# GothiProCoder/OCR-System

Measured on AMD Instinct MI355X. Metric: pages/sec end-to-end det+rec, A4@200DPI, higher is better.
Workload: dtype bf16; 1 GPU; end-to-end det+rec, batch=64 A4@200DPI pages per GPU (BASELINE configs[3]); pages_per_gpu=64, global_batch=64, lines_last_step=3279, pages_gathered_last_step=64, parallelism=pages sharded dp1, 1 all-gather/step, ranks=1, input=pages pre-decoded (uint8 RGB) and resident in HBM when the timed region starts, det_sub_batch=64

## Files before the change

### include/lumina_ocr.h

```cpp
#ifndef LUMINA_OCR_H
#define LUMINA_OCR_H
#include <stddef.h>
#include <stdint.h>

#ifdef __cplusplus
extern "C" {
#endif

typedef struct lumina_ocr lumina_ocr_t;

#define LUMINA_REC_H 32
#define LUMINA_REC_W 320
#define LUMINA_REC_T 80
#define LUMINA_MAX_WORDS 40
#define LUMINA_MAX_BOXES 1000

int lumina_ocr_create(int device, lumina_ocr_t** out);
void lumina_ocr_destroy(lumina_ocr_t* h);
const char* lumina_ocr_last_error(const lumina_ocr_t* h);
const char* lumina_ocr_version(void);
int lumina_ocr_set_option(lumina_ocr_t* h, const char* key, int value);

int lumina_ocr_load_det_weights(lumina_ocr_t* h, const void* blob, size_t nbytes);
int lumina_ocr_load_rec_weights(lumina_ocr_t* h, const void* blob, size_t nbytes);
int lumina_ocr_num_classes(const lumina_ocr_t* h);

int lumina_ocr_normalize(lumina_ocr_t* h, const uint8_t* img_dev, int n, int height, int width, int hp, int wp,
                         const float scale[3], const float shift[3], int layout_nchw, uint16_t* out_dev, void* stream);

int lumina_ocr_det_forward(lumina_ocr_t* h, const uint8_t* pages_dev, int batch, int height, int width, int hp, int wp,
                           uint16_t* prob_dev, void* stream);

int lumina_ocr_det_postprocess(lumina_ocr_t* h, const uint16_t* prob_dev, int batch, int hp, int wp, int valid_h, int valid_w,
                               float thresh, float box_thresh, float unclip_ratio, int min_size, int max_boxes,
                               int32_t* boxes_dev, float* scores_dev, int32_t* counts_dev, void* stream);

int lumina_ocr_rec_crop(lumina_ocr_t* h, const uint8_t* pages_dev, int batch, int height, int width, const int32_t* quads_dev,
                        const int32_t* page_idx_dev, int n_crops, uint8_t* crops_dev, int32_t* widths_dev, void* stream);

int lumina_ocr_rec_crop_oriented(lumina_ocr_t* h, const uint8_t* pages_dev, int batch, int height, int width, const int32_t* quads_dev,
                                 const int32_t* page_idx_dev, int n_crops, const int32_t* flip_dev, uint8_t* crops_dev, int32_t* widths_dev,
                                 void* stream);

int lumina_ocr_load_cls_weights(lumina_ocr_t* h, const void* blob, size_t nbytes);

int lumina_ocr_cls_crop(lumina_ocr_t* h, const uint8_t* pages_dev, int batch, int height, int width, const int32_t* quads_dev,
                        const int32_t* page_idx_dev, int n_crops, uint8_t* crops_dev, int32_t* widths_dev, void* stream);

int lumina_ocr_cls_forward(lumina_ocr_t* h, const uint8_t* crops_dev, const int32_t* widths_dev, int n_crops, float thresh, int32_t* label_dev,
                           float* score_dev, int32_t* flip_dev, void* stream);

int lumina_ocr_rec_forward(lumina_ocr_t* h, const uint8_t* crops_dev, const int32_t* widths_dev, int n_crops, int32_t* idx_dev,
                           float* prob_dev, void* stream);

int lumina_ocr_ctc_decode(lumina_ocr_t* h, const int32_t* idx_dev, const float* prob_dev, int n, int32_t* text_dev, int32_t* len_dev,
                          float* score_dev, void* stream);

int lumina_ocr_ctc_decode_words(lumina_ocr_t* h, const int32_t* idx_dev, const float* prob_dev, int n, const int32_t* quads_dev,
                                const int32_t* widths_dev, const int32_t* flip_dev , int space_id, int32_t* text_dev,
                                int32_t* len_dev, float* score_dev, int32_t* word_quads_dev, int32_t* word_span_dev, float* word_score_dev,
                                int32_t* word_count_dev, void* stream);

int lumina_ocr_resize_lanczos(lumina_ocr_t* h, const uint8_t* in_dev, int n, int height, int width, int channels, uint8_t* out_dev,
                              int out_h, int out_w, void* stream);
int lumina_ocr_enhance(lumina_ocr_t* h, const uint8_t* img_dev, int n, int height, int width, float contrast, float sharpness,
                       uint8_t* tmp_dev, uint8_t* out_dev, void* stream);

int lumina_ocr_binarize(lumina_ocr_t* h, const uint8_t* img_dev, int n, int height, int width, int adaptive, int threshold, uint8_t* out_dev,
                        void* stream);

int lumina_ocr_exif_transpose(lumina_ocr_t* h, const uint8_t* img_dev, int n, int height, int width, int orientation, uint8_t* out_dev, void* stream);
int lumina_ocr_grayscale(lumina_ocr_t* h, const uint8_t* img_dev, int n, int height, int width, uint8_t* out_dev, void* stream);
int lumina_ocr_denoise(lumina_ocr_t* h, const uint8_t* img_dev, int n, int height, int width, uint8_t* out_dev, void* stream);

int lumina_ocr_deskew(lumina_ocr_t* h, const uint8_t* pages_dev, int n, int height, int width, uint8_t* out_dev, double* rot_dev,
                      int32_t* info_dev, uint8_t* edges_dev, int32_t* segs_dev, int32_t* nsegs_dev, void* stream);
int lumina_ocr_deskew_warp(lumina_ocr_t* h, const uint8_t* pages_dev, int n, int height, int width, const double* rot_dev, uint8_t* out_dev,
                           void* stream);

int lumina_ocr_table_rules(lumina_ocr_t* h, const uint8_t* pages_dev, int n, int height, int width, int threshold, int gap, int min_len,
                           int max_thick, int max_rules, int32_t* hrules_dev, int32_t* vrules_dev, int32_t* counts_dev, uint64_t* hmask_dev,
                           void* stream);

int lumina_ocr_selection_marks(lumina_ocr_t* h, const uint8_t* pages_dev, int n, int height, int width, int threshold, int min_side,
                               int max_side, int max_marks, int32_t* marks_dev, int32_t* counts_dev, uint64_t* mask_dev, void* stream);

int lumina_ocr_rules_and_marks(lumina_ocr_t* h, const uint8_t* pages_dev, int n, int height, int width, int threshold, int gap, int min_len,
                               int max_thick, int max_rules, int32_t* hrules_dev, int32_t* vrules_dev, int32_t* rule_counts_dev, int min_side,
                               int max_side, int max_marks, int32_t* marks_dev, int32_t* mark_counts_dev, void* stream);

int lumina_ocr_selection_marks_round(lumina_ocr_t* h, const uint8_t* pages_dev, int n, int height, int width, int threshold, int min_side,
                                     int max_side, int max_marks, int32_t* marks_dev, int32_t* counts_dev, uint64_t* mask_dev, int out_max,
                                     int ring_div, int band_div, int band_min, int32_t* round_dev, int32_t* round_counts_dev, void* stream);

int lumina_ocr_rules_and_marks_round(lumina_ocr_t* h, const uint8_t* pages_dev, int n, int height, int width, int threshold, int gap,
                                     int min_len, int max_thick, int max_rules, int32_t* hrules_dev, int32_t* vrules_dev,
                                     int32_t* rule_counts_dev, int min_side, int max_side, int max_marks, int32_t* marks_dev,
                                     int32_t* mark_counts_dev, int out_max, int ring_div, int band_div, int band_min, int32_t* round_dev,
                                     int32_t* round_counts_dev, void* stream);

int lumina_ocr_barcodes(lumina_ocr_t* h, const uint8_t* pages_dev, int n, int height, int width, int threshold, int quiet, int max_dist,
                        int min_rows, int row_gap, int max_codes, int32_t* codes_dev, int32_t* syms_dev, int32_t* counts_dev,
                        const uint64_t* mask_in_dev, uint64_t* mask_out_dev, void* stream);

int lumina_ocr_barcodes_kinds(lumina_ocr_t* h, const uint8_t* pages_dev, int n, int height, int width, int threshold, int quiet, int max_dist,
                              int min_rows, int row_gap, int max_codes, int32_t* codes_dev, int32_t* syms_dev, int32_t* counts_dev,
                              const uint64_t* mask_in_dev, uint64_t* mask_out_dev, void* stream, int kinds);

int lumina_ocr_qrcodes(lumina_ocr_t* h, const uint8_t* pages_dev, int n, int height, int width, int threshold, int min_module, int max_module,
                       int quiet, int centre_tol, int ring_tol, int timing_max, int max_finders, int max_codes, int32_t* codes_dev,
                       int32_t* data_dev, int32_t* counts_dev, int32_t* finder_counts_dev, const uint64_t* mask_in_dev, uint64_t* mask_out_dev,
                       void* stream);

int lumina_ocr_qrcodes_versions(lumina_ocr_t* h, const uint8_t* pages_dev, int n, int height, int width, int threshold, int min_module,
                                int max_module, int quiet, int centre_tol, int ring_tol, int timing_max, int max_finders, int max_codes,
                                int max_version, int32_t* codes_dev, uint8_t* data_dev, int32_t* counts_dev, int32_t* finder_counts_dev,
                                const uint64_t* mask_in_dev, uint64_t* mask_out_dev, void* stream);

int lumina_ocr_datamatrix(lumina_ocr_t* h, const uint8_t* pages_dev, int n, int height, int width, int threshold, int min_module, int max_module,
                          int quiet, int timing_max, int solid_max, int max_candidates, int max_codes, int32_t* codes_dev, int32_t* data_dev,
                          int32_t* counts_dev, int32_t* candidate_counts_dev, const uint64_t* mask_in_dev, uint64_t* mask_out_dev, void* stream);

size_t lumina_ocr_aztec_workspace_bytes(int n, int height, int width, int max_finders, int max_codes);
int lumina_ocr_aztec(lumina_ocr_t* h, const uint8_t* pages_dev, int n, int height, int width, int threshold, int min_module, int max_module,
                     int quiet, int centre_tol, int ring_tol, int mark_max, int max_finders, int max_codes, int32_t* codes_dev, int32_t* data_dev,
                     int32_t* counts_dev, int32_t* finder_counts_dev, const uint64_t* mask_in_dev, uint64_t* mask_out_dev, void* stream);

size_t lumina_ocr_aztec_layers_workspace_bytes(int n, int height, int width, int max_finders, int max_codes);
int lumina_ocr_aztec_layers(lumina_ocr_t* h, const uint8_t* pages_dev, int n, int height, int width, int threshold, int min_module, int max_module,
                            int quiet, int centre_tol, int ring_tol, int mark_max, int max_finders, int max_codes, int max_layers, int32_t* codes_dev,
                            uint16_t* data_dev, int32_t* counts_dev, int32_t* finder_counts_dev, const uint64_t* mask_in_dev, uint64_t* mask_out_dev,
                            void* stream);

size_t lumina_ocr_page_quarter_workspace_bytes(int n, int height, int width);
int lumina_ocr_page_quarter(lumina_ocr_t* h, const uint8_t* pages_dev, int n, int height, int width, int threshold, int ratio,
                            int64_t* energies_dev, int32_t* sideways_dev, void* stream);
int lumina_ocr_page_turn(lumina_ocr_t* h, const uint8_t* pages_dev, int n, int height, int width, const int32_t* index_dev, int m, int turn,
                         uint8_t* out_dev, void* stream);
int lumina_ocr_page_vote(lumina_ocr_t* h, const int32_t* flip_dev, const int32_t* page_idx_dev, int n, int pages, int32_t* counts_dev, void* stream);

int lumina_ocr_load_svtr_weights(lumina_ocr_t* h, const void* blob, size_t nbytes);
int lumina_ocr_svtr_forward(lumina_ocr_t* h, const uint8_t* crops_dev, const int32_t* widths_dev, int n_crops, int32_t* idx_dev, float* prob_dev,
                            void* stream);
int lumina_ocr_svtr_num_classes(const lumina_ocr_t* h);
int lumina_ocr_svtr_dtype(const lumina_ocr_t* h);

int lumina_ocr_jpeg_encode(lumina_ocr_t* h, const uint8_t* pages_dev, int n, int height, int width, int quality, int optimize,
                           uint8_t* out_dev, size_t out_stride, int32_t* sizes_dev, void* stream);
int lumina_ocr_jpeg_probe(const uint8_t* file, size_t size, int info[6]);
int lumina_ocr_jpeg_decode(lumina_ocr_t* h, const uint8_t* const* files, const size_t* sizes, int n, int height, int width, uint8_t* out_dev,
                           int* status, void* stream);
int lumina_ocr_jpeg_decode_async(lumina_ocr_t* h, const uint8_t* const* files, const size_t* sizes, int n, int height, int width, uint8_t* out_dev,
                                 int* status_pinned, int passes, void* stream);
int lumina_ocr_jpeg_last_passes(const lumina_ocr_t* h);

int lumina_ocr_png_probe(const uint8_t* file, size_t size, int info[8]);
int lumina_ocr_png_decode(lumina_ocr_t* h, const uint8_t* const* files, const size_t* sizes, int n, int height, int width, uint8_t* out_dev,
                          int* status, void* stream);

int lumina_ocr_flate_image_decode(lumina_ocr_t* h, const uint8_t* const* streams, const size_t* sizes, int n, int height, int width,
                                  const int32_t* params, const uint8_t* const* palettes, uint8_t* out_dev, int* status, void* stream);
int lumina_ocr_ccitt_decode(lumina_ocr_t* h, const uint8_t* const* streams, const size_t* sizes, int n, int rows, int columns,
                            const int32_t* params, uint8_t* out_dev, int* status, void* stream);
int lumina_ocr_fax_decode(lumina_ocr_t* h, const uint8_t* const* streams, const size_t* sizes, int n, int rows, int columns,
                          const int32_t* params, uint8_t* out_dev, int* status, void* stream);

int lumina_ocr_strip_image_decode(lumina_ocr_t* h, const uint8_t* const* strips, const size_t* sizes, int m, const int32_t* strip_counts, int n,
                                  int height, int width, int rows_per_strip, const int32_t* params, const uint8_t* const* palettes,
                                  uint8_t* out_dev, int* status, void* stream);

int lumina_ocr_jpeg_coefficients(lumina_ocr_t* h, const uint8_t* pages_dev, int n, int height, int width, int quality, int16_t* coefs_dev,
                                 void* stream);

int lumina_ocr_conv2d(lumina_ocr_t* h, const uint16_t* x_dev, int n, int height, int width, int cin, const uint16_t* w_host,
                      const float* bias_host, int cout, int ks, int stride, int act, const uint16_t* res_dev, uint16_t* y_dev,
                      void* stream);
int lumina_ocr_read_tap(lumina_ocr_t* h, const char* name, uint16_t* out_host, size_t capacity_elems, int dims[4]);
int lumina_ocr_conv_timing(lumina_ocr_t* h, double* total_ms, double* total_flops, int* launches);
int lumina_ocr_conv_timing_detail(lumina_ocr_t* h, char* buf, size_t cap);

#ifdef __cplusplus
}
#endif
#endif
```

### ocr-system_amd/csrc/capi.hip

```cpp
#include <cstdlib>
#include <cstring>
#include <new>

#include "../../include/lumina_ocr.h"
#include "dbpost.h"
#include "deskew.h"
#include "engine.h"
#include "marks.h"
#include "barcodes.h"
#include "qrcodes.h"
#include "datamatrix.h"
#include "aztec.h"
#include "ops.h"
#include "orient.h"
#include "resize.h"
#include "runs.h"
#include "jpeg.h"
#include "jpegdec.h"
#include "lzw.h"
#include "pngdec.h"
#include "ccitt.h"
#include "stem_conv.h"
#include "tables.h"

#define API_TRY try {
#define API_CATCH(h)                                                             \
    }                                                                            \
    catch (const std::exception& e) { return locr_fail(h, "exception", e.what()); } \
    catch (...) { return locr_fail(h, "exception", "unknown"); }

namespace {
struct DeviceGuard {
    int prev = -1;
    hipError_t err;
    explicit DeviceGuard(int dev) {
        if (hipGetDevice(&prev) != hipSuccess) prev = -1;
        err = hipSetDevice(dev);
        if (prev == dev) prev = -1;
    }
    ~DeviceGuard() { if (prev >= 0) (void)hipSetDevice(prev); }
    DeviceGuard(const DeviceGuard&) = delete;
    DeviceGuard& operator=(const DeviceGuard&) = delete;
};
}
#define BIND(h)                                                                                              \
    if (!(h)) return 1;                                                                                      \
    DeviceGuard _device_guard((h)->device);                                                                  \
    if (_device_guard.err != hipSuccess) return locr_fail((h), "hipSetDevice", hipGetErrorString(_device_guard.err))

static int hip_rc(lumina_ocr* h, const char* what, hipError_t e) { return e == hipSuccess ? 0 : locr_fail(h, what, hipGetErrorString(e)); }

template <class F> static int drain_launches(lumina_ocr* h, const char* what, F&& f) {
    if (hipDeviceSynchronize() != hipSuccess) return locr_fail(h, what, "sync failed");
    for (const LaunchRecord& r : h->launches) {
        float t = 0.f;
        if (hipEventElapsedTime(&t, r.e0.get(), r.e1.get()) != hipSuccess) t = 0.f;
        f(r, t);
    }
    h->launches.clear();
    return 0;
}

template <class WS> static int fit_group(int group, int n, WS&& ws) {
    if (group > n) group = n;
    while (group > 1 && ws(group) > ((size_t)1 << 30)) group = (group + 1) / 2;
    return group;
}
template <class WS, class Body> static int for_page_groups(lumina_ocr* h, int n, int group, WS&& ws, Body&& body) {
    for (int b0 = 0; b0 < n; b0 += group) {
        const int nb = n - b0 < group ? n - b0 : group;
        if (eng_ws_reserve(h, ws(nb)) || body(b0, nb)) return 1;
    }
    return 0;
}

template <class T> struct CodeGroup {
    const uint8_t* rgb; int nb; int32_t* codes; T* data; int32_t* counts; int32_t* slot_counts; const unsigned long long* mask_in; unsigned long long* mask_out;
    template <class P> void bind(P& p) const { p.rgb = rgb; p.B = nb; p.codes = codes; p.counts = counts; p.mask_in = mask_in; p.mask_out = mask_out; }
};
template <class T, class WS, class Launch>
static int matrix_codes(lumina_ocr_t* h, const char* what, const char* bad_params, const uint8_t* pages_dev, int n, int height, int width, int max_codes,
                        int row_len, int32_t* codes_dev, T* data_dev, int32_t* counts_dev, int32_t* slot_counts_dev, const uint64_t* mask_in_dev,
                        uint64_t* mask_out_dev, WS ws, Launch launch) {
    if (!h) return 1;
    if (n == 0) return 0;
    if (!pages_dev || !codes_dev || !data_dev || !counts_dev || n < 0) return locr_fail(h, what, "bad arguments");
    if (bad_params) return locr_fail(h, what, bad_params);
    if (ws(1) == 0) return locr_fail(h, what, "bad dimensions (sides 1..65535)");
    BIND(h);
    API_TRY
    const size_t nw = ((size_t)width + 63) / 64;
    return for_page_groups(h, n, fit_group(h->post_group, n, ws), ws, [&](int b0, int nb) {
        CodeGroup<T> g{};
        g.rgb = pages_dev + (size_t)b0 * height * width * 3; g.nb = nb;
        g.codes = codes_dev + (size_t)b0 * max_codes * 12; g.data = data_dev + (size_t)b0 * max_codes * row_len; g.counts = counts_dev + b0;
        g.slot_counts = slot_counts_dev ? slot_counts_dev + b0 : nullptr;
        g.mask_in = mask_in_dev ? reinterpret_cast<const unsigned long long*>(mask_in_dev) + (size_t)b0 * height * nw : nullptr;
        g.mask_out = mask_out_dev ? reinterpret_cast<unsigned long long*>(mask_out_dev) + (size_t)b0 * height * nw : nullptr;
        return hip_rc(h, what, launch(g, h->ws.get(), h->ws.cap));
    });
    API_CATCH(h)
}

extern "C" {

const char* lumina_ocr_version(void) { return "lumina-ocr-mi355x 0.1 (gfx950)"; }

int lumina_ocr_create(int device, lumina_ocr_t** out) {
    if (!out) return 1;
    *out = nullptr;
    lumina_ocr* eng = new (std::nothrow) lumina_ocr();
    if (!eng) return 1;
    eng->device = device;
    int ndev = 0;
    if (hipGetDeviceCount(&ndev) != hipSuccess || device < 0 || device >= ndev) {
        eng->err = "no HIP device " + std::to_string(device) + " (device count " + std::to_string(ndev) + ")";
        *out = eng;
        return 2;
    }
    if (hipSetDevice(device) != hipSuccess) { eng->err = "hipSetDevice failed"; *out = eng; return 2; }
    if (const char* e = getenv("LUMINA_RING_ORIENT")) eng->ring_orient = atoi(e) < 0 ? -1 : (atoi(e) != 0);
    if (getenv("LUMINA_CONV_NO_RING")) eng->conv_ring = false;
    if (getenv("LUMINA_BLOCKED")) eng->blocked_layout = atoi(getenv("LUMINA_BLOCKED")) != 0;
    *out = eng;
    return 0;
}

void lumina_ocr_destroy(lumina_ocr_t* h) {
    if (!h) return;
    (void)hipSetDevice(h->device);
    delete h;
}

const char* lumina_ocr_last_error(const lumina_ocr_t* h) { return h ? h->err.c_str() : "null handle"; }

int lumina_ocr_set_option(lumina_ocr_t* h, const char* key, int value) {
    if (!h || !key) return 1;
    if (!strcmp(key, "det_sub_batch")) h->det_sub_batch = value > 0 ? value : 1;
    else if (!strcmp(key, "rec_sub_batch")) h->rec_sub_batch = value > 0 ? value : 1;
    else if (!strcmp(key, "cls_sub_batch")) h->cls_sub_batch = value > 0 ? value : 1;
    else if (!strcmp(key, "keep_taps")) h->keep_taps = value < 0 || value > 2 ? 0 : value;
    else if (!strcmp(key, "time_convs")) h->time_convs = value != 0;
    else if (!strcmp(key, "fuse_head")) h->fuse_head = value != 0;
    else if (!strcmp(key, "fuse_mb")) h->fuse_mb = value != 0;
    else if (!strcmp(key, "fuse_pool")) h->fuse_pool = value != 0;
    else if (!strcmp(key, "fuse_stem")) h->fuse_stem = value != 0;
    else if (!strcmp(key, "fpn_multi")) h->fpn_multi = value != 0;
    else if (!strcmp(key, "fpn_compose")) h->fpn_compose = value != 0;
    else if (!strcmp(key, "fuse_short")) h->fuse_short = value != 0;
    else if (!strcmp(key, "conv_ring")) h->conv_ring = value != 0;
    else if (!strcmp(key, "blocked_layout")) h->blocked_layout = value != 0;
    else if (!strcmp(key, "conv_big_min")) h->conv_big_min = value >= 0 ? value : 1024;
    else if (!strcmp(key, "ring_orient")) h->ring_orient = value < 0 ? -1 : (value != 0);
    else if (!strcmp(key, "post_group")) h->post_group = value > 0 ? value : 1;
    else if (!strcmp(key, "tail_group")) h->tail_group = value > 0 ? value : 0;
    else if (!strcmp(key, "svtr_f16")) h->svtr_f16 = value < 0 ? -1 : (value != 0);
    else if (!strcmp(key, "png_sub_batch_mb")) h->pd_sub_batch_mb = value > 0 ? value : 1;
    else if (!strcmp(key, "conv2d_variant")) h->conv2d_variant = value < 0 || value > 2 ? 0 : value;
    else return locr_fail(h, "set_option: unknown key", key);
    return 0;
}

int lumina_ocr_load_det_weights(lumina_ocr_t* h, const void* blob, size_t nbytes) {
    if (!h || !blob) return 1;
    BIND(h);
    API_TRY return eng_load_det(h, blob, nbytes); API_CATCH(h)
}
int lumina_ocr_load_rec_weights(lumina_ocr_t* h, const void* blob, size_t nbytes) {
    if (!h || !blob) return 1;
    BIND(h);
    API_TRY return eng_load_rec(h, blob, nbytes); API_CATCH(h)
}
int lumina_ocr_num_classes(const lumina_ocr_t* h) { return h ? h->num_classes : 0; }

int lumina_ocr_normalize(lumina_ocr_t* h, const uint8_t* img_dev, int n, int height, int width, int hp, int wp, const float scale[3],
                         const float shift[3], int layout_nchw, uint16_t* out_dev, void* stream) {
    if (!h || !img_dev || !out_dev || hp < height || wp < width) return locr_fail(h, "normalize", "bad arguments");
    BIND(h);
    return hip_rc(h, "normalize", normalize_launch(img_dev, out_dev, n, height, width, hp, wp, height, width, scale, shift, layout_nchw, (hipStream_t)stream));
}

int lumina_ocr_det_forward(lumina_ocr_t* h, const uint8_t* pages_dev, int batch, int height, int width, int hp, int wp, uint16_t* prob_dev,
                           void* stream) {
    if (!h || !pages_dev || !prob_dev) return locr_fail(h, "det_forward", "null argument");
    BIND(h);
    API_TRY return eng_det_forward(h, pages_dev, batch, height, width, hp, wp, prob_dev, (hipStream_t)stream); API_CATCH(h)
}

int lumina_ocr_det_postprocess(lumina_ocr_t* h, const uint16_t* prob_dev, int batch, int hp, int wp, int valid_h, int valid_w, float thresh,
                               float box_thresh, float unclip_ratio, int min_size, int max_boxes, int32_t* boxes_dev, float* scores_dev,
                               int32_t* counts_dev, void* stream) {
    if (!h || !prob_dev || !boxes_dev || !scores_dev || !counts_dev) return locr_fail(h, "det_postprocess", "null argument");
    if (batch <= 0 || max_boxes <= 0 || valid_h > hp || valid_w > wp) return locr_fail(h, "det_postprocess", "bad dimensions");
    BIND(h);
    API_TRY
    return for_page_groups(h, batch, h->post_group, [&](int nb) { return dbpost_workspace_bytes(nb, hp, wp, max_boxes); }, [&](int b0, int nb) {
        DbPostParams p{};
        p.prob = prob_dev + (size_t)b0 * hp * wp; p.B = nb; p.Hp = hp; p.Wp = wp; p.valid_h = valid_h; p.valid_w = valid_w;
        p.thresh = thresh; p.box_thresh = box_thresh; p.unclip_ratio = unclip_ratio; p.min_size = min_size; p.max_boxes = max_boxes;
        p.boxes = boxes_dev + (size_t)b0 * max_boxes * 8; p.scores = scores_dev + (size_t)b0 * max_boxes; p.counts = counts_dev + b0;
        return hip_rc(h, "det_postprocess", dbpost_launch(p, h->ws.get(), h->ws.cap, (hipStream_t)stream));
    });
    API_CATCH(h)
}

int lumina_ocr_rec_crop(lumina_ocr_t* h, const uint8_t* pages_dev, int batch, int height, int width, const int32_t* quads_dev,
                        const int32_t* page_idx_dev, int n_crops, uint8_t* crops_dev, int32_t* widths_dev, void* stream) {
    if (!h || !pages_dev || !quads_dev || !page_idx_dev || !crops_dev || !widths_dev) return locr_fail(h, "rec_crop", "null argument");
    BIND(h);
    (void)batch;
    return hip_rc(h, "rec_crop", rec_crop_launch(pages_dev, height, width, quads_dev, page_idx_dev, n_crops, crops_dev, widths_dev, (hipStream_t)stream));
}

int lumina_ocr_load_cls_weights(lumina_ocr_t* h, const void* blob, size_t nbytes) {
    if (!h || !blob) return locr_fail(h, "load_cls_weights", "null argument");
    BIND(h);
    API_TRY return eng_load_cls(h, blob, nbytes); API_CATCH(h)
}

int lumina_ocr_cls_forward(lumina_ocr_t* h, const uint8_t* crops_dev, const int32_t* widths_dev, int n_crops, float thresh, int32_t* label_dev,
                           float* score_dev, int32_t* flip_dev, void* stream) {
    if (!h) return 1;
    if (n_crops <= 0) return 0;
    if (!crops_dev || !label_dev || !score_dev || !flip_dev) return locr_fail(h, "cls_forward", "null argument");
    BIND(h);
    API_TRY return eng_cls_forward(h, crops_dev, widths_dev, n_crops, thresh, label_dev, score_dev, flip_dev, (hipStream_t)stream); API_CATCH(h)
}

int lumina_ocr_rec_crop_oriented(lumina_ocr_t* h, const uint8_t* pages_dev, int batch, int height, int width, const int32_t* quads_dev,
                                 const int32_t* page_idx_dev, int n_crops, const int32_t* flip_dev, uint8_t* crops_dev, int32_t* widths_dev,
                                 void* stream) {
    if (!h) return 1;
    if (n_crops <= 0) return 0;
    if (!pages_dev || !quads_dev || !page_idx_dev || !flip_dev || !crops_dev || !widths_dev) return locr_fail(h, "rec_crop_oriented", "null argument");
    BIND(h);
    (void)batch;
    return hip_rc(h, "rec_crop_oriented", rec_crop_launch(pages_dev, height, width, quads_dev, page_idx_dev, n_crops, crops_dev, widths_dev,
                                                         (hipStream_t)stream, flip_dev));
}

int lumina_ocr_cls_crop(lumina_ocr_t* h, const uint8_t* pages_dev, int batch, int height, int width, const int32_t* quads_dev,
                        const int32_t* page_idx_dev, int n_crops, uint8_t* crops_dev, int32_t* widths_dev, void* stream) {
    if (!h) return 1;
    if (n_crops <= 0) return 0;
    if (!pages_dev || !quads_dev || !page_idx_dev || !crops_dev || !widths_dev) return locr_fail(h, "cls_crop", "null argument");
    BIND(h);
    (void)batch;
    return hip_rc(h, "cls_crop", cls_crop_launch(pages_dev, height, width, quads_dev, page_idx_dev, n_crops, crops_dev, widths_dev, (hipStream_t)stream));
}

int lumina_ocr_rec_forward(lumina_ocr_t* h, const uint8_t* crops_dev, const int32_t* widths_dev, int n_crops, int32_t* idx_dev, float* prob_dev,
                           void* stream) {
    if (!h || !crops_dev || !idx_dev || !prob_dev) return locr_fail(h, "rec_forward", "null argument");
    BIND(h);
    API_TRY return eng_rec_forward(h, crops_dev, widths_dev, n_crops, idx_dev, prob_dev, (hipStream_t)stream); API_CATCH(h)
}

int lumina_ocr_load_svtr_weights(lumina_ocr_t* h, const void* blob, size_t nbytes) {
    if (!h || !blob) return locr_fail(h, "load_svtr_weights", "null argument");
    BIND(h);
    API_TRY return eng_load_svtr(h, blob, nbytes); API_CATCH(h)
}

int lumina_ocr_svtr_forward(lumina_ocr_t* h, const uint8_t* crops_dev, const int32_t* widths_dev, int n_crops, int32_t* idx_dev, float* prob_dev,
                            void* stream) {
    if (!h || !crops_dev || !idx_dev || !prob_dev) return locr_fail(h, "svtr_forward", "null argument");
    BIND(h);
    API_TRY return eng_svtr_forward(h, crops_dev, widths_dev, n_crops, idx_dev, prob_dev, (hipStream_t)stream); API_CATCH(h)
}

int lumina_ocr_ctc_decode(lumina_ocr_t* h, const int32_t* idx_dev, const float* prob_dev, int n, int32_t* text_dev, int32_t* len_dev,
                          float* score_dev, void* stream) {
    if (!h || !idx_dev || !prob_dev || !text_dev || !len_dev || !score_dev) return locr_fail(h, "ctc_decode", "null argument");
    BIND(h);
    if (n <= 0) return 0;
    return hip_rc(h, "ctc_decode", ctc_collapse_launch(idx_dev, prob_dev, text_dev, len_dev, score_dev, n, LUMINA_REC_T, (hipStream_t)stream));
}

int lumina_ocr_ctc_decode_words(lumina_ocr_t* h, const int32_t* idx_dev, const float* prob_dev, int n, const int32_t* quads_dev,
                                const int32_t* widths_dev, const int32_t* flip_dev, int space_id, int32_t* text_dev, int32_t* len_dev,
                                float* score_dev, int32_t* word_quads_dev, int32_t* word_span_dev, float* word_score_dev, int32_t* word_count_dev,
                                void* stream) {
    if (!h) return 1;
    if (n <= 0) return 0;
    if (!idx_dev || !prob_dev || !quads_dev || !widths_dev || !text_dev || !len_dev || !score_dev || !word_quads_dev || !word_span_dev ||
        !word_score_dev || !word_count_dev)
        return locr_fail(h, "ctc_decode_words", "null argument");
    BIND(h);
    return hip_rc(h, "ctc_decode_words", ctc_words_launch(idx_dev, prob_dev, quads_dev, widths_dev, flip_dev, space_id, text_dev, len_dev, score_dev,
                                                          word_quads_dev, word_span_dev, word_score_dev, word_count_dev, n, LUMINA_REC_T,
                                                          (hipStream_t)stream));
}

int lumina_ocr_conv2d(lumina_ocr_t* h, const uint16_t* x_dev, int n, int height, int width, int cin, const uint16_t* w_host,
                      const float* bias_host, int cout, int ks, int stride, int act, const uint16_t* res_dev, uint16_t* y_dev, void* stream) {
    if (!h || !x_dev || !w_host || !bias_host || !y_dev) return locr_fail(h, "conv2d", "null argument");
    if (cout % 8 != 0) return locr_fail(h, "conv2d", "cout must be a multiple of 8");
    BIND(h);
    API_TRY
    ConvLayer L;
    L.name = "conv2d"; L.ks = ks; L.stride = stride; L.cin = cin; L.cout = cout; L.act = act;
    if (!conv_pick_cfg(ks, stride, cin, cout, &L.cfg)) return locr_fail(h, "conv2d", "unsupported ks/stride/cin");
    std::vector<bf16_t> packed(conv_packed_weight_elems(cout, ks, cin, L.cfg.bn));
    pack_conv_weights(w_host, cout, ks, cin, L.cfg.bn, L.cfg.ck, packed.data(), L.cfg.nw == 6 ? 1 : 0);
    const int ntiles = (cout + L.cfg.bn - 1) / L.cfg.bn;
    std::vector<float> bias((size_t)ntiles * L.cfg.bn, 0.f);
    memcpy(bias.data(), bias_host, sizeof(float) * cout);
    const bool big_ok = ks == 3 && stride == 1 && cin >= 32 && cin % 16 == 0 && cout % 64 == 0 && L.cfg.bn == 64;
    if (h->conv2d_variant > 0 && !big_ok) return locr_fail(h, "conv2d", "conv2d_variant 1/2 needs ks 3, stride 1, cin % 16 == 0, cin >= 32, cout % 64 == 0");
    DeviceMem dw, db, dw2;
    auto upload = [](DeviceMem* d, const void* host, size_t bytes) {
        hipError_t e = mem_alloc(d, bytes);
        return e == hipSuccess ? hipMemcpy(d->get(), host, bytes, hipMemcpyHostToDevice) : e;
    };
    if (upload(&dw, packed.data(), packed.size() * 2) != hipSuccess || upload(&db, bias.data(), bias.size() * 4) != hipSuccess) return locr_fail(h, "conv2d", "weight upload");
    L.wpk = static_cast<bf16_t*>(dw.get()); L.bias = static_cast<float*>(db.get());
    if (h->conv2d_variant > 0) {
        L.cfg_big = L.cfg; L.cfg_big.nw = 6; L.cfg_big.ck = 16;
        std::vector<bf16_t> packed2(conv_packed_weight_elems(cout, ks, cin, 64));
        pack_conv_weights(w_host, cout, ks, cin, 64, 16, packed2.data(), 1);
        if (upload(&dw2, packed2.data(), packed2.size() * 2) != hipSuccess) return locr_fail(h, "conv2d", "weight upload");
        L.wpk_big = static_cast<bf16_t*>(dw2.get());
    }
    Tensor4 x; x.p = const_cast<bf16_t*>(x_dev); x.n = n; x.h = height; x.w = width; x.c = cin;
    Tensor4 y; y.p = y_dev; y.n = n; y.c = cout;
    y.h = (ks == 3) ? (height - 1) / stride + 1 : height / stride;
    y.w = (ks == 3) ? (width - 1) / stride + 1 : width / stride;
    Tensor4 r; r.p = const_cast<bf16_t*>(res_dev); r.n = n; r.h = y.h; r.w = y.w; r.c = cout;
    ConvCall call;
    call.res = res_dev ? &r : nullptr; call.variant = h->conv2d_variant;
    int rc = eng_run_conv(h, L, x, &y, (hipStream_t)stream, call);
    hipError_t e = hipStreamSynchronize((hipStream_t)stream);
    if (rc) return rc;
    return hip_rc(h, "conv2d sync", e);
    API_CATCH(h)
}

int lumina_ocr_read_tap(lumina_ocr_t* h, const char* name, uint16_t* out_host, size_t capacity_elems, int dims[4]) {
    if (!h || !name || !dims) return 1;
    auto it = h->taps.find(name);
    if (it == h->taps.end()) return locr_fail(h, "read_tap: unknown tap", name);
    BIND(h);
    const Tensor4& t = it->second;
    dims[0] = t.n; dims[1] = t.h; dims[2] = t.w; dims[3] = t.c;
    if (!out_host) return 0;
    if (capacity_elems < t.elems()) return locr_fail(h, "read_tap", "buffer too small");
    if (hipDeviceSynchronize() != hipSuccess) return locr_fail(h, "read_tap", "sync failed");
    return hip_rc(h, "read_tap", hipMemcpy(out_host, t.p, t.elems() * sizeof(bf16_t), hipMemcpyDeviceToHost));
}

int lumina_ocr_conv_timing(lumina_ocr_t* h, double* total_ms, double* total_flops, int* launches) {
    if (!h || !total_ms || !total_flops || !launches) return 1;
    BIND(h);
    double ms = 0, fl = 0;
    int count = 0;
    if (drain_launches(h, "conv_timing", [&](const LaunchRecord& r, float t) { ms += t; fl += r.flop; ++count; })) return 1;
    *total_ms = ms; *total_flops = fl; *launches = count;
    return 0;
}

static int get_coeffs(lumina_ocr* h, int in_size, int out_size, lumina_ocr::Coeffs* out) {
    auto key = std::make_pair(in_size, out_size);
    auto it = h->coeff_cache.find(key);
    if (it == h->coeff_cache.end()) {
        std::vector<int> bounds, kk;
        lumina_ocr::Coeffs c;
        lanczos_coeffs(in_size, out_size, &c.ksize, &bounds, &kk);
        c.bounds_host = std::make_shared<std::vector<int>>(bounds);
        c.bounds = static_cast<int*>(eng_upload(h, bounds.data(), bounds.size() * 4));
        c.kk = static_cast<int*>(eng_upload(h, kk.data(), kk.size() * 4));
        if (!c.bounds || !c.kk) return locr_fail(h, "resize", "coefficient table upload");
        it = h->coeff_cache.emplace(key, c).first;
    }
    *out = it->second;
    return 0;
}

int lumina_ocr_resize_lanczos(lumina_ocr_t* h, const uint8_t* in_dev, int n, int height, int width, int channels, uint8_t* out_dev,
                              int out_h, int out_w, void* stream) {
    if (!h || !in_dev || !out_dev || n <= 0 || height <= 0 || width <= 0 || out_h <= 0 || out_w <= 0 || channels <= 0)
        return locr_fail(h, "resize_lanczos", "bad arguments");
    BIND(h);
    API_TRY
    hipStream_t st = (hipStream_t)stream;
    const uint8_t* src = in_dev;
    int cur_w = width;
    const bool need_h = out_w != width, need_v = out_h != height;
    if (!need_h && !need_v) {
        return hip_rc(h, "resize_lanczos", hipMemcpyAsync(out_dev, in_dev, (size_t)n * height * width * channels, hipMemcpyDeviceToDevice, st));
    }
    if (need_h) {
        lumina_ocr::Coeffs c;
        if (get_coeffs(h, width, out_w, &c)) return 1;
        uint8_t* dst = out_dev;
        if (need_v) {
            if (hip_rc(h, "resize_lanczos", h->aux.reserve((size_t)n * height * out_w * channels))) return 1;
            dst = h->aux.get();
        }
        if (hip_rc(h, "resize_lanczos", resample_launch(src, dst, c.bounds, c.kk, c.ksize, n, height, width, channels, out_w, 0, c.bounds_host->data(), st))) return 1;
        src = dst; cur_w = out_w;
    }
    if (need_v) {
        lumina_ocr::Coeffs c;
        if (get_coeffs(h, height, out_h, &c)) return 1;
        if (hip_rc(h, "resize_lanczos", resample_launch(src, out_dev, c.bounds, c.kk, c.ksize, n, height, cur_w, channels, out_h, 1, c.bounds_host->data(), st))) return 1;
    }
    return 0;
    API_CATCH(h)
}

int lumina_ocr_enhance(lumina_ocr_t* h, const uint8_t* img_dev, int n, int height, int width, float contrast, float sharpness,
                       uint8_t* tmp_dev, uint8_t* out_dev, void* stream) {
    if (!h || !img_dev || !tmp_dev || !out_dev || n <= 0) return locr_fail(h, "enhance", "bad arguments");
    BIND(h);
    if (hip_rc(h, "enhance", h->sums.reserve(sizeof(unsigned long long) * (size_t)n))) return 1;
    unsigned long long* sums = reinterpret_cast<unsigned long long*>(h->sums.get());
    return hip_rc(h, "enhance", enhance_launch(img_dev, tmp_dev, out_dev, sums, n, height, width, contrast, sharpness, (hipStream_t)stream));
}

int lumina_ocr_binarize(lumina_ocr_t* h, const uint8_t* img_dev, int n, int height, int width, int adaptive, int threshold, uint8_t* out_dev, void* stream) {
    if (!h || !img_dev || !out_dev || n <= 0 || height <= 0 || width <= 0) return locr_fail(h, "binarize", "bad arguments");
    BIND(h);
    return hip_rc(h, "binarize", binarize_launch(img_dev, out_dev, n, height, width, adaptive != 0, threshold, (hipStream_t)stream));
}

int lumina_ocr_exif_transpose(lumina_ocr_t* h, const uint8_t* img_dev, int n, int height, int width, int orientation, uint8_t* out_dev, void* stream) {
    if (!h || !img_dev || !out_dev || n <= 0 || height <= 0 || width <= 0 || orientation < 1 || orientation > 8 || img_dev == out_dev)
        return locr_fail(h, "exif_transpose", "bad arguments (orientation 1..8, not in place)");
    BIND(h);
    return hip_rc(h, "exif_transpose", exif_transpose_launch(img_dev, out_dev, n, height, width, orientation, (hipStream_t)stream));
}

int lumina_ocr_grayscale(lumina_ocr_t* h, const uint8_t* img_dev, int n, int height, int width, uint8_t* out_dev, void* stream) {
    if (!h || !img_dev || !out_dev || n <= 0 || height <= 0 || width <= 0) return locr_fail(h, "grayscale", "bad arguments");
    BIND(h);
    return hip_rc(h, "grayscale", grayscale_launch(img_dev, out_dev, n, height, width, (hipStream_t)stream));
}

int lumina_ocr_denoise(lumina_ocr_t* h, const uint8_t* img_dev, int n, int height, int width, uint8_t* out_dev, void* stream) {
    if (!h || !img_dev || !out_dev || n <= 0 || height <= 0 || width <= 0 || img_dev == out_dev) return locr_fail(h, "denoise", "bad arguments (not in place)");
    BIND(h);
    return hip_rc(h, "denoise", median3_launch(img_dev, out_dev, n, height, width, (hipStream_t)stream));
}

int lumina_ocr_jpeg_encode(lumina_ocr_t* h, const uint8_t* pages_dev, int n, int height, int width, int quality, int optimize,
                           uint8_t* out_dev, size_t out_stride, int32_t* sizes_dev, void* stream) {
    if (!h || !pages_dev || !out_dev || !sizes_dev || n <= 0 || height <= 0 || width <= 0) return locr_fail(h, "jpeg_encode", "bad arguments");
    BIND(h);
    API_TRY
    if (eng_ws_reserve(h, jpeg_workspace_bytes(n, height, width))) return 1;
    JpegParams p{};
    p.rgb = pages_dev; p.n = n; p.height = height; p.width = width; p.quality = quality; p.optimize = optimize != 0; p.out = out_dev; p.out_stride = out_stride; p.sizes = sizes_dev;
    return hip_rc(h, "jpeg_encode", jpeg_encode_launch(p, h->ws.get(), h->ws.cap, (hipStream_t)stream));
    API_CATCH(h)
}

int lumina_ocr_jpeg_probe(const uint8_t* file, size_t size, int info[6]) {
    if (!file || !info) return -1;
    JdInfo i{};
    const int rc = jpegdec_probe(file, size, &i);
    info[0] = i.width; info[1] = i.height; info[2] = i.ncomp; info[3] = i.hs; info[4] = i.vs; info[5] = i.restart;
    return rc;
}

// ... 483 lines not shown
```

### ocr-system_amd/csrc/conv_mfma.h

```cpp
#pragma once
#include "common.h"

enum ConvOutMode : int {
    OUT_NORMAL = 0,
    OUT_UPSAMPLE = 1,
    OUT_CONVT = 2,
    OUT_CONVT1 = 3,
    OUT_POOL = 4,
};

struct ConvParams {
    const bf16_t* x;
    const bf16_t* wpk;
    const float* bias;
    const bf16_t* res;
    bf16_t* y;
    int N, H, W, Cin;
    int Ho, Wo;
    int Cout;
    int y_cstride, y_coff;
    int res_cstride, res_h, res_w, res_shift;
    int act;
    int out_mode, up_shift, convt_c;
    int tiles_x, tiles_y, n_tiles;
    const bf16_t* fuse_w;
    float fuse_b;
    const bf16_t* gate;
    int gate_hw;
    int dbg_skip;
    int pix_limit;
    const bf16_t* zeros;
    int x_blk, y_blk, res_blk;
    int n_src;
    const bf16_t* xs[4];
    int xs_shift[4];
    int xs_nchunk[4], xs_cstride[4];
    const bf16_t* wpk2;
    const float* bias2;
    bf16_t* y2;
    int y2_cstride;
};

struct ConvKernelCfg {
    int ks, stride, bn, ck, tw, nw;
};

size_t conv_packed_weight_elems(int cout_gemm, int ks, int cin, int bn);
void pack_conv_weights(const bf16_t* ohwi, int cout_gemm, int ks, int cin, int bn, int ck, bf16_t* out, int row_major = 0);

bool conv_pick_cfg(int ks, int stride, int cin, int cout_gemm, ConvKernelCfg* cfg);
hipError_t conv_launch(const ConvKernelCfg& cfg, ConvParams p, hipStream_t stream);
const char* conv_kernel_name(const ConvKernelCfg& cfg);

bool conv_ring_supported(const ConvKernelCfg& cfg, const ConvParams& p);
bool conv_ring_transposed(const ConvParams& p, int orientation);
hipError_t conv_ring_launch(ConvParams p, int orientation, hipStream_t stream);
const char* conv_ring_kernel_name(const ConvParams& p, int orientation);

bool conv_pw_supported(const ConvKernelCfg& cfg, const ConvParams& p);
hipError_t conv_pw_launch(const ConvParams& p, hipStream_t stream);
```

### ocr-system_amd/csrc/conv_mfma.hip

```cpp
#include "conv_mfma.h"

#include <cstdlib>

namespace {

template <int KS, int S, int BN, int CK, int TW, int NW = 4, int DB = 0, int MT = 2>
struct Cfg {
    static constexpr int NTHR = NW * 64;
    static constexpr bool DMA = (DB == 3 || DB == 4);
    static constexpr bool POOL = (DB == 4);
    static constexpr bool SC = (DB == 5);
    static_assert(!SC || (KS == 3 && S == 2 && CK == 16), "fused shortcut: the 3x3 / stride-2 block-entry kernel");
    static constexpr int TH = NW * MT;
    static constexpr int PAD = (KS == 3) ? 1 : 0;
    static constexpr int HH = (TH - 1) * S + KS;
    static constexpr int HW = (TW - 1) * S + KS;
    static constexpr int HWP = HW;
    static constexpr int NPL = CK / 8;
    static constexpr int HPX = HH * HWP;
    static constexpr int PMOD = (NPL >= 8) ? 2 : 4;
    static constexpr int PLANE_A = HPX + ((PMOD - HPX % 16) + 16) % 16;
    static constexpr int TAPS = KS * KS;
    static constexpr int WROWS = TAPS * BN;
    static constexpr int PLANE_W = WROWS;
    static constexpr int NT = BN / 32;
    static constexpr int A_BYTES = DMA ? HPX * NPL * 16 : PLANE_A * NPL * 16;
    static constexpr int W_BYTES = PLANE_W * NPL * 16;
    static constexpr int W2_ROWS = SC ? 4 * BN : 0, W2_ITEMS = W2_ROWS * NPL, W2IT = (W2_ITEMS + NTHR - 1) / NTHR, W2_BYTES = W2_ITEMS * 16;
    static constexpr int A_PIX = DMA ? NPL * 16 : 16, A_SL = DMA ? 16 : PLANE_A * 16;
    static constexpr int W_ROW = DMA ? NPL * 16 : 16, W_SL = DMA ? 16 : PLANE_W * 16;
    static constexpr int STAGE_PITCH = BN * 2 + 16;
    static constexpr int STAGE_BYTES = TH * TW * STAGE_PITCH;
    static constexpr int BUF_BYTES = A_BYTES + W_BYTES + W2_BYTES;
    static constexpr int LDS_BYTES = (BUF_BYTES * (DMA ? 2 : 1)) > STAGE_BYTES ? (BUF_BYTES * (DMA ? 2 : 1)) : STAGE_BYTES;
    static_assert(!DMA || (CK == 16 && KS == 3 && S == 1), "DMA variant: 3x3 / stride 1 / 16-channel chunks");
    static constexpr int A_ITEMS = HH * HW * NPL;
    static constexpr int AIT = (A_ITEMS + NTHR - 1) / NTHR;
    static constexpr int W_ITEMS = WROWS * NPL;
    static constexpr int WIT = (W_ITEMS + NTHR - 1) / NTHR;
    static constexpr int CPP = BN / 8;
};

__device__ __forceinline__ bf16x8_t lds_frag(const unsigned char* p) { return *reinterpret_cast<const bf16x8_t*>(p); }

__device__ __forceinline__ uint32_t mul_bf16x2(uint32_t a, uint32_t b) {
    const float lo = __uint_as_float(a << 16) * __uint_as_float(b << 16);
    const float hi = __uint_as_float(a & 0xFFFF0000u) * __uint_as_float(b & 0xFFFF0000u);
    return pack_bf16x2(lo, hi);
}
__device__ __forceinline__ uint4 mul_bf16x8(uint4 a, uint4 b) {
    return make_uint4(mul_bf16x2(a.x, b.x), mul_bf16x2(a.y, b.y), mul_bf16x2(a.z, b.z), mul_bf16x2(a.w, b.w));
}

template <int KS, int S, int BN, int CK, int TW, int NW, int DB, int MT>
__global__ __launch_bounds__(NW * 64, (BN <= 64 ? 2 : 1)) void conv_mfma_kernel(const ConvParams p) {
    using C = Cfg<KS, S, BN, CK, TW, NW, DB, MT>;
    constexpr int NTHR = C::NTHR;
    extern __shared__ __attribute__((aligned(16))) unsigned char smem[];

    const int tid = threadIdx.x, lane = tid & 63, wave = tid >> 6;
    unsigned char* sA = smem;
    unsigned char* sW = sA + C::A_BYTES;
    const int r = lane & 31, h = lane >> 5;

    const int lid = xcd_remap(blockIdx.x, gridDim.x);
    const int ntile = lid % p.n_tiles;
    const int mtile = lid / p.n_tiles;
    const int tiles_per_img = p.tiles_x * p.tiles_y;
    const int n_img = mtile / tiles_per_img;
    const int trem = mtile - n_img * tiles_per_img;
    const int tile_y = trem / p.tiles_x, tile_x = trem - tile_y * p.tiles_x;

    const bf16_t* ximg = p.x + (size_t)n_img * p.H * p.W * p.Cin;
    const int nchunks = p.Cin / CK;
    const bf16_t* wbase = p.wpk + (size_t)ntile * nchunks * C::W_ITEMS * 8;

    const bool blk_dbg = CK == 16 && (p.dbg_skip & 8);
    const int pstride = blk_dbg ? 16 : p.Cin;
    const int cadv = blk_dbg ? p.H * p.W * 16 : CK;
    int a_goff[C::AIT], a_loff[C::AIT];
    int a_gate[KS == 1 ? C::AIT : 1];
    constexpr bool pool = C::POOL;
    const int oyb = pool ? tile_y * (C::TH - 2) - 1 : tile_y * C::TH, oxb = pool ? tile_x * (TW - 2) - 1 : tile_x * TW;
    const int iy0 = oyb * S - C::PAD, ix0 = oxb * S - C::PAD;
#pragma unroll
    for (int it = 0; it < C::AIT; ++it) {
        const int i = tid + NTHR * it;
        const int pi = i / C::NPL, c = i - pi * C::NPL;
        const int hy = pi / C::HW, hx = pi - hy * C::HW;
        const int iy = iy0 + hy, ix = ix0 + hx;
        const bool item = i < C::A_ITEMS;
        const bool inb = item && iy >= 0 && iy < p.H && ix >= 0 && ix < p.W && (p.pix_limit == 0 || iy * p.W + ix < p.pix_limit);
        a_goff[it] = inb ? (iy * p.W + ix) * pstride + c * 8 : -1;
        a_loff[it] = item ? (c * C::PLANE_A + hy * C::HWP + hx) * 16 : -1;
        if constexpr (KS == 1) a_gate[it] = (inb && p.gate != nullptr) ? ((iy * p.W + ix) / p.gate_hw) * p.Cin + c * 8 : -1;
    }

    uint4 a_reg[C::AIT], w_reg[C::WIT];
    uint4 g_reg[KS == 1 ? C::AIT : 1];
    uint4 w2_reg[C::SC ? C::W2IT : 1];
    unsigned char* sW2 = sW + C::W_BYTES;
    const bf16_t* wbase2 = C::SC ? p.wpk2 + (size_t)ntile * nchunks * C::W2_ITEMS * 8 : nullptr;
#define ISSUE_LOADS(chunk_)                                                                          \
    {                                                                                                \
        const bf16_t* xa = ximg + (chunk_) * cadv;                                                   \
        const bool skipa_ = (p.dbg_skip & 2) && (chunk_) > 0, skipw_ = (p.dbg_skip & 1) && (chunk_) > 0; \
        _Pragma("unroll") for (int it = 0; it < C::AIT; ++it) {                                      \
            uint4 t_ = make_uint4(0, 0, 0, 0);                                                       \
            if (a_goff[it] >= 0 && !skipa_) t_ = *reinterpret_cast<const uint4*>(xa + a_goff[it]);   \
            a_reg[it] = t_;                                                                          \
            if constexpr (KS == 1) {                                                                 \
                uint4 g_ = make_uint4(0, 0, 0, 0);                                                   \
                if (a_gate[it] >= 0) g_ = *reinterpret_cast<const uint4*>(p.gate + a_gate[it] + (chunk_) * CK); \
                g_reg[it] = g_;                                                                      \
            }                                                                                        \
        }                                                                                            \
        const uint4* wsrc = reinterpret_cast<const uint4*>(wbase + (size_t)(chunk_) * C::W_ITEMS * 8); \
        _Pragma("unroll") for (int it = 0; it < C::WIT; ++it) {                                      \
            const int i = tid + NTHR * it;                                                          \
            uint4 t_ = make_uint4(0, 0, 0, 0);                                                       \
            if ((C::W_ITEMS % NTHR == 0 || i < C::W_ITEMS) && !skipw_) t_ = wsrc[i];                 \
            w_reg[it] = t_;                                                                          \
        }                                                                                            \
        if constexpr (C::SC) {                                                                       \
            const uint4* w2src = reinterpret_cast<const uint4*>(wbase2 + (size_t)(chunk_) * C::W2_ITEMS * 8); \
            _Pragma("unroll") for (int it = 0; it < C::W2IT; ++it) {                                 \
                const int i = tid + NTHR * it;                                                      \
                uint4 t_ = make_uint4(0, 0, 0, 0);                                                   \
                if (C::W2_ITEMS % NTHR == 0 || i < C::W2_ITEMS) t_ = w2src[i];                       \
                w2_reg[it] = t_;                                                                     \
            }                                                                                        \
        }                                                                                            \
    }
#define WRITE_LDS(boff_)                                                                             \
    {                                                                                                \
        _Pragma("unroll") for (int it = 0; it < C::AIT; ++it) {                                      \
            if constexpr (KS == 1) { if (a_gate[it] >= 0) a_reg[it] = mul_bf16x8(a_reg[it], g_reg[it]); } \
            if (a_loff[it] >= 0) *reinterpret_cast<uint4*>(sA + (boff_) + a_loff[it]) = a_reg[it];   \
        }                                                                                            \
        _Pragma("unroll") for (int it = 0; it < C::WIT; ++it) {                                      \
            const int i = tid + NTHR * it;                                                          \
            if (C::W_ITEMS % NTHR == 0 || i < C::W_ITEMS) *reinterpret_cast<uint4*>(sW + (boff_) + i * 16) = w_reg[it]; \
        }                                                                                            \
        if constexpr (C::SC) {                                                                       \
            _Pragma("unroll") for (int it = 0; it < C::W2IT; ++it) {                                 \
                const int i = tid + NTHR * it;                                                      \
                if (C::W2_ITEMS % NTHR == 0 || i < C::W2_ITEMS) *reinterpret_cast<uint4*>(sW2 + (boff_) + i * 16) = w2_reg[it]; \
            }                                                                                        \
        }                                                                                            \
    }

#define DMA_ISSUE(chunk_, boff_)                                                                     \
    {                                                                                                \
        const bf16_t* xa = ximg + (chunk_) * cadv;                                                   \
        const bool skipa_ = (p.dbg_skip & 2) && (chunk_) > 0, skipw_ = (p.dbg_skip & 1) && (chunk_) > 0; \
        _Pragma("unroll") for (int it = 0; it < C::AIT; ++it) {                                      \
            const int i = tid + NTHR * it;                                                           \
            if ((C::A_ITEMS % NTHR == 0 || i < C::A_ITEMS) && !skipa_) {                             \
                const bf16_t* src_ = a_goff[it] >= 0 ? xa + a_goff[it] : p.zeros;                    \
                __builtin_amdgcn_global_load_lds((const __attribute__((address_space(1))) void*)(src_), \
                    (__attribute__((address_space(3))) void*)(sA + (boff_) + (i - lane) * 16), 16, 0, 0); \
            }                                                                                        \
        }                                                                                            \
        const bf16_t* wsrc = wbase + (size_t)(chunk_) * C::W_ITEMS * 8;                              \
        _Pragma("unroll") for (int it = 0; it < C::WIT; ++it) {                                      \
            const int i = tid + NTHR * it;                                                           \
            if ((C::W_ITEMS % NTHR == 0 || i < C::W_ITEMS) && !skipw_)                               \
                __builtin_amdgcn_global_load_lds((const __attribute__((address_space(1))) void*)(wsrc + i * 8), \
                    (__attribute__((address_space(3))) void*)(sW + (boff_) + (i - lane) * 16), 16, 0, 0); \
        }                                                                                            \
    }

    f32x16_t acc[MT][C::NT];
#pragma unroll
    for (int mt = 0; mt < MT; ++mt)
#pragma unroll
        for (int nt = 0; nt < C::NT; ++nt)
#pragma unroll
            for (int j = 0; j < 16; ++j) acc[mt][nt][j] = 0.f;
    f32x16_t acc2[C::SC ? MT : 1][C::SC ? C::NT : 1];
    if constexpr (C::SC) {
#pragma unroll
        for (int mt = 0; mt < MT; ++mt)
#pragma unroll
            for (int nt = 0; nt < C::NT; ++nt)
#pragma unroll
                for (int j = 0; j < 16; ++j) acc2[mt][nt][j] = 0.f;
    }

    int aoff[MT];
#pragma unroll
    for (int mt = 0; mt < MT; ++mt) {
        const int ty = wave * MT + mt, tx = r;
        aoff[mt] = h * C::A_SL + ((ty * S) * C::HWP + tx * S) * C::A_PIX;
    }
    const int woff = h * C::W_SL + r * C::W_ROW;
    const int woff2 = h * (C::W2_ROWS * 16) + r * 16;

    constexpr int NSTEPS = C::TAPS * (CK / 16);
    bf16x8_t bfr[2][MT], afr[2][C::NT];
#define LOAD_FRAGS(boff_, st_, set_)                                                                               \
    {                                                                                                              \
        const int tap_ = (st_) / (CK / 16), kc_ = (st_) % (CK / 16), kh_ = tap_ / KS, kw_ = tap_ % KS;              \
        _Pragma("unroll") for (int mt = 0; mt < MT; ++mt)                                                           \
            bfr[set_][mt] = lds_frag(sA + (boff_) + aoff[mt] + (2 * kc_) * C::A_SL + (kh_ * C::HWP + kw_) * C::A_PIX); \
        _Pragma("unroll") for (int nt = 0; nt < C::NT; ++nt)                                                       \
            afr[set_][nt] = lds_frag(sW + (boff_) + woff + (2 * kc_) * C::W_SL + (tap_ * BN + nt * 32) * C::W_ROW);   \
    }
#define COMPUTE_CHUNK(boff_)                                                                                       \
    LOAD_FRAGS(boff_, 0, 0)                                                                                        \
    __builtin_amdgcn_sched_barrier(0);                                                                             \
    _Pragma("unroll") for (int st = 0; st < NSTEPS; ++st) {                                                        \
        _Pragma("unroll") for (int mt = 0; mt < MT; ++mt)                                                           \
            _Pragma("unroll") for (int nt = 0; nt < C::NT; ++nt)                                                   \
                acc[mt][nt] = __builtin_amdgcn_mfma_f32_32x32x16_bf16(afr[st & 1][nt], bfr[st & 1][mt], acc[mt][nt], 0, 0, 0); \
        if constexpr (C::SC) {    \
            if (st == 4 || st == 5 || st == 7 || st == 8) {                                                        \
                const int t2_ = (st == 4) ? 0 : (st == 5) ? 1 : (st == 7) ? 2 : 3;                                 \
                bf16x8_t a2_[C::NT];                                                                               \
                _Pragma("unroll") for (int nt = 0; nt < C::NT; ++nt) a2_[nt] = lds_frag(sW2 + (boff_) + woff2 + (t2_ * BN + nt * 32) * 16); \
                _Pragma("unroll") for (int mt = 0; mt < MT; ++mt)                                                   \
                    _Pragma("unroll") for (int nt = 0; nt < C::NT; ++nt)                                           \
                        acc2[mt][nt] = __builtin_amdgcn_mfma_f32_32x32x16_bf16(a2_[nt], bfr[st & 1][mt], acc2[mt][nt], 0, 0, 0); \
            }                                                                                                      \
        }                                                                                                          \
        if (st + 1 < NSTEPS) LOAD_FRAGS(boff_, st + 1, (st + 1) & 1)                                               \
        _Pragma("unroll") for (int q_ = 0; q_ < MT * C::NT; ++q_) {                                                \
            __builtin_amdgcn_sched_group_barrier(0x008, 1, 0);                      \
            if (q_ < MT + C::NT) __builtin_amdgcn_sched_group_barrier(0x100, 1, 0);  \
        }                                                                                                          \
        __builtin_amdgcn_sched_barrier(0);                                                                         \
    }
    if constexpr (C::DMA) {
        DMA_ISSUE(0, 0);
        for (int chunk = 0; chunk < nchunks; ++chunk) {
            const int boff = (chunk & 1) * C::BUF_BYTES;
            asm volatile("s_waitcnt vmcnt(0)" ::: "memory");
            __syncthreads();
            if (chunk + 1 < nchunks) DMA_ISSUE(chunk + 1, C::BUF_BYTES - boff);
            COMPUTE_CHUNK(boff)
        }
    } else {
        ISSUE_LOADS(0);
        for (int chunk = 0; chunk < nchunks; ++chunk) {
            __syncthreads();
            WRITE_LDS(0);
            __syncthreads();
            if (chunk + 1 < nchunks) ISSUE_LOADS(chunk + 1);
            COMPUTE_CHUNK(0)
        }
    }
#undef COMPUTE_CHUNK
#undef LOAD_FRAGS
#undef DMA_ISSUE

    const int cout_r8 = (p.Cout + 7) & ~7;
    const float* bptr = p.bias + ntile * BN;
    float4 bias_r[C::NT][4];
#pragma unroll
    for (int nt = 0; nt < C::NT; ++nt)
#pragma unroll
        for (int g = 0; g < 4; ++g) bias_r[nt][g] = *reinterpret_cast<const float4*>(bptr + nt * 32 + 8 * g + 4 * h);
    uint2 res_r[MT][C::NT][4];
    const bool has_res = p.res != nullptr;
    if (has_res) {
#pragma unroll
        for (int mt = 0; mt < MT; ++mt) {
            const int ty = wave * MT + mt, tx = r;
            const int oy = oyb + ty, ox = oxb + tx;
            const bool pvalid = oy >= 0 && ox >= 0 && oy < p.Ho && ox < p.Wo && (p.pix_limit == 0 || oy * p.Wo + ox < p.pix_limit);
            const bf16_t* rrow = p.res + (((size_t)n_img * p.res_h + (oy >> p.res_shift)) * p.res_w + (ox >> p.res_shift)) * p.res_cstride + ntile * BN;
#pragma unroll
            for (int nt = 0; nt < C::NT; ++nt)
#pragma unroll
                for (int g = 0; g < 4; ++g) {
                    const int cn = nt * 32 + 8 * g + 4 * h;
                    uint2 rv = make_uint2(0, 0);
                    if (pvalid && ntile * BN + cn < cout_r8) rv = *reinterpret_cast<const uint2*>(rrow + cn);
                    res_r[mt][nt][g] = rv;
                }
        }
    }
    const bool direct = KS == 3 && !C::DMA && p.out_mode == OUT_NORMAL && !(p.dbg_skip & 32);
    if (!direct) __syncthreads();
    unsigned char* stage = smem;
#pragma unroll
    for (int mt = 0; mt < MT; ++mt)
#pragma unroll
        for (int nt = 0; nt < C::NT; ++nt)
#pragma unroll
            for (int g = 0; g < 4; ++g) {
                const float4 b4 = bias_r[nt][g];
                acc[mt][nt][4 * g + 0] += b4.x; acc[mt][nt][4 * g + 1] += b4.y;
                acc[mt][nt][4 * g + 2] += b4.z; acc[mt][nt][4 * g + 3] += b4.w;
                if (has_res) {
                    const uint2 rv = res_r[mt][nt][g];
                    acc[mt][nt][4 * g + 0] += __uint_as_float(rv.x << 16); acc[mt][nt][4 * g + 1] += __uint_as_float(rv.x & 0xFFFF0000u);
                    acc[mt][nt][4 * g + 2] += __uint_as_float(rv.y << 16); acc[mt][nt][4 * g + 3] += __uint_as_float(rv.y & 0xFFFF0000u);
                }
            }
#define FOR_ALL_ACC(expr)                                                          \
    _Pragma("unroll") for (int mt = 0; mt < MT; ++mt)                               \
        _Pragma("unroll") for (int nt = 0; nt < C::NT; ++nt)                       \
            _Pragma("unroll") for (int j = 0; j < 16; ++j) { const float v = acc[mt][nt][j]; acc[mt][nt][j] = (expr); }
    if (p.act == ACT_RELU) { FOR_ALL_ACC(fmaxf(v, 0.f)) }
    else if (p.act == ACT_HSWISH) { FOR_ALL_ACC(v * fminf(fmaxf(v + 3.f, 0.f), 6.f) * (1.f / 6.f)) }
    else if (p.act == ACT_SIGMOID) { FOR_ALL_ACC(fast_sigmoidf(v)) }
    else if (p.act == ACT_HSIGMOID) { FOR_ALL_ACC(fminf(fmaxf(0.2f * v + 0.5f, 0.f), 1.f)) }
    else if (p.act == ACT_GELU) { FOR_ALL_ACC(gelu_erf(v)) }
#undef FOR_ALL_ACC
    if constexpr (KS == 3) {
        if (direct) {
#pragma unroll
            for (int mt = 0; mt < MT; ++mt) {
                const int oy = oyb + wave * MT + mt, ox = oxb + r;
                const bool pvalid = oy < p.Ho && ox < p.Wo;
#pragma unroll
                for (int nt = 0; nt < C::NT; ++nt)
#pragma unroll
                    for (int gp = 0; gp < 2; ++gp) {
                        const int g0 = 2 * gp, g1 = 2 * gp + 1;
                        const uint32_t q0x = pack_bf16x2(acc[mt][nt][4 * g0 + 0], acc[mt][nt][4 * g0 + 1]), q0y = pack_bf16x2(acc[mt][nt][4 * g0 + 2], acc[mt][nt][4 * g0 + 3]);
                        const uint32_t q1x = pack_bf16x2(acc[mt][nt][4 * g1 + 0], acc[mt][nt][4 * g1 + 1]), q1y = pack_bf16x2(acc[mt][nt][4 * g1 + 2], acc[mt][nt][4 * g1 + 3]);
                        const auto sx = __builtin_amdgcn_permlane32_swap(q0x, q1x, false, false);
                        const auto sy = __builtin_amdgcn_permlane32_swap(q0y, q1y, false, false);
                        const uint4 v = make_uint4(sx[0], sy[0], sx[1], sy[1]);
                        const int co = ntile * BN + nt * 32 + 16 * gp + 8 * h;
                        if (!pvalid || co >= cout_r8) continue;
                        *reinterpret_cast<uint4*>(p.y + (((size_t)n_img * p.Ho + oy) * p.Wo + ox) * p.y_cstride + p.y_coff + co) = v;
                    }
            }
            if constexpr (C::SC) {
                const float* b2 = p.bias2 + ntile * BN;
#pragma unroll
                for (int mt = 0; mt < MT; ++mt) {
                    const int oy = oyb + wave * MT + mt, ox = oxb + r;
                    const bool pvalid = oy < p.Ho && ox < p.Wo;
#pragma unroll
                    for (int nt = 0; nt < C::NT; ++nt)
#pragma unroll
                        for (int gp = 0; gp < 2; ++gp) {
                            const int g0 = 2 * gp, g1 = 2 * gp + 1;
                            const float4 ba = *reinterpret_cast<const float4*>(b2 + nt * 32 + 8 * g0 + 4 * h), bb = *reinterpret_cast<const float4*>(b2 + nt * 32 + 8 * g1 + 4 * h);
                            const uint32_t q0x = pack_bf16x2(acc2[mt][nt][4 * g0 + 0] + ba.x, acc2[mt][nt][4 * g0 + 1] + ba.y), q0y = pack_bf16x2(acc2[mt][nt][4 * g0 + 2] + ba.z, acc2[mt][nt][4 * g0 + 3] + ba.w);
                            const uint32_t q1x = pack_bf16x2(acc2[mt][nt][4 * g1 + 0] + bb.x, acc2[mt][nt][4 * g1 + 1] + bb.y), q1y = pack_bf16x2(acc2[mt][nt][4 * g1 + 2] + bb.z, acc2[mt][nt][4 * g1 + 3] + bb.w);
                            const auto sx = __builtin_amdgcn_permlane32_swap(q0x, q1x, false, false);
                            const auto sy = __builtin_amdgcn_permlane32_swap(q0y, q1y, false, false);
                            const uint4 v = make_uint4(sx[0], sy[0], sx[1], sy[1]);
                            const int co = ntile * BN + nt * 32 + 16 * gp + 8 * h;
                            if (!pvalid || co >= cout_r8) continue;
                            *reinterpret_cast<uint4*>(p.y2 + (((size_t)n_img * p.Ho + oy) * p.Wo + ox) * p.y2_cstride + co) = v;
                        }
                }
            }
            return;
        }
    }
#pragma unroll
    for (int mt = 0; mt < MT; ++mt) {
        const int tp = (wave * MT + mt) * TW + r;
#pragma unroll
        for (int nt = 0; nt < C::NT; ++nt)
#pragma unroll
            for (int g = 0; g < 4; ++g) {
                const int cn = nt * 32 + 8 * g + 4 * h;
                uint2 o;
                o.x = pack_bf16x2(acc[mt][nt][4 * g + 0], acc[mt][nt][4 * g + 1]);
                o.y = pack_bf16x2(acc[mt][nt][4 * g + 2], acc[mt][nt][4 * g + 3]);
                *reinterpret_cast<uint2*>(stage + tp * C::STAGE_PITCH + cn * 2) = o;
            }
    }
    __syncthreads();
    if (p.out_mode == OUT_CONVT && p.fuse_w != nullptr) {
        if constexpr (BN == 64) {
            const int q = ntile;
#pragma unroll
            for (int mt = 0; mt < MT; ++mt) {
                f32x16_t d2;
#pragma unroll
                for (int j = 0; j < 16; ++j) d2[j] = 0.f;
                const int tp = (wave * MT + mt) * TW + r;
#pragma unroll
                for (int ks = 0; ks < 4; ++ks) {
                    const bf16x8_t bfr = lds_frag(stage + tp * C::STAGE_PITCH + (ks * 16 + h * 8) * 2);
                    const bf16x8_t afr = *reinterpret_cast<const bf16x8_t*>(p.fuse_w + ((ks * 2 + h) * 32 + r) * 8);
                    d2 = __builtin_amdgcn_mfma_f32_32x32x16_bf16(afr, bfr, d2, 0, 0, 0);
                }
                const int ty = wave * MT + mt, tx = r;
                const int oy = oyb + ty, ox = oxb + tx;
                if (h == 0 && oy < p.Ho && ox < p.Wo) {
                    const int yy = 4 * oy + 2 * (q >> 1), xx = 4 * ox + 2 * (q & 1);
                    bf16_t* dst = p.y + ((size_t)n_img * (4 * p.Ho) + yy) * (size_t)(4 * p.Wo) + xx;
                    *reinterpret_cast<uint32_t*>(dst) = pack_bf16x2(apply_act(d2[0] + p.fuse_b, ACT_SIGMOID), apply_act(d2[1] + p.fuse_b, ACT_SIGMOID));
                    *reinterpret_cast<uint32_t*>(dst + 4 * p.Wo) = pack_bf16x2(apply_act(d2[2] + p.fuse_b, ACT_SIGMOID), apply_act(d2[3] + p.fuse_b, ACT_SIGMOID));
                }
            }
        }
        return;
    }
    if constexpr (C::POOL) {
        {
            constexpr int PH = (C::TH - 2) / 2, PW = (TW - 2) / 2;
            const int Hq = (p.Ho - 1) / 2 + 1, Wq = (p.Wo - 1) / 2 + 1;
            for (int i = tid; i < PH * PW * C::CPP; i += NTHR) {
                const int pp = i / C::CPP, ch = i - pp * C::CPP;
                const int pr = pp / PW, pc = pp - pr * PW;
                const int py = tile_y * PH + pr, px = tile_x * PW + pc;
                const int co = ntile * BN + ch * 8;
                if (py >= Hq || px >= Wq || co >= cout_r8) continue;
                float m[8];
#pragma unroll
                for (int j = 0; j < 8; ++j) m[j] = -3.0e38f;
#pragma unroll
                for (int dy = 0; dy < 3; ++dy)
#pragma unroll
                    for (int dx = 0; dx < 3; ++dx) {
                        const int lr = 2 * pr + dy, lc = 2 * pc + dx;
                        const int cy = oyb + lr, cx = oxb + lc;
                        if (cy < 0 || cy >= p.Ho || cx < 0 || cx >= p.Wo) continue;
                        const uint4 v = *reinterpret_cast<const uint4*>(stage + (lr * TW + lc) * C::STAGE_PITCH + ch * 16);
                        const uint32_t w4[4] = {v.x, v.y, v.z, v.w};
#pragma unroll
                        for (int j = 0; j < 4; ++j) {
                            m[2 * j] = fmaxf(m[2 * j], __uint_as_float(w4[j] << 16));
                            m[2 * j + 1] = fmaxf(m[2 * j + 1], __uint_as_float(w4[j] & 0xFFFF0000u));
                        }
                    }
                const uint4 o = make_uint4(pack_bf16x2(m[0], m[1]), pack_bf16x2(m[2], m[3]), pack_bf16x2(m[4], m[5]), pack_bf16x2(m[6], m[7]));
                *reinterpret_cast<uint4*>(p.y + (((size_t)n_img * Hq + py) * Wq + px) * p.y_cstride + p.y_coff + co) = o;
            }
            return;
        }
    }
#pragma unroll
    for (int k = 0; k < (C::TH * TW * C::CPP + NTHR - 1) / NTHR; ++k) {
        const int i = tid + NTHR * k;
        const int tp = i / C::CPP, ch = i - tp * C::CPP;
        if (tp >= C::TH * TW) continue;
        const int ty = tp / TW, tx = tp - ty * TW;
        const int oy = oyb + ty, ox = oxb + tx;
        const int co = ntile * BN + ch * 8;
        if (oy >= p.Ho || ox >= p.Wo || co >= cout_r8 || (p.pix_limit != 0 && oy * p.Wo + ox >= p.pix_limit)) continue;
        const uint4 v = *reinterpret_cast<const uint4*>(stage + tp * C::STAGE_PITCH + ch * 16);
        if (p.out_mode == OUT_NORMAL) {
            bf16_t* dst = p.y + (((size_t)n_img * p.Ho + oy) * p.Wo + ox) * p.y_cstride + p.y_coff + co;
            *reinterpret_cast<uint4*>(dst) = v;
        } else if (p.out_mode == OUT_UPSAMPLE) {
            const int f = 1 << p.up_shift;
            const int HoU = p.Ho << p.up_shift, WoU = p.Wo << p.up_shift;
            for (int dy = 0; dy < f; ++dy)
                for (int dx = 0; dx < f; ++dx) {
                    bf16_t* dst = p.y + (((size_t)n_img * HoU + (oy * f + dy)) * WoU + (ox * f + dx)) * p.y_cstride + p.y_coff + co;
                    *reinterpret_cast<uint4*>(dst) = v;
                }
        } else if (p.out_mode == OUT_CONVT) {
            const int q = co / p.convt_c, cc = co - q * p.convt_c;
            const int yy = 2 * oy + (q >> 1), xx = 2 * ox + (q & 1);
            bf16_t* dst = p.y + (((size_t)n_img * (2 * p.Ho) + yy) * (2 * p.Wo) + xx) * p.y_cstride + p.y_coff + cc;
            *reinterpret_cast<uint4*>(dst) = v;
        } else {
            if (ch == 0) {
                bf16_t* dst = p.y + ((size_t)n_img * (2 * p.Ho) + 2 * oy) * (size_t)(2 * p.Wo) + 2 * ox;
                *reinterpret_cast<uint32_t*>(dst) = v.x;
                *reinterpret_cast<uint32_t*>(dst + 2 * p.Wo) = v.y;
            }
        }
    }
}

template <int KS, int S, int BN, int CK, int TW, int NW = 4, int DB = 0, int MT = 2>
hipError_t launch_t(const ConvParams& p, hipStream_t stream) {
    using C = Cfg<KS, S, BN, CK, TW, NW, DB, MT>;
    auto kern = conv_mfma_kernel<KS, S, BN, CK, TW, NW, DB, MT>;
    { hipError_t e = locr_dyn_lds(reinterpret_cast<const void*>(kern), C::LDS_BYTES); if (e != hipSuccess) return e; }
    const int grid = p.N * p.tiles_x * p.tiles_y * p.n_tiles;
    hipLaunchKernelGGL(kern, dim3(grid), dim3(C::NTHR), C::LDS_BYTES, stream, p);
    return hipGetLastError();
}

}

size_t conv_packed_weight_elems(int cout_gemm, int ks, int cin, int bn) {
    const int ntiles = (cout_gemm + bn - 1) / bn;
    return (size_t)ntiles * bn * ks * ks * cin;
}

void pack_conv_weights(const bf16_t* ohwi, int cout_gemm, int ks, int cin, int bn, int ck, bf16_t* out, int row_major) {
    const int ntiles = (cout_gemm + bn - 1) / bn, taps = ks * ks, npl = ck / 8, nchunks = cin / ck;
    const size_t wrows = (size_t)taps * bn;
    if (row_major) {
        for (int nt = 0; nt < ntiles; ++nt)
            for (int chunk = 0; chunk < nchunks; ++chunk)
                for (int tap = 0; tap < taps; ++tap)
                    for (int n = 0; n < bn; ++n) {
                        const int co = nt * bn + n;
                        bf16_t* dst = out + (((size_t)nt * nchunks + chunk) * wrows + (size_t)tap * bn + n) * ck;
                        for (int j = 0; j < ck; ++j)
                            dst[j] = co < cout_gemm ? ohwi[((size_t)co * taps + tap) * cin + chunk * ck + j] : (bf16_t)0;
                    }
        return;
    }
    for (int nt = 0; nt < ntiles; ++nt)
        for (int chunk = 0; chunk < nchunks; ++chunk)
            for (int c = 0; c < npl; ++c)
                for (int tap = 0; tap < taps; ++tap)
                    for (int n = 0; n < bn; ++n) {
                        const int co = nt * bn + n;
                        bf16_t* dst = out + ((((size_t)nt * nchunks + chunk) * npl + c) * wrows + (size_t)tap * bn + n) * 8;
                        for (int j = 0; j < 8; ++j)
                            dst[j] = co < cout_gemm ? ohwi[((size_t)co * taps + tap) * cin + chunk * ck + c * 8 + j] : (bf16_t)0;
                    }
}

bool conv_pick_cfg(int ks, int stride, int cin, int cout_gemm, ConvKernelCfg* cfg) {
    if (!((ks == 1 && stride == 1) || (ks == 2 && stride == 2) || (ks == 3 && (stride == 1 || stride == 2)))) return false;
    if (cin % 16 != 0) return false;
    cfg->ks = ks; cfg->stride = stride; cfg->tw = 32; cfg->nw = 4;
    cfg->ck = (cin % 32 == 0) ? 32 : 16;
    cfg->bn = cout_gemm <= 32 ? 32 : (cout_gemm <= 64 ? 64 : 128);
    if (cfg->bn == 128) cfg->bn = 64;
    if (ks == 3 && stride == 2 && cfg->bn == 128 && cfg->ck == 32) cfg->bn = 64;
    if (stride == 2) cfg->ck = 16;
    if (const char* e = getenv("LUMINA_CONV_CKS2")) { if (stride == 2) cfg->ck = atoi(e) == 32 && cin % 32 == 0 ? 32 : 16; }
    if (ks == 3 && stride == 1 && cin == 32 && cfg->bn == 32) cfg->ck = 16;
    if (const char* e = getenv("LUMINA_CONV_CK3")) { if (ks == 3 && stride == 1 && cin >= atoi(e)) cfg->ck = 16; }
    if (const char* e = getenv("LUMINA_CONV_NW")) {
        if ((atoi(e) == 5 || atoi(e) == 6) && ks == 3 && stride == 1 && cfg->bn == 64 && cin >= 64) { cfg->nw = atoi(e); cfg->ck = 16; }
    }
    return true;
}

const char* conv_kernel_name(const ConvKernelCfg& c) {
    static thread_local char buf[64];
    const int db = c.nw == 6 ? 3 : 0, mt = (c.nw == 5 || c.nw == 6) ? 4 : 2;
    snprintf(buf, sizeof(buf), "conv_mfma_kernel<%d,%d,%d,%d,32,4,%d,%d>", c.ks, c.stride, c.bn, c.ck, db, mt);
    return buf;
}

#define DISPATCH(KS_, S_, BN_, CK_)                                                             \
    if (cfg.ks == KS_ && cfg.stride == S_ && cfg.bn == BN_ && cfg.ck == CK_) return launch_t<KS_, S_, BN_, CK_, 32>(p, stream);

hipError_t conv_launch(const ConvKernelCfg& cfg, ConvParams p, hipStream_t stream) {
    static const int dbg = getenv("LUMINA_CONV_DBG") ? atoi(getenv("LUMINA_CONV_DBG")) : 0;
    p.dbg_skip = dbg;
    p.tiles_x = ceil_div(p.Wo, 32);
    p.tiles_y = ceil_div(p.Ho, 8);
    p.n_tiles = ceil_div(p.Cout, cfg.bn);
    if (cfg.nw == 5) {
        p.tiles_y = ceil_div(p.Ho, 16);
        if (cfg.ks == 3 && cfg.stride == 1 && cfg.bn == 64 && cfg.ck == 16) return launch_t<3, 1, 64, 16, 32, 4, 0, 4>(p, stream);
        return hipErrorInvalidValue;
    }
    if (p.wpk2 != nullptr) {
        if (!(cfg.ks == 3 && cfg.stride == 2 && cfg.bn == 64 && cfg.ck == 16 && cfg.nw == 4) || p.out_mode != OUT_NORMAL || (dbg & 32) || p.bias2 == nullptr ||
            p.y2 == nullptr || p.H % 2 != 0 || p.W % 2 != 0 || p.res != nullptr || p.y2_cstride % 8 != 0) return hipErrorInvalidValue;
        return launch_t<3, 2, 64, 16, 32, 4, 5, 2>(p, stream);
    }
    if (p.out_mode == OUT_POOL && cfg.nw != 6) return hipErrorInvalidValue;
    if (cfg.nw == 6) {
        p.tiles_y = ceil_div(p.Ho, 16);
        if (p.out_mode == OUT_POOL) {
            p.tiles_y = ceil_div((p.Ho - 1) / 2 + 1, 7);
            p.tiles_x = ceil_div((p.Wo - 1) / 2 + 1, 15);
        }
        if (p.zeros == nullptr) return hipErrorInvalidValue;
        if (cfg.ks == 3 && cfg.stride == 1 && cfg.bn == 64 && cfg.ck == 16)
            return p.out_mode == OUT_POOL ? launch_t<3, 1, 64, 16, 32, 4, 4, 4>(p, stream) : launch_t<3, 1, 64, 16, 32, 4, 3, 4>(p, stream);
        return hipErrorInvalidValue;
    }
    DISPATCH(3, 1, 32, 32) DISPATCH(3, 1, 64, 32) DISPATCH(3, 1, 128, 32) DISPATCH(3, 1, 64, 16)
    DISPATCH(3, 2, 32, 32) DISPATCH(3, 2, 64, 32) DISPATCH(3, 2, 64, 16)
    DISPATCH(1, 1, 32, 32) DISPATCH(1, 1, 64, 32) DISPATCH(1, 1, 128, 32)
    DISPATCH(1, 1, 32, 16) DISPATCH(1, 1, 64, 16) DISPATCH(1, 1, 128, 16)
    DISPATCH(2, 2, 32, 32) DISPATCH(2, 2, 64, 32) DISPATCH(2, 2, 128, 32) DISPATCH(2, 2, 32, 16) DISPATCH(2, 2, 64, 16)
    DISPATCH(3, 2, 32, 16) DISPATCH(3, 1, 32, 16)
    return hipErrorInvalidValue;
}
```

### ocr-system_amd/csrc/engine.h

```cpp
#pragma once
#include <map>
#include <memory>
#include <string>
#include <type_traits>
#include <vector>

#include "common.h"
#include "conv_mfma.h"
#include "mbconv.h"
#include "svtr.h"

struct Tensor4 {
    bf16_t* p = nullptr;
    int n = 0, h = 0, w = 0, c = 0;
    bool blk = false;
    int n_src = 0; const bf16_t* xs[4] = {nullptr, nullptr, nullptr, nullptr}; int xs_shift[4] = {0, 0, 0, 0};
    int xs_c[4] = {0, 0, 0, 0}, xs_cs[4] = {0, 0, 0, 0};
    int src_c(int k) const { return xs_c[k] ? xs_c[k] : c / n_src; }
    int src_cs(int k) const { return xs_cs[k] ? xs_cs[k] : src_c(k); }
    size_t elems() const { return (size_t)n * h * w * c; }
};

struct ConvLayer {
    std::string name;
    int ks = 1, stride = 1, cin = 0, cout = 0;
    int act = ACT_NONE;
    bool convt = false;
    int convt_c = 0;
    ConvKernelCfg cfg{};
    bf16_t* wpk = nullptr;
    ConvKernelCfg cfg_big{}; bf16_t* wpk_big = nullptr;
    bf16_t* fuse_w = nullptr; float fuse_b = 0.f;
    double alg_flop_per_px = 0;
    float* bias = nullptr;
};

struct DwLayer { int k = 3, c = 0; bf16_t* w = nullptr; float* bias = nullptr; };
struct SeLayer { int c = 0, mid = 0; bf16_t *w1 = nullptr, *w2 = nullptr; float *b1 = nullptr, *b2 = nullptr; };

struct RecBlock {
    int k, cin, exp, cout, se_mid, stride_h, act;
    bool se, res;
    ConvLayer expand, project;
    DwLayer dw;
    bf16_t* we_pk = nullptr; float* be_pk = nullptr;
    SeLayer sel;
};

struct SvtrLinear {
    int K = 0, N = 0, taps = 1, cin = 0, act = ACT_NONE;
    uint16_t* w = nullptr;
    float* bias = nullptr;
    float *gamma = nullptr, *beta = nullptr;
};
struct SvtrBlock { int dim = 0, heads = 0, gh = 0, gw = 0; bool local = false; SvtrLinear qkv, proj, fc1, fc2; };
struct SvtrModel {
    bool loaded = false;
    int dtype = 0;
    int dims[3] = {64, 128, 256}, depths[3] = {3, 6, 3}, heads[3] = {2, 4, 8}, local_blocks = 6, out_ch = 192;
    int num_classes = 0, ctc_ntiles = 0;
    SvtrLinear pe1, pe2, sub[2], last;
    uint16_t* pos = nullptr;
    std::vector<SvtrBlock> blocks;
    bf16_t* ctc_wpk = nullptr; float* ctc_bias = nullptr;
};

struct DeviceFree { void operator()(void* p) const { (void)hipFree(p); } };
struct PinnedFree { void operator()(void* p) const { (void)hipHostFree(p); } };
struct EventDestroy { void operator()(hipEvent_t e) const { (void)hipEventDestroy(e); } };
using DeviceMem = std::unique_ptr<void, DeviceFree>;
using PinnedMem = std::unique_ptr<void, PinnedFree>;
using Event = std::unique_ptr<std::remove_pointer<hipEvent_t>::type, EventDestroy>;
inline hipError_t mem_alloc(DeviceMem* m, size_t bytes) { void* p = nullptr; hipError_t e = hipMalloc(&p, bytes); m->reset(p); return e; }
inline hipError_t mem_alloc(PinnedMem* m, size_t bytes) { void* p = nullptr; hipError_t e = hipHostMalloc(&p, bytes, hipHostMallocDefault); m->reset(p); return e; }

template <class Mem> struct Growable {
    Mem mem;
    size_t cap = 0;
    uint8_t* get() const { return static_cast<uint8_t*>(mem.get()); }
    hipError_t reserve(size_t bytes, hipEvent_t in_use = nullptr) {
        if (bytes <= cap) return hipSuccess;
        hipError_t e = in_use ? hipEventSynchronize(in_use) : hipDeviceSynchronize();
        if (e != hipSuccess) return e;
        mem.reset(); cap = 0;
        if ((e = mem_alloc(&mem, bytes)) != hipSuccess) return e;
        cap = bytes;
        return hipSuccess;
    }
};

struct LaunchRecord { Event e0, e1; double flop, bytes; std::string layer, kernel; };

struct HostBlobTensor { int dtype; std::vector<int> dims; const uint8_t* data; size_t nbytes; };

struct lumina_ocr {
    int device = 0;
    std::string err;
    bool det_loaded = false;
    std::map<std::string, ConvLayer> det;
    bf16_t* stem_wpk = nullptr; float* stem_bias = nullptr;
    bool rec_loaded = false;
    int num_classes = 0, ctc_ntiles = 0;
    bf16_t* rstem_wpk = nullptr; float* rstem_bias = nullptr;
    std::vector<RecBlock> rblocks;
    ConvLayer rconv2, xproj[2];
    bf16_t* whh[2] = {nullptr, nullptr};
    bf16_t* ctc_wpk = nullptr; float* ctc_bias = nullptr;
    SvtrModel svtr;
    bool cls_loaded = false;
    bf16_t* cstem_wpk = nullptr; float* cstem_bias = nullptr;
    std::vector<RecBlock> cblocks;
    ConvLayer cconv2;
    float *cls_fc_w = nullptr, *cls_fc_b = nullptr;
    Growable<DeviceMem> ws;
    Arena arena;
    std::vector<DeviceMem> owned;
    bf16_t* zeros = nullptr;
    int det_sub_batch = 16, rec_sub_batch = 4096, cls_sub_batch = 4096, post_group = 64;
    int tail_group = 16;
    std::map<std::string, Tensor4> taps;
    int keep_taps = 0;
    bool fuse_head = true;
    bool fuse_pool = true;
    int conv_big_min = 1024;
    bool blocked_layout = true;
    bool conv_ring = true;
    int svtr_f16 = -1;
    int conv2d_variant = 0;
    int ring_orient = -1;
    bool fuse_short = true;
    bool fpn_compose = true;
    bool fpn_multi = true;
    bool fuse_stem = true;
    bool fuse_mb = true;
    bool time_convs = false;
    std::vector<LaunchRecord> launches;
    struct Coeffs { int ksize = 0; int* bounds = nullptr; int* kk = nullptr; std::shared_ptr<std::vector<int>> bounds_host; };
    std::map<std::pair<int, int>, Coeffs> coeff_cache;
    Growable<DeviceMem> aux;
    Growable<DeviceMem> sums;
    int jd_last_passes = 0;
    struct Staging { Growable<PinnedMem> buf; Event uploaded; };
    Staging jd_stage[2];
    int jd_stage_next = 0;
    Staging pd_stage;
    int pd_sub_batch_mb = 768;
    float* dk_trig = nullptr; short* dk_wtab = nullptr;
};

int locr_fail(lumina_ocr* eng, const char* what, const char* detail);
bool parse_blob(lumina_ocr* eng, const void* blob, size_t n, std::map<std::string, HostBlobTensor>* out);

int eng_load_det(lumina_ocr* eng, const void* blob, size_t n);
int eng_load_rec(lumina_ocr* eng, const void* blob, size_t n);
int eng_det_forward(lumina_ocr* eng, const uint8_t* pages, int B, int H, int W, int Hp, int Wp, bf16_t* prob, hipStream_t st);
int eng_rec_forward(lumina_ocr* eng, const uint8_t* crops, const int* widths, int N, int* idx, float* prob, hipStream_t st);
int eng_load_svtr(lumina_ocr* eng, const void* blob, size_t n);
int eng_load_cls(lumina_ocr* eng, const void* blob, size_t n);
int eng_cls_forward(lumina_ocr* eng, const uint8_t* crops, const int* widths, int N, float thresh, int* label, float* score, int* flip, hipStream_t st);
int eng_svtr_forward(lumina_ocr* eng, const uint8_t* crops, const int* widths, int N, int* idx, float* prob, hipStream_t st);
int eng_ws_reserve(lumina_ocr* eng, size_t bytes);
void* eng_upload(lumina_ocr* eng, const void* host, size_t bytes);
struct ConvCall {
    const Tensor4* res = nullptr; int res_shift = 0;
    int out_mode = OUT_NORMAL, up_shift = 0;
    int y_cstride = 0, y_coff = 0;
    bool flat = false;
    const bf16_t* gate = nullptr;
    const ConvLayer* short_l = nullptr; Tensor4* short_y = nullptr;
    int variant = 0;
    ConvCall& residual(const Tensor4* r, int shift = 0) { res = r; res_shift = shift; return *this; }
    ConvCall& mode(int m) { out_mode = m; return *this; }
    ConvCall& upsample(int shift) { out_mode = OUT_UPSAMPLE; up_shift = shift; return *this; }
    ConvCall& channel_slice(int cstride, int coff) { y_cstride = cstride; y_coff = coff; return *this; }
    ConvCall& flat_gemm(bool on = true) { flat = on; return *this; }
    ConvCall& gated(const bf16_t* g) { gate = g; return *this; }
    ConvCall& shortcut(const ConvLayer* l, Tensor4* y) { short_l = l; short_y = y; return *this; }
};
int eng_run_conv(lumina_ocr* eng, const ConvLayer& L, const Tensor4& x, Tensor4* y, hipStream_t st, const ConvCall& c = {});
```

### ocr-system_amd/csrc/engine.hip

```cpp
#include "engine.h"

#include <cstdlib>
#include <cstring>

#include "ops.h"
#include "stem_conv.h"

int locr_fail(lumina_ocr* eng, const char* what, const char* detail) {
    if (eng) eng->err = std::string(what) + ": " + (detail ? detail : "");
    return 1;
}

#define RUN(expr) do { if ((expr) != 0) return 1; } while (0)

#include <mutex>
#include <set>
hipError_t locr_dyn_lds(const void* kernel, int bytes) {
    static std::mutex mu;
    static std::set<std::pair<int, const void*>> done;
    int dev = 0;
    hipError_t e = hipGetDevice(&dev);
    if (e != hipSuccess) return e;
    std::lock_guard<std::mutex> lk(mu);
    if (done.count({dev, kernel})) return hipSuccess;
// ... 67 lines not shown

static inline int rup(int v, int m) { return (v + m - 1) / m * m; }
constexpr int CLS_H = 48, CLS_W = 192, CLS_FEAT = 200;

static bool get_wb(lumina_ocr* eng, const std::map<std::string, HostBlobTensor>& m, const std::string& name,
                   const HostBlobTensor** w, const HostBlobTensor** b) {
    auto iw = m.find(name + ".w"), ib = m.find(name + ".b");
    if (iw == m.end() || ib == m.end() || iw->second.dtype != 1 || ib->second.dtype != 0) {
        locr_fail(eng, "missing/ill-typed tensor", name.c_str());
        return false;
    }
    *w = &iw->second; *b = &ib->second;
    return true;
}

static bool make_conv(lumina_ocr* eng, const std::map<std::string, HostBlobTensor>& m, const std::string& name, int ks, int stride,
                      int cin_r, int cout_r, int cin_p, int cout_p, int act, ConvLayer* L, int bias_repeat = 1) {
    const HostBlobTensor *w, *b;
    if (!get_wb(eng, m, name, &w, &b)) return false;
    if (w->dims.size() != 4 || w->dims[0] != cout_r || w->dims[1] != ks || w->dims[3] != cin_r ||
        (int)b->dims[0] * bias_repeat != cout_r) {
        locr_fail(eng, "unexpected tensor shape", name.c_str());
        return false;
    }
    L->name = name; L->ks = ks; L->stride = stride; L->cin = cin_p; L->cout = cout_p; L->act = act;
    if (!conv_pick_cfg(ks, stride, cin_p, cout_p, &L->cfg)) { locr_fail(eng, "no conv kernel config", name.c_str()); return false; }
    const int taps = ks * ks;
    std::vector<bf16_t> padded((size_t)cout_p * taps * cin_p, 0);
    const bf16_t* src = reinterpret_cast<const bf16_t*>(w->data);
    for (int co = 0; co < cout_r; ++co)
        for (int t = 0; t < taps; ++t)
            memcpy(&padded[((size_t)co * taps + t) * cin_p], &src[((size_t)co * taps + t) * cin_r], sizeof(bf16_t) * cin_r);
    std::vector<bf16_t> packed(conv_packed_weight_elems(cout_p, ks, cin_p, L->cfg.bn));
    pack_conv_weights(padded.data(), cout_p, ks, cin_p, L->cfg.bn, L->cfg.ck, packed.data());
    L->wpk = static_cast<bf16_t*>(eng_upload(eng, packed.data(), packed.size() * sizeof(bf16_t)));
    static const int dma = getenv("LUMINA_CONV_DMA") != nullptr ? atoi(getenv("LUMINA_CONV_DMA")) : 1;
    if (ks == 3 && stride == 1 && L->cfg.bn == 64 && (cin_p >= 64 || name == "stem.conv3") && L->cfg.nw == 4) {
        L->cfg_big = L->cfg; L->cfg_big.nw = dma ? 6 : 5; L->cfg_big.ck = 16;
        std::vector<bf16_t> packed2(conv_packed_weight_elems(cout_p, ks, cin_p, 64));
        pack_conv_weights(padded.data(), cout_p, ks, cin_p, 64, 16, packed2.data(), dma ? 1 : 0);
        L->wpk_big = static_cast<bf16_t*>(eng_upload(eng, packed2.data(), packed2.size() * sizeof(bf16_t)));
    }
    const int ntiles = (cout_p + L->cfg.bn - 1) / L->cfg.bn;
    std::vector<float> bias((size_t)ntiles * L->cfg.bn, 0.f);
    const float* bs = reinterpret_cast<const float*>(b->data);
    const int bn_r = b->dims[0];
    for (int i = 0; i < cout_r; ++i) bias[i] = bs[i % bn_r];
    L->bias = static_cast<float*>(eng_upload(eng, bias.data(), bias.size() * sizeof(float)));
    if (!L->wpk || !L->bias) { locr_fail(eng, "device upload failed", name.c_str()); return false; }
    return true;
}

static inline float host_bf16_to_f32(bf16_t b) { uint32_t u = (uint32_t)b << 16; float f; memcpy(&f, &u, 4); return f; }
static inline bf16_t host_f32_to_bf16(float f) {
    uint32_t u; memcpy(&u, &f, 4);
    return (bf16_t)((u + 0x7fffu + ((u >> 16) & 1u)) >> 16);
}

static inline uint16_t bf16_bits_to(uint16_t b, int dtype) {
    if (!dtype) return b;
    uint32_t u = (uint32_t)b << 16;
    float f; memcpy(&f, &u, 4);
    const _Float16 hv = (_Float16)f;
    uint16_t o; memcpy(&o, &hv, 2);
    return o;
}

static int load_stem(lumina_ocr* eng, const std::map<std::string, HostBlobTensor>& m, const char* name, int cout, bf16_t** wpk, float** bias) {
    const HostBlobTensor *w, *b;
    if (!get_wb(eng, m, name, &w, &b)) return 1;
    if (w->dims.size() != 4 || w->dims[0] != cout || w->dims[1] != 3 || w->dims[2] != 3 || w->dims[3] != 3 || b->dims[0] != cout)
        return locr_fail(eng, name, "shape");
    bf16_t packed[2 * 2 * 32 * 8];
    pack_stem_weights(reinterpret_cast<const bf16_t*>(w->data), cout, packed);
    float padded[32] = {0};
    memcpy(padded, b->data, sizeof(float) * cout);
    *wpk = static_cast<bf16_t*>(eng_upload(eng, packed, sizeof(packed)));
    *bias = static_cast<float*>(eng_upload(eng, padded, sizeof(padded)));
    return *wpk && *bias ? 0 : locr_fail(eng, "upload", name);
}

static int load_ctc_head(lumina_ocr* eng, const std::map<std::string, HostBlobTensor>& m, const char* name, int K, int dtype, int* num_classes,
                         int* ntiles, bf16_t** wpk, float** bias) {
    auto w = m.find(std::string(name) + ".w"), b = m.find(std::string(name) + ".b");
    if (w == m.end() || b == m.end() || w->second.dims.size() != 2 || w->second.dims[1] != K || b->second.dims[0] != w->second.dims[0])
        return locr_fail(eng, name, "missing/shape");
    const int C = w->second.dims[0];
    *num_classes = C; *ntiles = (C + 63) / 64;
    std::vector<bf16_t> conv((size_t)C * K), packed(ctc_packed_weight_elems(C, K));
    const bf16_t* src = reinterpret_cast<const bf16_t*>(w->second.data);
    for (size_t i = 0; i < conv.size(); ++i) conv[i] = bf16_bits_to(src[i], dtype);
    pack_ctc_weights(conv.data(), C, K, packed.data());
    std::vector<float> padded((size_t)*ntiles * 64, -1.0e30f);
    memcpy(padded.data(), b->second.data, sizeof(float) * C);
    *wpk = static_cast<bf16_t*>(eng_upload(eng, packed.data(), packed.size() * sizeof(bf16_t)));
    *bias = static_cast<float*>(eng_upload(eng, padded.data(), padded.size() * sizeof(float)));
    return *wpk && *bias ? 0 : locr_fail(eng, "upload", name);
}

static int compose_fpn_p2(lumina_ocr* eng, const std::map<std::string, HostBlobTensor>& m) {
    const HostBlobTensor *wi, *bi, *wp, *bp;
    if (!get_wb(eng, m, "fpn.in2", &wi, &bi) || !get_wb(eng, m, "fpn.p2", &wp, &bp)) return 1;
    const float* b_in2 = reinterpret_cast<const float*>(bi->data);
    for (int i = 0; i < 256; ++i)
        if (b_in2[i] != 0.f) return 0;
    const bf16_t* Wi = reinterpret_cast<const bf16_t*>(wi->data);
    const bf16_t* Wp = reinterpret_cast<const bf16_t*>(wp->data);
    std::vector<bf16_t> w((size_t)64 * 9 * 320);
    std::vector<double> win((size_t)256 * 64);
    for (size_t i = 0; i < win.size(); ++i) win[i] = (double)host_bf16_to_f32(Wi[i]);
    for (int co = 0; co < 64; ++co)
        for (int t = 0; t < 9; ++t) {
            double acc[64] = {0};
            const bf16_t* row = Wp + ((size_t)co * 9 + t) * 256;
            for (int mm = 0; mm < 256; ++mm) {
                const double a = (double)host_bf16_to_f32(row[mm]);
                for (int ci = 0; ci < 64; ++ci) acc[ci] += a * win[(size_t)mm * 64 + ci];
            }
            bf16_t* dst = &w[((size_t)co * 9 + t) * 320];
            for (int ci = 0; ci < 64; ++ci) dst[ci] = host_f32_to_bf16((float)acc[ci]);
            memcpy(dst + 64, row, 256 * sizeof(bf16_t));
        }
    std::map<std::string, HostBlobTensor> mm;
    mm["fpn.p2c.w"] = HostBlobTensor{1, {64, 3, 3, 320}, reinterpret_cast<const uint8_t*>(w.data()), w.size() * sizeof(bf16_t)};
    mm["fpn.p2c.b"] = *bp;
    ConvLayer& L = eng->det["fpn.p2c"];
    if (!make_conv(eng, mm, "fpn.p2c", 3, 1, 320, 64, 320, 64, ACT_NONE, &L)) return 1;
    L.alg_flop_per_px = 2.0 * 64 * 256 + 2.0 * 9 * 256 * 64;
    return 0;
}

int eng_load_det(lumina_ocr* eng, const void* blob, size_t n) {
    std::map<std::string, HostBlobTensor> m;
    if (!parse_blob(eng, blob, n, &m)) return 1;
    LOCR_CHECK(hipSetDevice(eng->device));
    eng->det.clear();
    RUN(load_stem(eng, m, "stem.conv1", 32, &eng->stem_wpk, &eng->stem_bias));
    auto add = [&](const std::string& name, int ks, int stride, int cin, int cout, int act) -> bool {
        return make_conv(eng, m, name, ks, stride, cin, cout, cin, cout, act, &eng->det[name]);
    };
    if (!add("stem.conv2", 3, 1, 32, 32, ACT_RELU) || !add("stem.conv3", 3, 1, 32, 64, ACT_RELU)) return 1;
    const int chs[4] = {64, 128, 256, 512};
    int cin = 64;
    for (int i = 0; i < 4; ++i) {
        for (int j = 0; j < 2; ++j) {
            const std::string p = "s" + std::to_string(i) + ".b" + std::to_string(j);
            const int stride = (i > 0 && j == 0) ? 2 : 1;
            if (!add(p + ".conv0", 3, stride, cin, chs[i], ACT_RELU)) return 1;
            if (!add(p + ".conv1", 3, 1, chs[i], chs[i], ACT_RELU)) return 1;
            if (j == 0) {
                if (i == 0) { if (!add(p + ".short", 1, 1, cin, chs[i], ACT_NONE)) return 1; }
                else { if (!add(p + ".short", 2, 2, cin, chs[i], ACT_NONE)) return 1; }
            }
            cin = chs[i];
        }
    }
    for (int l = 5; l >= 2; --l) {
        if (!add("fpn.in" + std::to_string(l), 1, 1, chs[l - 2], 256, ACT_NONE)) return 1;
        if (!add("fpn.p" + std::to_string(l), 3, 1, 256, 64, ACT_NONE)) return 1;
    }
    if (!add("head.conv1", 3, 1, 256, 64, ACT_RELU)) return 1;
    if (compose_fpn_p2(eng, m)) return 1;
    {
        ConvLayer& L = eng->det["head.convt2"];
        if (!make_conv(eng, m, "head.convt2", 1, 1, 64, 256, 64, 256, ACT_RELU, &L, 4)) return 1;
        L.convt = true; L.convt_c = 64;
        ConvLayer& L3 = eng->det["head.convt3"];
        if (!make_conv(eng, m, "head.convt3", 1, 1, 64, 4, 64, 4, ACT_SIGMOID, &L3, 4)) return 1;
        L3.convt = true; L3.convt_c = 1;
        const HostBlobTensor *w3, *b3;
        if (!get_wb(eng, m, "head.convt3", &w3, &b3)) return 1;
        ConvLayer& Lf = eng->det["head.convt2.fused"];
        Lf = L;
        Lf.name = "head.convt2+3";
        {
            const bf16_t* w3s = reinterpret_cast<const bf16_t*>(w3->data);
            std::vector<bf16_t> img(4 * 2 * 32 * 8, 0);
            for (int ks = 0; ks < 4; ++ks)
                for (int hh = 0; hh < 2; ++hh)
                    for (int row = 0; row < 4; ++row)
                        for (int j = 0; j < 8; ++j) img[((ks * 2 + hh) * 32 + row) * 8 + j] = w3s[row * 64 + ks * 16 + hh * 8 + j];
            Lf.fuse_w = static_cast<bf16_t*>(eng_upload(eng, img.data(), img.size() * sizeof(bf16_t)));
        }
        Lf.fuse_b = reinterpret_cast<const float*>(b3->data)[0];
        if (!Lf.fuse_w) return locr_fail(eng, "upload", "head.convt3 fused weights");
    }
    eng->det_loaded = true;
    return 0;
}

static bool conv_takes_big(const lumina_ocr* eng, const ConvLayer& L, int n, int ho, int wo, bool flat) {
    static const bool no_big = getenv("LUMINA_CONV_NO_BIG") != nullptr;
    static const long long big_min_env = getenv("LUMINA_CONV_BIG_MIN") ? atoll(getenv("LUMINA_CONV_BIG_MIN")) : -1;
    const long long nb_eff = n > eng->det_sub_batch ? n : eng->det_sub_batch;
    const long long big_blocks = nb_eff * ((ho + 15) / 16) * ((wo + 31) / 32) * ((L.cout + L.cfg.bn - 1) / L.cfg.bn);
    const long long big_min = big_min_env >= 0 ? big_min_env : eng->conv_big_min;
    return !no_big && !flat && L.wpk_big != nullptr && big_blocks >= big_min;
}

struct LaunchTimer {
    lumina_ocr* eng; hipStream_t st; Event e0, e1;
    LaunchTimer(lumina_ocr* e, hipStream_t s, bool enabled = true) : eng(e), st(s) {
        if (!enabled || !e->time_convs) return;
        hipEvent_t a = nullptr, b = nullptr;
        if (hipEventCreate(&a) == hipSuccess) e0.reset(a);
        if (hipEventCreate(&b) == hipSuccess) e1.reset(b);
        if (!e0 || !e1 || hipEventRecord(e0.get(), st) != hipSuccess) { e0.reset(); e1.reset(); }
    }
    bool on() const { return e1 != nullptr; }
    void done(std::string layer, std::string kernel, double flop, double bytes) {
        if (!on() || hipEventRecord(e1.get(), st) != hipSuccess) return;
        eng->launches.push_back(LaunchRecord{std::move(e0), std::move(e1), flop, bytes, std::move(layer), std::move(kernel)});
    }
};

static int conv_params(lumina_ocr* eng, const ConvLayer& L, const Tensor4& x, const Tensor4& y, const ConvCall& c, ConvParams* out) {
    ConvParams p{};
    p.zeros = zero_block(eng);
    if (!p.zeros) return locr_fail(eng, "conv", "zero block upload failed");
    p.gate = c.gate; p.gate_hw = x.h * x.w;
    p.x = x.p; p.wpk = L.wpk; p.bias = L.bias; p.res = c.res ? c.res->p : nullptr; p.y = y.p;
    p.Cin = L.cin; p.Cout = L.cout; p.act = L.act;
    p.out_mode = c.out_mode; p.up_shift = c.up_shift; p.convt_c = L.convt_c;
    p.fuse_w = (c.out_mode == OUT_CONVT) ? L.fuse_w : nullptr; p.fuse_b = L.fuse_b;
    if (c.flat) {
        const long long m = (long long)x.n * x.h * x.w;
        p.N = 1; p.W = 32; p.H = (int)((m + 31) / 32); p.pix_limit = (int)m;
        p.Ho = p.H; p.Wo = 32;
        p.res_h = p.H; p.res_w = 32;
    } else {
        p.N = x.n; p.H = x.h; p.W = x.w; p.pix_limit = 0;
        p.Ho = (L.ks == 3) ? (x.h - 1) / L.stride + 1 : x.h / L.stride;
        p.Wo = (L.ks == 3) ? (x.w - 1) / L.stride + 1 : x.w / L.stride;
        if (c.res) { p.res_h = c.res->h; p.res_w = c.res->w; }
    }
    p.res_shift = c.res_shift;
    p.x_blk = x.blk; p.y_blk = y.blk; p.res_blk = c.res ? c.res->blk : 0;
    p.n_src = x.n_src;
    for (int k = 0; k < 4; ++k) {
        p.xs[k] = x.xs[k]; p.xs_shift[k] = x.xs_shift[k];
        p.xs_nchunk[k] = k < x.n_src ? x.src_c(k) / 16 : 0; p.xs_cstride[k] = k < x.n_src ? x.src_cs(k) : 0;
    }
    p.res_cstride = c.res ? c.res->c : 0;
    p.y_cstride = c.y_cstride ? c.y_cstride : y.c;
    p.y_coff = c.y_coff;
    if (const ConvLayer* s = c.short_l) {
        const Tensor4* sy = c.short_y;
        if (sy == nullptr || s->cin != L.cin || s->cout != L.cout || s->cfg.bn != L.cfg.bn || s->cfg.ck != L.cfg.ck || s->ks != 2 || s->stride != 2 ||
            sy->c != L.cout || sy->h != y.h || sy->w != y.w)
            return locr_fail(eng, "fused shortcut: layer mismatch", L.name.c_str());
        p.wpk2 = s->wpk; p.bias2 = s->bias; p.y2 = sy->p; p.y2_cstride = sy->c;
    }
    if (x.c != L.cin) return locr_fail(eng, "conv input channels mismatch", L.name.c_str());
    *out = p;
    return 0;
}

enum ConvKernel { CONV_TILE_8X32, CONV_TILE_16X32, CONV_POINTWISE, CONV_RING };
struct ConvChoice { ConvKernel kernel; ConvKernelCfg cfg; const bf16_t* wpk; };

static int conv_choose(lumina_ocr* eng, const ConvLayer& L, const ConvParams& p, const ConvCall& c, ConvChoice* out) {
    if (p.out_mode == OUT_POOL && (L.wpk_big == nullptr || L.cfg_big.nw != 6)) return locr_fail(eng, "fused max pool needs the LDS-DMA conv kernel", L.name.c_str());
    const bool forced = c.variant != 0 && L.wpk_big != nullptr;
    const bool big = forced || p.out_mode == OUT_POOL || p.n_src > 1 || conv_takes_big(eng, L, p.N, p.Ho, p.Wo, c.flat);
    if (forced && c.variant == 2 && !conv_ring_supported(L.cfg_big, p)) return locr_fail(eng, "conv2d_variant 2: the ring kernel does not take this layer", L.name.c_str());
    *out = big ? ConvChoice{CONV_TILE_16X32, L.cfg_big, L.wpk_big} : ConvChoice{CONV_TILE_8X32, L.cfg, L.wpk};
    static const bool no_pw = getenv("LUMINA_CONV_NO_PW") != nullptr;
    const bool ring_on = c.variant == 0 ? eng->conv_ring : c.variant == 2;
    if (!no_pw && !big && conv_pw_supported(out->cfg, p)) out->kernel = CONV_POINTWISE;
    else if (ring_on && big && conv_ring_supported(out->cfg, p)) out->kernel = CONV_RING;
    if (p.n_src > 1 && out->kernel != CONV_RING) return locr_fail(eng, "a multi-source input reached a kernel other than the ring kernel", L.name.c_str());
    if (out->kernel != CONV_RING && (p.x_blk || p.y_blk || p.res_blk)) return locr_fail(eng, "a channel-blocked tensor reached a kernel that cannot address it", L.name.c_str());
    return 0;
}

static hipError_t conv_dispatch(const lumina_ocr* eng, const ConvChoice& k, const ConvParams& p, hipStream_t st) {
    if (k.kernel == CONV_RING) return conv_ring_launch(p, eng->ring_orient, st);
    return k.kernel == CONV_POINTWISE ? conv_pw_launch(p, st) : conv_launch(k.cfg, p, st);
}

static void conv_account(const lumina_ocr* eng, const ConvLayer& L, const Tensor4& x, const ConvCall& c, const ConvParams& p, const ConvChoice& k, LaunchTimer* tm) {
    const ConvLayer* s = c.short_l;
    const double px = c.flat ? (double)p.pix_limit : (double)p.N * p.Ho * p.Wo;
    const double flop = (L.alg_flop_per_px > 0 ? px * L.alg_flop_per_px : 2.0 * px * L.ks * L.ks * L.cin * L.cout) + (s ? 2.0 * px * 4 * s->cin * s->cout : 0.0);
    double in_elems = (double)x.elems();
    if (x.n_src > 1) { in_elems = 0; for (int i = 0; i < x.n_src; ++i) in_elems += (double)x.n * (x.h >> x.xs_shift[i]) * (x.w >> x.xs_shift[i]) * x.src_c(i); }
    const double bytes = 2.0 * (in_elems + px * (c.out_mode == OUT_CONVT && p.fuse_w ? 4.0 : (double)L.cout) * (c.out_mode == OUT_UPSAMPLE ? (double)(1 << (2 * c.up_shift)) : (c.out_mode == OUT_POOL ? 0.25 : 1.0)) + (c.res ? px * (double)L.cout / (double)(1 << (2 * c.res_shift)) : 0.0) + (double)L.ks * L.ks * L.cin * L.cout +
                                (s ? px * (double)s->cout + 4.0 * s->cin * s->cout : 0.0));
    std::string kname = k.kernel == CONV_POINTWISE ? (L.cin == 64 ? "conv_pw_kernel<64>" : "conv_pw_kernel<128>") : conv_kernel_name(k.cfg);
    if (k.kernel == CONV_RING) kname = conv_ring_kernel_name(p, eng->ring_orient);
    if (s) { const size_t pos = kname.rfind(",0,2>"); if (pos != std::string::npos) kname.replace(pos, 5, ",5,2>"); }
    if (c.out_mode == OUT_POOL && k.kernel != CONV_RING) { const size_t pos = kname.rfind(",3,4>"); if (pos != std::string::npos) kname.replace(pos, 5, ",4,4>"); }
    tm->done(s ? L.name + "+short" : L.name, kname, flop, bytes);
}

int eng_run_conv(lumina_ocr* eng, const ConvLayer& L, const Tensor4& x, Tensor4* y, hipStream_t st, const ConvCall& c) {
    ConvParams p;
    RUN(conv_params(eng, L, x, *y, c, &p));
    if (x.p == nullptr || y->p == nullptr) return ws_null(eng, L.name.c_str());
    LaunchTimer tm(eng, st);
    ConvChoice k;
    RUN(conv_choose(eng, L, p, c, &k));
    p.wpk = k.wpk;
    hipError_t e = conv_dispatch(eng, k, p, st);
    if (e != hipSuccess) return locr_fail(eng, L.name.c_str(), hipGetErrorString(e));
    if (tm.on()) conv_account(eng, L, x, c, p, k, &tm);
    return 0;
}

static void tap(lumina_ocr* eng, const char* name, const Tensor4& t) { if (eng->keep_taps && t.p) eng->taps[name] = t; }

static int run_stem(lumina_ocr* eng, const char* name, const uint8_t* x, const int* widths, int N, int H, int W, const bf16_t* wpk, const float* bias,
                    int act, const float scale[3], const float shift[3], const Tensor4& y, hipStream_t st, const ConvLayer* conv2 = nullptr) {
    if (eng->arena.counting() || y.p == nullptr) return 0;
    StemParams sp{};
    sp.x = x; sp.wpk = wpk; sp.bias = bias; sp.y = y.p; sp.valid_w_per_img = widths;
    sp.N = N; sp.H = H; sp.W = W; sp.valid_h = H; sp.valid_w = W; sp.Ho = y.h; sp.Wo = y.w; sp.Cout_store = y.c;
    sp.act = act;
    for (int c = 0; c < 3; ++c) { sp.scale[c] = scale[c]; sp.shift[c] = shift[c]; }
    hipError_t e = conv2 ? stem12_launch(sp, conv2->wpk, conv2->bias, st) : stem_conv_launch(sp, st);
    return e == hipSuccess ? 0 : locr_fail(eng, name, hipGetErrorString(e));
}
static const float STEM_SCALE_PM1[3] = {2.0f / 255.0f, 2.0f / 255.0f, 2.0f / 255.0f}, STEM_SHIFT_PM1[3] = {-1.0f, -1.0f, -1.0f};

static int det_forward_sub(lumina_ocr* eng, const uint8_t* pages, int B, int H, int W, int Hp, int Wp, bf16_t* prob, hipStream_t st) {
    const bool dry = eng->arena.counting();
    auto& D = eng->det;
    ConvLayer& c2 = D["stem.conv2"];
    const bool fuse_stem = eng->fuse_stem && eng->keep_taps != 1 && c2.cfg.bn == 32 && c2.cfg.ck == 16 && c2.act == ACT_RELU;
    Tensor4 t1{};
    if (!fuse_stem || dry) t1 = ws_tensor(eng, B, Hp / 2, Wp / 2, 32);
    Tensor4 t2 = ws_tensor(eng, B, Hp / 2, Wp / 2, 32);
    {
        const float mean[3] = {0.485f, 0.456f, 0.406f}, stdv[3] = {0.229f, 0.224f, 0.225f};
        float scale[3], shift[3];
        for (int c = 0; c < 3; ++c) { scale[c] = 1.0f / (255.0f * stdv[c]); shift[c] = -mean[c] / stdv[c]; }
        RUN(run_stem(eng, "stem.conv1", pages, nullptr, B, H, W, eng->stem_wpk, eng->stem_bias, ACT_RELU, scale, shift, fuse_stem ? t2 : t1, st, fuse_stem ? &c2 : nullptr));
    }
    if (!fuse_stem) {
        tap(eng, "stem.conv1", t1);
        RUN(eng_run_conv(eng, c2, t1, &t2, st)); tap(eng, "stem.conv2", t2);
    }
    const bool fuse_pool = eng->fuse_pool && eng->keep_taps != 1;
    Tensor4 t3{};
    if (!fuse_pool || dry) t3 = ws_tensor(eng, B, Hp / 2, Wp / 2, 64);
    Tensor4 x = ws_tensor(eng, B, Hp / 4, Wp / 4, 64);
    if (fuse_pool) {
        RUN(eng_run_conv(eng, D["stem.conv3"], t2, &x, st, ConvCall().mode(OUT_POOL)));
    } else {
        RUN(eng_run_conv(eng, D["stem.conv3"], t2, &t3, st)); tap(eng, "stem.conv3", t3);
        if (!dry && x.p) {
            hipError_t e = maxpool_launch(t3.p, x.p, B, t3.h, t3.w, 64, 3, 2, 1, x.h, x.w, st);
            if (e != hipSuccess) return locr_fail(eng, "stem.pool", hipGetErrorString(e));
        }
    }
    tap(eng, "stem.pool", x);
    const int chs[4] = {64, 128, 256, 512};
    Tensor4 feats[4];
    for (int i = 0; i < 4; ++i) {
        for (int j = 0; j < 2; ++j) {
            const std::string p = "s" + std::to_string(i) + ".b" + std::to_string(j);
            const int stride = (i > 0 && j == 0) ? 2 : 1;
            Tensor4 y = ws_tensor(eng, B, x.h / stride, x.w / stride, chs[i]);
            const bool blk = i == 0 && eng->blocked_layout && eng->keep_taps == 0 && eng->conv_ring && !dry &&
                             conv_takes_big(eng, D[p + ".conv0"], B, x.h, x.w, false) && conv_takes_big(eng, D[p + ".conv1"], B, x.h, x.w, false);
            y.blk = blk;
            const ConvLayer& c0 = D[p + ".conv0"];
            const bool fuse_sc = eng->fuse_short && i > 0 && j == 0 && x.h % 2 == 0 && x.w % 2 == 0 && c0.cfg.bn == 64 && c0.cfg.ck == 16 && c0.cfg.nw == 4 &&
                                 D[p + ".short"].cfg.bn == 64 && D[p + ".short"].cfg.ck == 16;
            Tensor4 sc = x;
            if (j == 0) sc = ws_tensor(eng, B, y.h, y.w, chs[i]);
            if (fuse_sc) {
                RUN(eng_run_conv(eng, c0, x, &y, st, ConvCall().shortcut(&D[p + ".short"], &sc)));
            } else {
                RUN(eng_run_conv(eng, c0, x, &y, st));
                if (j == 0) RUN(eng_run_conv(eng, D[p + ".short"], x, &sc, st, ConvCall().flat_gemm(i == 0)));
            }
            Tensor4 o = ws_tensor(eng, B, y.h, y.w, chs[i]);
            o.blk = blk && j == 0;
            RUN(eng_run_conv(eng, D[p + ".conv1"], y, &o, st, ConvCall().residual(&sc)));
            tap(eng, p.c_str(), o);
            x = o;
        }
        feats[i] = x;
    }
    Tensor4 in5 = ws_tensor(eng, B, feats[3].h, feats[3].w, 256);
    RUN(eng_run_conv(eng, D["fpn.in5"], feats[3], &in5, st));
    Tensor4 out4 = ws_tensor(eng, B, feats[2].h, feats[2].w, 256);
    RUN(eng_run_conv(eng, D["fpn.in4"], feats[2], &out4, st, ConvCall().residual(&in5, 1)));
    Tensor4 out3 = ws_tensor(eng, B, feats[1].h, feats[1].w, 256);
    RUN(eng_run_conv(eng, D["fpn.in3"], feats[1], &out3, st, ConvCall().residual(&out4, 1)));
    ConvLayer& hc1 = D["head.conv1"];
    const bool multi = eng->fpn_multi && eng->keep_taps != 1 && eng->conv_ring && conv_takes_big(eng, hc1, B, Hp / 4, Wp / 4, false) &&
                       (Hp / 4) % 8 == 0 && (Wp / 4) % 8 == 0;
    auto slice = [](const Tensor4& t, int b0, int nb) {
        Tensor4 r = t;
        r.n = nb;
        if (t.p) r.p = t.p + (size_t)b0 * t.h * t.w * t.c;
        return r;
    };
    const bool compose = eng->fpn_compose && eng->conv_ring && D.count("fpn.p2c") != 0;
    auto run_p2 = [&](const Tensor4& c2, const Tensor4& o3, Tensor4* lateral, Tensor4* dst, int y_cstride, int y_coff) -> int {
        if (compose) {
            Tensor4 in = c2;
            in.c = 320; in.n_src = 2;
            in.xs[0] = c2.p; in.xs[1] = o3.p; in.p = o3.p;
            in.xs_shift[0] = 0; in.xs_shift[1] = 1; in.xs_c[0] = 64; in.xs_c[1] = 256;
            return eng_run_conv(eng, D["fpn.p2c"], in, dst, st, ConvCall().channel_slice(y_cstride, y_coff));
        }
        RUN(eng_run_conv(eng, D["fpn.in2"], c2, lateral, st, ConvCall().residual(&o3, 1)));
        return eng_run_conv(eng, D["fpn.p2"], *lateral, dst, st, ConvCall().channel_slice(y_cstride, y_coff));
    };
    auto head_tail = [&](const Tensor4& h1, bf16_t* prob_g, int nb) -> int {
        Tensor4 pm; pm.p = dry ? nullptr : prob_g; pm.n = nb; pm.h = Hp; pm.w = Wp; pm.c = 1;
        if (eng->fuse_head && eng->keep_taps != 1)
            return eng_run_conv(eng, D["head.convt2.fused"], h1, &pm, st, ConvCall().mode(OUT_CONVT));
        Tensor4 h2 = ws_tensor(eng, nb, Hp / 2, Wp / 2, 64);
        RUN(eng_run_conv(eng, D["head.convt2"], h1, &h2, st, ConvCall().mode(OUT_CONVT))); tap(eng, "head.convt2", h2);
        return eng_run_conv(eng, D["head.convt3"], h2, &pm, st, ConvCall().mode(OUT_CONVT1));
    };
    if (multi) {
        Tensor4 p5 = ws_tensor(eng, B, in5.h, in5.w, 64), p4 = ws_tensor(eng, B, out4.h, out4.w, 64), p3 = ws_tensor(eng, B, out3.h, out3.w, 64);
        RUN(eng_run_conv(eng, D["fpn.p5"], in5, &p5, st)); tap(eng, "fpn.p5", p5);
        RUN(eng_run_conv(eng, D["fpn.p4"], out4, &p4, st)); tap(eng, "fpn.p4", p4);
        RUN(eng_run_conv(eng, D["fpn.p3"], out3, &p3, st)); tap(eng, "fpn.p3", p3);
        const int G = (eng->keep_taps == 0 && eng->tail_group > 0 && B > eng->tail_group) ? eng->tail_group : B;
        Tensor4 out2{};
        if (!compose) out2 = ws_tensor(eng, G, feats[0].h, feats[0].w, 256);
        Tensor4 p2 = ws_tensor(eng, G, feats[0].h, feats[0].w, 64);
        Tensor4 h1 = ws_tensor(eng, G, Hp / 4, Wp / 4, 64);
        for (int g0 = 0; g0 < B; g0 += G) {
            const int nb = B - g0 < G ? B - g0 : G;
            Tensor4 o2 = slice(out2, 0, nb), p2g = slice(p2, 0, nb), h1g = slice(h1, 0, nb), o3 = slice(out3, g0, nb);
            RUN(run_p2(slice(feats[0], g0, nb), o3, &o2, &p2g, 0, 0));
            tap(eng, "fpn.p2", p2g);
            Tensor4 cat = p2g;
            cat.c = 256; cat.n_src = 4;
            cat.xs[0] = slice(p5, g0, nb).p; cat.xs[1] = slice(p4, g0, nb).p; cat.xs[2] = slice(p3, g0, nb).p; cat.xs[3] = p2g.p;
            cat.xs_shift[0] = 3; cat.xs_shift[1] = 2; cat.xs_shift[2] = 1; cat.xs_shift[3] = 0;
            RUN(eng_run_conv(eng, hc1, cat, &h1g, st)); tap(eng, "head.conv1", h1g);
            RUN(head_tail(h1g, prob ? prob + (size_t)g0 * Hp * Wp : nullptr, nb));
        }
        return 0;
    }
    Tensor4 out2{};
    if (!compose) out2 = ws_tensor(eng, B, feats[0].h, feats[0].w, 256);
    Tensor4 fuse = ws_tensor(eng, B, Hp / 4, Wp / 4, 256);
    RUN(eng_run_conv(eng, D["fpn.p5"], in5, &fuse, st, ConvCall().upsample(3).channel_slice(256, 0)));
    RUN(eng_run_conv(eng, D["fpn.p4"], out4, &fuse, st, ConvCall().upsample(2).channel_slice(256, 64)));
    RUN(eng_run_conv(eng, D["fpn.p3"], out3, &fuse, st, ConvCall().upsample(1).channel_slice(256, 128)));
    RUN(run_p2(feats[0], out3, &out2, &fuse, 256, 192));
    tap(eng, "fpn.fuse", fuse);
    Tensor4 h1 = ws_tensor(eng, B, Hp / 4, Wp / 4, 64);
    RUN(eng_run_conv(eng, hc1, fuse, &h1, st)); tap(eng, "head.conv1", h1);
    return head_tail(h1, prob, B);
}

template <class Run> static int forward_sub_batched(lumina_ocr* eng, int n, int sb, Run&& run) {
    eng->arena = Arena();
    RUN(run(0, sb));
    RUN(eng_ws_reserve(eng, eng->arena.off + 4096));
    eng->taps.clear();
    for (int b0 = 0; b0 < n; b0 += sb) {
        eng->arena = Arena(eng->ws.get(), eng->ws.cap);
        RUN(run(b0, n - b0 < sb ? n - b0 : sb));
        if (eng->arena.overflow) return ws_null(eng, "forward");
    }
    return 0;
}

int eng_det_forward(lumina_ocr* eng, const uint8_t* pages, int B, int H, int W, int Hp, int Wp, bf16_t* prob, hipStream_t st) {
    if (!eng->det_loaded) return locr_fail(eng, "det_forward", "det weights not loaded");
    if (Hp % 32 || Wp % 32 || Hp < H || Wp < W || B <= 0) return locr_fail(eng, "det_forward", "Hp/Wp must be multiples of 32 and >= H/W");
    LOCR_CHECK(hipSetDevice(eng->device));
    return forward_sub_batched(eng, B, eng->det_sub_batch < B ? eng->det_sub_batch : B, [&](int b0, int nb) {
        return det_forward_sub(eng, pages + (size_t)b0 * H * W * 3, nb, H, W, Hp, Wp, prob + (size_t)b0 * Hp * Wp, st);
    });
}

static inline int cp16(int c) { return rup(c, 16); }
static int make_div(double v, int d = 8) {
    int nv = (int)(v + d / 2.0) / d * d;
    if (nv < d) nv = d;
    if (nv < 0.9 * v) nv += d;
    return nv;
}

static bool make_dw(lumina_ocr* eng, const std::map<std::string, HostBlobTensor>& m, const std::string& name, int k, int c_r, int c_p, DwLayer* L) {
    const HostBlobTensor *w, *b;
    if (!get_wb(eng, m, name, &w, &b)) return false;
    if (w->dims.size() != 4 || w->dims[0] != c_r || w->dims[1] != k || w->dims[3] != 1) { locr_fail(eng, "dw shape", name.c_str()); return false; }
    std::vector<bf16_t> wt((size_t)k * k * c_p, 0);
    const bf16_t* src = reinterpret_cast<const bf16_t*>(w->data);
    for (int c = 0; c < c_r; ++c)
        for (int t = 0; t < k * k; ++t) wt[(size_t)t * c_p + c] = src[(size_t)c * k * k + t];
    std::vector<float> bias(c_p, 0.f);
    memcpy(bias.data(), b->data, sizeof(float) * c_r);
    L->k = k; L->c = c_p;
    L->w = static_cast<bf16_t*>(eng_upload(eng, wt.data(), wt.size() * sizeof(bf16_t)));
    L->bias = static_cast<float*>(eng_upload(eng, bias.data(), bias.size() * sizeof(float)));
    return L->w && L->bias;
}

static bool make_se(lumina_ocr* eng, const std::map<std::string, HostBlobTensor>& m, const std::string& pfx, int c_r, int c_p, int mid, SeLayer* L) {
    const HostBlobTensor *w1, *b1, *w2, *b2;
    if (!get_wb(eng, m, pfx + ".se1", &w1, &b1) || !get_wb(eng, m, pfx + ".se2", &w2, &b2)) return false;
    if (w1->dims[0] != mid || w1->dims[3] != c_r || w2->dims[0] != c_r || w2->dims[3] != mid) { locr_fail(eng, "se shape", pfx.c_str()); return false; }
    std::vector<bf16_t> a((size_t)mid * c_p, 0), bmat((size_t)c_p * mid, 0);
    const bf16_t* s1 = reinterpret_cast<const bf16_t*>(w1->data);
    const bf16_t* s2 = reinterpret_cast<const bf16_t*>(w2->data);
    for (int i = 0; i < mid; ++i) memcpy(&a[(size_t)i * c_p], &s1[(size_t)i * c_r], sizeof(bf16_t) * c_r);
    memcpy(bmat.data(), s2, sizeof(bf16_t) * (size_t)c_r * mid);
    std::vector<float> bb2(c_p, 0.f);
    memcpy(bb2.data(), b2->data, sizeof(float) * c_r);
    L->c = c_p; L->mid = mid;
    L->w1 = static_cast<bf16_t*>(eng_upload(eng, a.data(), a.size() * sizeof(bf16_t)));
    L->w2 = static_cast<bf16_t*>(eng_upload(eng, bmat.data(), bmat.size() * sizeof(bf16_t)));
    L->b1 = static_cast<float*>(eng_upload(eng, b1->data, sizeof(float) * mid));
    L->b2 = static_cast<float*>(eng_upload(eng, bb2.data(), bb2.size() * sizeof(float)));
    return L->w1 && L->w2 && L->b1 && L->b2;
}

static int load_mv3_blocks(lumina_ocr* eng, const std::map<std::string, HostBlobTensor>& m, const std::string& prefix, double scale, const int* sh,
                           int cin, std::vector<RecBlock>* blocks) {
    struct Row { int k, exp, c; bool se; int act; };
    static const Row rows[11] = {{3, 16, 16, true, ACT_RELU},    {3, 72, 24, false, ACT_RELU},   {3, 88, 24, false, ACT_RELU},
                                 {5, 96, 40, true, ACT_HSWISH},  {5, 240, 40, true, ACT_HSWISH}, {5, 240, 40, true, ACT_HSWISH},
                                 {5, 120, 48, true, ACT_HSWISH}, {5, 144, 48, true, ACT_HSWISH}, {5, 288, 96, true, ACT_HSWISH},
                                 {5, 576, 96, true, ACT_HSWISH}, {5, 576, 96, true, ACT_HSWISH}};
    blocks->clear();
    blocks->resize(11);
    for (int i = 0; i < 11; ++i) {
        RecBlock& B = (*blocks)[i];
        B.k = rows[i].k; B.cin = cin; B.exp = make_div(rows[i].exp * scale); B.cout = make_div(rows[i].c * scale);
        B.se = rows[i].se; B.se_mid = B.exp / 4; B.stride_h = sh[i]; B.act = rows[i].act;
        B.res = (B.stride_h == 1 && B.cin == B.cout);
        const std::string p = prefix + ".b" + std::to_string(i);
        if (!make_conv(eng, m, p + ".expand", 1, 1, B.cin, B.exp, cp16(B.cin), cp16(B.exp), B.act, &B.expand)) return 1;
        if (!make_dw(eng, m, p + ".dw", B.k, B.exp, cp16(B.exp), &B.dw)) return locr_fail(eng, "dw", p.c_str());
        {
            const HostBlobTensor *w, *b;
            if (!get_wb(eng, m, p + ".expand", &w, &b)) return 1;
            const int ec = cp16(B.exp), cc = cp16(B.cin);
            std::vector<bf16_t> padded((size_t)ec * cc, 0), packed(mbconv_expand_packed_elems(ec, cc));
            const bf16_t* src = reinterpret_cast<const bf16_t*>(w->data);
            for (int r = 0; r < B.exp; ++r) memcpy(&padded[(size_t)r * cc], &src[(size_t)r * B.cin], sizeof(bf16_t) * B.cin);
            mbconv_pack_expand(padded.data(), ec, cc, packed.data());
            std::vector<float> bias((size_t)((ec + 31) / 32) * 32, 0.f);
            memcpy(bias.data(), b->data, sizeof(float) * B.exp);
            B.we_pk = static_cast<bf16_t*>(eng_upload(eng, packed.data(), packed.size() * sizeof(bf16_t)));
            B.be_pk = static_cast<float*>(eng_upload(eng, bias.data(), bias.size() * sizeof(float)));
            if (!B.we_pk || !B.be_pk) return locr_fail(eng, "upload", (p + ".expand (fused)").c_str());
        }
        if (B.se && !make_se(eng, m, p, B.exp, cp16(B.exp), B.se_mid, &B.sel)) return 1;
        if (!make_conv(eng, m, p + ".project", 1, 1, B.exp, B.cout, cp16(B.exp), cp16(B.cout), ACT_NONE, &B.project)) return 1;
        cin = B.cout;
    }
    return 0;
}

int eng_load_rec(lumina_ocr* eng, const void* blob, size_t n) {
    std::map<std::string, HostBlobTensor> m;
    if (!parse_blob(eng, blob, n, &m)) return 1;
    LOCR_CHECK(hipSetDevice(eng->device));
    const double scale = 0.5;
    const int c0 = make_div(16 * scale);
    RUN(load_stem(eng, m, "rec.conv1", c0, &eng->rstem_wpk, &eng->rstem_bias));
    static const int sh[11] = {1, 2, 1, 2, 1, 1, 1, 1, 2, 1, 1};
    if (load_mv3_blocks(eng, m, "rec", scale, sh, c0, &eng->rblocks)) return 1;
    const int cin = eng->rblocks.back().cout;
    if (!make_conv(eng, m, "rec.conv2", 1, 1, cin, 288, cp16(cin), 288, ACT_HSWISH, &eng->rconv2)) return 1;
    const int Hh = 96;
    for (int l = 0; l < 2; ++l) {
        const int din = l == 0 ? 288 : 2 * Hh;
        const std::string pf = "lstm.l" + std::to_string(l) + ".fw", pb = "lstm.l" + std::to_string(l) + ".bw";
        auto wf = m.find(pf + ".w_ih"), wb = m.find(pb + ".w_ih"), bf = m.find(pf + ".b"), bb = m.find(pb + ".b");
        auto hf = m.find(pf + ".w_hh"), hb = m.find(pb + ".w_hh");
        if (wf == m.end() || wb == m.end() || bf == m.end() || bb == m.end() || hf == m.end() || hb == m.end())
            return locr_fail(eng, "lstm tensors missing", pf.c_str());
        if (wf->second.dims[0] != 4 * Hh || wf->second.dims[1] != din || hf->second.dims[1] != Hh) return locr_fail(eng, "lstm shape", pf.c_str());
        std::vector<uint8_t> wcat(wf->second.nbytes + wb->second.nbytes), bcat(bf->second.nbytes + bb->second.nbytes);
        memcpy(wcat.data(), wf->second.data, wf->second.nbytes); memcpy(wcat.data() + wf->second.nbytes, wb->second.data, wb->second.nbytes);
        memcpy(bcat.data(), bf->second.data, bf->second.nbytes); memcpy(bcat.data() + bf->second.nbytes, bb->second.data, bb->second.nbytes);
        std::map<std::string, HostBlobTensor> mm;
        mm["x.w"] = HostBlobTensor{1, {8 * Hh, 1, 1, din}, wcat.data(), wcat.size()};
        mm["x.b"] = HostBlobTensor{0, {8 * Hh}, bcat.data(), bcat.size()};
        if (!make_conv(eng, mm, "x", 1, 1, din, 8 * Hh, din, 8 * Hh, ACT_NONE, &eng->xproj[l])) return 1;
        eng->xproj[l].name = "lstm.l" + std::to_string(l) + ".xproj";
        std::vector<uint8_t> hcat(hf->second.nbytes + hb->second.nbytes);
        memcpy(hcat.data(), hf->second.data, hf->second.nbytes); memcpy(hcat.data() + hf->second.nbytes, hb->second.data, hb->second.nbytes);
        eng->whh[l] = static_cast<bf16_t*>(eng_upload(eng, hcat.data(), hcat.size()));
        if (!eng->whh[l]) return locr_fail(eng, "upload", "whh");
    }
    RUN(load_ctc_head(eng, m, "ctc.fc", 2 * Hh, 0, &eng->num_classes, &eng->ctc_ntiles, &eng->ctc_wpk, &eng->ctc_bias));
    eng->rec_loaded = true;
    return 0;
}

#define LAUNCH(name, expr)                                                                                        \
    do {                                                                                                          \
        if (!dry) {                                                                                               \
            if (eng->arena.overflow) return ws_null(eng, name);                                                   \
            hipError_t _e = (expr); if (_e != hipSuccess) return locr_fail(eng, name, hipGetErrorString(_e));     \
        }                                                                                                         \
    } while (0)

static int run_mv3_block(lumina_ocr* eng, const RecBlock& B, const std::string& name, Tensor4* x, hipStream_t st) {
    const bool dry = eng->arena.counting();
    const int N = x->n;
    const int ho = (x->h + 2 * (B.k / 2) - B.k) / B.stride_h + 1;
    MbParams mp{};
    mp.we = B.we_pk; mp.be = B.be_pk; mp.wd = B.dw.w; mp.bd = B.dw.bias;
    mp.N = N; mp.H = x->h; mp.W = x->w; mp.cin = x->c; mp.expc = cp16(B.exp); mp.Ho = ho; mp.act = B.act;
    const bool fused_mb = eng->fuse_mb && mbconv_supported(mp, B.k, B.stride_h);
    Tensor4 e1{};
    if (!fused_mb || dry) e1 = ws_tensor(eng, N, x->h, x->w, cp16(B.exp));
    Tensor4 d = ws_tensor(eng, N, ho, x->w, cp16(B.exp));
    float* pool = B.se ? eng->arena.take<float>((size_t)N * mb_strips(x->w) * d.c) : nullptr;
    if (fused_mb) {
        mp.x = x->p; mp.d = d.p; mp.pool = pool;
        if (!dry && x->p && d.p) {
            LaunchTimer tm(eng, st);
            LAUNCH("mbconv", mbconv_launch(mp, B.k, B.stride_h, st));
            const double opx = (double)N * ho * x->w, ipx = (double)N * x->h * x->w;
            tm.done(name + ".expand+dw", "mbconv_kernel<" + std::to_string(B.k) + "," + std::to_string(B.stride_h) + "," + std::to_string(B.act) + ">",
                    2.0 * ipx * x->c * mp.expc + 2.0 * opx * B.k * B.k * mp.expc, 2.0 * (ipx * x->c + opx * mp.expc));
        }
    } else {
        RUN(eng_run_conv(eng, B.expand, *x, &e1, st, ConvCall().flat_gemm()));
        LAUNCH("dwconv", dwconv_launch(e1.p, B.dw.w, B.dw.bias, d.p, N, e1.h, e1.w, e1.c, B.k, B.stride_h, B.act, st));
        if (B.se) LAUNCH("se_pool", se_pool_launch(d.p, pool, N, d.h, d.w, d.c, st));
    }
    const bf16_t* se_gate_ptr = nullptr;
    if (B.se) {
        bf16_t* gate = eng->arena.take<bf16_t>((size_t)N * d.c);
        LAUNCH("se_fc", se_fc_launch(pool, mb_strips(d.w), B.sel.w1, B.sel.b1, B.sel.w2, B.sel.b2, gate, N, d.h * d.w, d.c, B.sel.mid, st));
        se_gate_ptr = gate;
    }
    Tensor4 o = ws_tensor(eng, N, d.h, d.w, cp16(B.cout));
    RUN(eng_run_conv(eng, B.project, d, &o, st, ConvCall().flat_gemm().residual(B.res ? x : nullptr).gated(se_gate_ptr)));
    tap(eng, name.c_str(), o);
    *x = o;
    return 0;
}
// ... 292 lines not shown
```

### ocr-system_amd/csrc/stem_conv.hip

```cpp
#include "stem_conv.h"

namespace {

constexpr int TH = 8, TW = 32;
constexpr int HH = 2 * (TH - 1) + 3, HW = 2 * (TW - 1) + 3;
constexpr int ROW = HW * 3 + 1;
constexpr int STAGE_PITCH = 32 * 2 + 16;

template <int NHH, int NHW, int NROW>
__device__ __forceinline__ void fill_halo_u8(bf16_t* halo, const StemParams& p, int n_img, int iy0, int ix0, int vh, int vw, int tid) {
    constexpr int SEG = NHW * 3, WPR = (SEG + 3) / 4 + 1, NIT = (NHH * WPR + 255) / 256;
    static_assert(NROW > SEG, "one dump element per row");
    const long long img_off = (long long)n_img * p.H * p.W * 3, all_bytes = (long long)p.N * p.H * p.W * 3;
    const unsigned char* xal = p.x + (img_off & ~3ll);
    const int mis = (int)(img_off & 3);
    const long long lo64 = -(img_off & ~3ll), hi64 = all_bytes - (img_off & ~3ll);
    const int lo_lim = lo64 < -0x7fffffffll ? -0x7fffffff : (int)lo64, hi_lim = hi64 > 0x7fffffffll ? 0x7fffffff : (int)hi64;
    const float sc0 = p.scale[0], sc1 = p.scale[1], sc2 = p.scale[2], sh0 = p.shift[0], sh1 = p.shift[1], sh2 = p.shift[2];
    uint32_t word[NIT];
    int e0s[NIT];
#pragma unroll
    for (int u = 0; u < NIT; ++u) {
        const int i = tid + 256 * u;
        const int hy = i / WPR, wi = i - hy * WPR, iy = iy0 + hy;
        const int q = mis + (iy * p.W + ix0) * 3;
        const int w0 = (q & ~3) + 4 * wi;
        e0s[u] = w0 - q;
        const bool ld = i < NHH * WPR && iy >= 0 && iy < vh && w0 >= lo_lim && w0 + 4 <= hi_lim;
        const uint32_t wv = *reinterpret_cast<const uint32_t*>(xal + (ld ? w0 : 0));
        word[u] = ld ? wv : 0u;
    }
    if (hi_lim & 3) {
#pragma unroll 1
        for (int u = 0; u < NIT; ++u) {
            const int i = tid + 256 * u;
            const int hy = i / WPR, wi = i - hy * WPR, iy = iy0 + hy;
            const int q = mis + (iy * p.W + ix0) * 3, w0 = (q & ~3) + 4 * wi;
            if (i < NHH * WPR && iy >= 0 && iy < vh && w0 >= lo_lim && w0 < hi_lim && w0 + 4 > hi_lim) {
                uint32_t wv = 0;
                for (int b = 0; b < 4; ++b) if (w0 + b < hi_lim) wv |= (uint32_t)xal[w0 + b] << (8 * b);
#pragma unroll
                for (int uu = 0; uu < NIT; ++uu) if (uu == u) word[uu] = wv;
            }
        }
    }
#pragma unroll
    for (int u = 0; u < NIT; ++u) {
        const int i = tid + 256 * u;
        const int hy = min(i / WPR, NHH - 1), iy = iy0 + hy;
        const bool rowin = iy >= 0 && iy < vh, item = i < NHH * WPR;
        const int e0 = e0s[u];
        const int hx0 = (e0 + 3) / 3 - 1, c0 = e0 - hx0 * 3;
        bf16_t* hrow = halo + hy * NROW;
        float S[4], T[4];
        S[0] = c0 == 0 ? sc0 : (c0 == 1 ? sc1 : sc2); S[1] = c0 == 0 ? sc1 : (c0 == 1 ? sc2 : sc0); S[2] = c0 == 0 ? sc2 : (c0 == 1 ? sc0 : sc1); S[3] = S[0];
        T[0] = c0 == 0 ? sh0 : (c0 == 1 ? sh1 : sh2); T[1] = c0 == 0 ? sh1 : (c0 == 1 ? sh2 : sh0); T[2] = c0 == 0 ? sh2 : (c0 == 1 ? sh0 : sh1); T[3] = T[0];
#pragma unroll
        for (int b = 0; b < 4; ++b) {
            const int e = e0 + b;
            const int ix = ix0 + hx0 + ((c0 + b >= 3) ? 1 : 0);
            float v = (float)((word[u] >> (8 * b)) & 0xffu) * S[b];
            v = v + T[b];
            const uint32_t keep = (rowin && (unsigned)ix < (unsigned)vw) ? 0xffffu : 0u;
            const int idx = (item && (unsigned)e < (unsigned)SEG) ? e : SEG;
            hrow[idx] = (bf16_t)(f32_to_bf16(v) & keep);
        }
    }
}

template <int NROW>
__device__ __forceinline__ void stem_koff(int h, int (&koff)[2][8]) {
#pragma unroll
    for (int ks = 0; ks < 2; ++ks)
#pragma unroll
        for (int j = 0; j < 8; ++j) {
            const int k = ks * 16 + h * 8 + j, kh = k / 9;
            koff[ks][j] = k < 27 ? kh * NROW + (k - kh * 9) : 0;
        }
}

__global__ __launch_bounds__(256) void stem_conv_kernel(const StemParams p) {
    __shared__ __attribute__((aligned(16))) unsigned char smem[256 * STAGE_PITCH > HH * ROW * 2 ? 256 * STAGE_PITCH : HH * ROW * 2];
    bf16_t* halo = reinterpret_cast<bf16_t*>(smem);

    const int tid = threadIdx.x, lane = tid & 63, wave = tid >> 6, r = lane & 31, h = lane >> 5;
    const int tiles_x = (p.Wo + TW - 1) / TW, tiles_y = (p.Ho + TH - 1) / TH;
    const int bid = blockIdx.x;
    const int n_img = bid / (tiles_x * tiles_y);
    const int trem = bid - n_img * tiles_x * tiles_y;
    const int tile_y = trem / tiles_x, tile_x = trem - tile_y * tiles_x;
    const int vw = p.valid_w_per_img ? p.valid_w_per_img[n_img] : p.valid_w;
    const int vh = p.valid_h;

    const int iy0 = tile_y * TH * 2 - 1, ix0 = tile_x * TW * 2 - 1;
    fill_halo_u8<HH, HW, ROW>(halo, p, n_img, iy0, ix0, vh, vw, tid);
    __syncthreads();

    f32x16_t acc[2];
#pragma unroll
    for (int mt = 0; mt < 2; ++mt)
#pragma unroll
        for (int j = 0; j < 16; ++j) acc[mt][j] = 0.f;
    int koff[2][8];
    stem_koff<ROW>(h, koff);
#pragma unroll
    for (int ks = 0; ks < 2; ++ks) {
        const bf16x8_t afr = *reinterpret_cast<const bf16x8_t*>(p.wpk + ((ks * 2 + h) * 32 + r) * 8);
#pragma unroll
        for (int mt = 0; mt < 2; ++mt) {
            const bf16_t* hb = halo + (2 * (wave * 2 + mt)) * ROW + 6 * r;
            union { bf16x8_t v; bf16_t s[8]; } b;
#pragma unroll
            for (int j = 0; j < 8; ++j) b.s[j] = hb[koff[ks][j]];
            acc[mt] = __builtin_amdgcn_mfma_f32_32x32x16_bf16(afr, b.v, acc[mt], 0, 0, 0);
        }
    }
    __syncthreads();

    unsigned char* stage = smem;
#pragma unroll
    for (int mt = 0; mt < 2; ++mt)
#pragma unroll
        for (int g = 0; g < 4; ++g) {
            const float4 b4 = *reinterpret_cast<const float4*>(p.bias + 8 * g + 4 * h);
            acc[mt][4 * g + 0] += b4.x; acc[mt][4 * g + 1] += b4.y; acc[mt][4 * g + 2] += b4.z; acc[mt][4 * g + 3] += b4.w;
        }
#define STEM_ALL(expr) _Pragma("unroll") for (int mt = 0; mt < 2; ++mt) _Pragma("unroll") for (int j = 0; j < 16; ++j) { const float v = acc[mt][j]; acc[mt][j] = (expr); }
    if (p.act == ACT_RELU) { STEM_ALL(fmaxf(v, 0.f)) }
    else if (p.act == ACT_HSWISH) { STEM_ALL(v * fminf(fmaxf(v + 3.f, 0.f), 6.f) * (1.f / 6.f)) }
    else if (p.act != ACT_NONE) { STEM_ALL(apply_act(v, p.act)) }
#undef STEM_ALL
#pragma unroll
    for (int mt = 0; mt < 2; ++mt) {
        const int tp = (wave * 2 + mt) * TW + r;
#pragma unroll
        for (int g = 0; g < 4; ++g) {
            uint2 o;
            o.x = pack_bf16x2(acc[mt][4 * g + 0], acc[mt][4 * g + 1]);
            o.y = pack_bf16x2(acc[mt][4 * g + 2], acc[mt][4 * g + 3]);
            *reinterpret_cast<uint2*>(stage + tp * STAGE_PITCH + (8 * g + 4 * h) * 2) = o;
        }
    }
    __syncthreads();
    const int cpp = p.Cout_store / 8;
    for (int i = tid; i < 256 * cpp; i += 256) {
        const int tp = i / cpp, ch = i - tp * cpp;
        const int ty = tp / TW, tx = tp - ty * TW;
        const int oy = tile_y * TH + ty, ox = tile_x * TW + tx;
        if (oy >= p.Ho || ox >= p.Wo) continue;
        const uint4 v = *reinterpret_cast<const uint4*>(stage + tp * STAGE_PITCH + ch * 16);
        *reinterpret_cast<uint4*>(p.y + (((size_t)n_img * p.Ho + oy) * p.Wo + ox) * p.Cout_store + ch * 8) = v;
    }
}

constexpr int F_T1H = TH + 2, F_T1W = TW + 2, F_T1PX = F_T1H * F_T1W;
constexpr int F_HH = 2 * (F_T1H - 1) + 3, F_HW = 2 * (F_T1W - 1) + 3;
constexpr int F_ROW = F_HW * 3 + 1;
constexpr int F_HALO_BYTES = F_HH * F_ROW * 2, F_T1_BYTES = ((F_T1PX + 31) / 32) * 32 * 64;
__global__ __launch_bounds__(256) void stem12_kernel(const StemParams p, const bf16_t* w2pk, const float* bias2) {
    static_assert(256 * STAGE_PITCH <= F_T1_BYTES, "the output stage re-uses the t1 tile");
    __shared__ __attribute__((aligned(16))) unsigned char smem[F_HALO_BYTES + F_T1_BYTES];
    bf16_t* halo = reinterpret_cast<bf16_t*>(smem);
    unsigned char* t1 = smem + F_HALO_BYTES;
    const int tid = threadIdx.x, lane = tid & 63, wave = tid >> 6, r = lane & 31, h = lane >> 5;
    const int tiles_x = (p.Wo + TW - 1) / TW, tiles_y = (p.Ho + TH - 1) / TH;
    const int bid = blockIdx.x;
    const int n_img = bid / (tiles_x * tiles_y);
    const int trem = bid - n_img * tiles_x * tiles_y;
    const int tile_y = trem / tiles_x, tile_x = trem - tile_y * tiles_x;
    const int vw = p.valid_w, vh = p.valid_h;

    const int y1_0 = tile_y * TH - 1, x1_0 = tile_x * TW - 1;
    const int iy0 = 2 * y1_0 - 1, ix0 = 2 * x1_0 - 1;
    fill_halo_u8<F_HH, F_HW, F_ROW>(halo, p, n_img, iy0, ix0, vh, vw, tid);
    __syncthreads();

    {
        bf16x8_t a1[2];
#pragma unroll
        for (int ks = 0; ks < 2; ++ks) a1[ks] = *reinterpret_cast<const bf16x8_t*>(p.wpk + ((ks * 2 + h) * 32 + r) * 8);
        float4 b1[4];
#pragma unroll
        for (int g = 0; g < 4; ++g) b1[g] = *reinterpret_cast<const float4*>(p.bias + 8 * g + 4 * h);
        int koff[2][8];
        stem_koff<F_ROW>(h, koff);
        for (int tile = wave; tile * 32 < F_T1PX; tile += 4) {
            const int pidx = tile * 32 + r;
            const int pc = min(pidx, F_T1PX - 1);
            const int py = pc / F_T1W, px = pc - py * F_T1W;
            const bf16_t* hb = halo + (2 * py) * F_ROW + 6 * px;
            f32x16_t acc;
#pragma unroll
            for (int j = 0; j < 16; ++j) acc[j] = 0.f;
#pragma unroll
            for (int ks = 0; ks < 2; ++ks) {
                union { bf16x8_t v; bf16_t s[8]; } b;
#pragma unroll
                for (int j = 0; j < 8; ++j) b.s[j] = hb[koff[ks][j]];
                acc = __builtin_amdgcn_mfma_f32_32x32x16_bf16(a1[ks], b.v, acc, 0, 0, 0);
            }
            const int y1 = y1_0 + py, x1 = x1_0 + px;
            const bool inimg = y1 >= 0 && y1 < p.Ho && x1 >= 0 && x1 < p.Wo;
            if (pidx < F_T1PX) {
                const int swz = (pidx >> 2) & 3;
#pragma unroll
                for (int g = 0; g < 4; ++g) {
                    uint2 o = make_uint2(0, 0);
                    if (inimg) {
                        o.x = pack_bf16x2(fmaxf(acc[4 * g + 0] + b1[g].x, 0.f), fmaxf(acc[4 * g + 1] + b1[g].y, 0.f));
                        o.y = pack_bf16x2(fmaxf(acc[4 * g + 2] + b1[g].z, 0.f), fmaxf(acc[4 * g + 3] + b1[g].w, 0.f));
                    }
                    *reinterpret_cast<uint2*>(t1 + pidx * 64 + ((g ^ swz) * 16) + 8 * h) = o;
                }
            }
        }
    }
    bf16x8_t w2[9];
#pragma unroll
    for (int tap = 0; tap < 9; ++tap) w2[tap] = *reinterpret_cast<const bf16x8_t*>(w2pk + ((size_t)h * (9 * 32) + tap * 32 + r) * 8);
    __syncthreads();

    f32x16_t acc2[2];
#pragma unroll
    for (int mt = 0; mt < 2; ++mt)
#pragma unroll
        for (int j = 0; j < 16; ++j) acc2[mt][j] = 0.f;
#pragma unroll
    for (int kc = 0; kc < 2; ++kc) {
#pragma unroll
        for (int tap = 0; tap < 9; ++tap) {
#pragma unroll
            for (int mt = 0; mt < 2; ++mt) {
                const int pp = (wave * 2 + mt + tap / 3) * F_T1W + r + tap % 3;
                const bf16x8_t bf = *reinterpret_cast<const bf16x8_t*>(t1 + pp * 64 + (((2 * kc + h) ^ ((pp >> 2) & 3)) * 16));
                acc2[mt] = __builtin_amdgcn_mfma_f32_32x32x16_bf16(w2[tap], bf, acc2[mt], 0, 0, 0);
            }
        }
        if (kc == 0) {
#pragma unroll
            for (int tap = 0; tap < 9; ++tap) w2[tap] = *reinterpret_cast<const bf16x8_t*>(w2pk + ((size_t)(2 + h) * (9 * 32) + tap * 32 + r) * 8);
        }
    }
    __syncthreads();

    unsigned char* stage = t1;
#pragma unroll
    for (int mt = 0; mt < 2; ++mt) {
        const int tp = (wave * 2 + mt) * TW + r;
#pragma unroll
        for (int g = 0; g < 4; ++g) {
            const float4 b4 = *reinterpret_cast<const float4*>(bias2 + 8 * g + 4 * h);
            uint2 o;
            o.x = pack_bf16x2(apply_act(acc2[mt][4 * g + 0] + b4.x, ACT_RELU), apply_act(acc2[mt][4 * g + 1] + b4.y, ACT_RELU));
            o.y = pack_bf16x2(apply_act(acc2[mt][4 * g + 2] + b4.z, ACT_RELU), apply_act(acc2[mt][4 * g + 3] + b4.w, ACT_RELU));
            *reinterpret_cast<uint2*>(stage + tp * STAGE_PITCH + (8 * g + 4 * h) * 2) = o;
        }
    }
    __syncthreads();
    for (int i = tid; i < 256 * 4; i += 256) {
        const int tp = i >> 2, ch = i & 3;
        const int ty = tp / TW, tx = tp - ty * TW;
        const int oy = tile_y * TH + ty, ox = tile_x * TW + tx;
        if (oy >= p.Ho || ox >= p.Wo) continue;
        *reinterpret_cast<uint4*>(p.y + (((size_t)n_img * p.Ho + oy) * p.Wo + ox) * 32 + ch * 8) = *reinterpret_cast<const uint4*>(stage + tp * STAGE_PITCH + ch * 16);
    }
}

__global__ void normalize_kernel(const uint8_t* x, bf16_t* y, int N, int H, int W, int Hp, int Wp, int vh, int vw,
                                 float s0, float s1, float s2, float b0, float b1, float b2, int nchw) {
    const size_t total = (size_t)N * Hp * Wp;
    for (size_t i = (size_t)blockIdx.x * blockDim.x + threadIdx.x; i < total; i += (size_t)gridDim.x * blockDim.x) {
        const int xx = (int)(i % Wp);
        const size_t t = i / Wp;
        const int yy = (int)(t % Hp), n = (int)(t / Hp);
        float v[3] = {0.f, 0.f, 0.f};
        if (yy < vh && xx < vw) {
            const uint8_t* s = x + (((size_t)n * H + yy) * W + xx) * 3;
            v[0] = (float)s[0] * s0; v[0] = v[0] + b0;
            v[1] = (float)s[1] * s1; v[1] = v[1] + b1;
            v[2] = (float)s[2] * s2; v[2] = v[2] + b2;
        }
        if (nchw) {
            const size_t plane = (size_t)Hp * Wp;
            bf16_t* d = y + (size_t)n * 3 * plane + (size_t)yy * Wp + xx;
            d[0] = f32_to_bf16(v[0]); d[plane] = f32_to_bf16(v[1]); d[2 * plane] = f32_to_bf16(v[2]);
        } else {
            bf16_t* d = y + i * 3;
            d[0] = f32_to_bf16(v[0]); d[1] = f32_to_bf16(v[1]); d[2] = f32_to_bf16(v[2]);
        }
    }
}

}

void pack_stem_weights(const bf16_t* ohwi, int cout, bf16_t* out ) {
    for (int ks = 0; ks < 2; ++ks)
        for (int h = 0; h < 2; ++h)
            for (int co = 0; co < 32; ++co)
                for (int j = 0; j < 8; ++j) {
                    const int k = ks * 16 + h * 8 + j;
                    out[((ks * 2 + h) * 32 + co) * 8 + j] = (co < cout && k < 27) ? ohwi[co * 27 + k] : (bf16_t)0;
                }
}

hipError_t stem_conv_launch(const StemParams& p, hipStream_t stream) {
    const int tiles_x = (p.Wo + TW - 1) / TW, tiles_y = (p.Ho + TH - 1) / TH;
    hipLaunchKernelGGL(stem_conv_kernel, dim3(p.N * tiles_x * tiles_y), dim3(256), 0, stream, p);
    return hipGetLastError();
}

hipError_t stem12_launch(const StemParams& p, const bf16_t* w2pk, const float* bias2, hipStream_t stream) {
    if (p.valid_w_per_img != nullptr || p.Cout_store != 32 || p.act != ACT_RELU) return hipErrorInvalidValue;
    const int tiles_x = (p.Wo + TW - 1) / TW, tiles_y = (p.Ho + TH - 1) / TH;
    hipLaunchKernelGGL(stem12_kernel, dim3(p.N * tiles_x * tiles_y), dim3(256), 0, stream, p, w2pk, bias2);
    return hipGetLastError();
}

hipError_t normalize_launch(const uint8_t* x, bf16_t* y, int N, int H, int W, int Hp, int Wp, int vh, int vw,
                            const float* scale, const float* shift, int nchw, hipStream_t stream) {
    const size_t total = (size_t)N * Hp * Wp;
    int grid = (int)((total + 255) / 256);
    if (grid > 256 * 16) grid = 256 * 16;
    hipLaunchKernelGGL(normalize_kernel, dim3(grid), dim3(256), 0, stream, x, y, N, H, W, Hp, Wp, vh, vw, scale[0], scale[1],
                       scale[2], shift[0], shift[1], shift[2], nchw);
    return hipGetLastError();
}
```

### ocr-system_amd/lumina_ocr/engine.py

```python
from __future__ import annotations

import ctypes
import os
from pathlib import Path
from typing import Dict, Optional, Tuple

import numpy as np

from . import arch

_LIB_PATH = Path(__file__).resolve().parent.parent / "lib" / "liblumina_ocr.so"

REC_H, REC_W, REC_T = 32, 320, 80
MAX_WORDS = 40
MAX_BOXES = 1000


class EngineUnavailable(RuntimeError):
    pass


class EngineError(RuntimeError):
    pass


_lib = None


def load_library() -> ctypes.CDLL:
    global _lib
    if _lib is not None:
        return _lib
    path = Path(os.environ.get("LUMINA_OCR_LIB", str(_LIB_PATH)))
    if not path.exists():
        raise EngineUnavailable(f"{path} not found: build it with `make -C ocr-system_amd` (hipcc, gfx950)")
    lib = ctypes.CDLL(str(path))
    c = ctypes
    vp, i32, f32, sz = c.c_void_p, c.c_int, c.c_float, c.c_size_t
    sig = {
        "lumina_ocr_create": (i32, [i32, c.POINTER(vp)]),
        "lumina_ocr_destroy": (None, [vp]),
        "lumina_ocr_last_error": (c.c_char_p, [vp]),
        "lumina_ocr_version": (c.c_char_p, []),
        "lumina_ocr_set_option": (i32, [vp, c.c_char_p, i32]),
        "lumina_ocr_load_det_weights": (i32, [vp, vp, sz]),
        "lumina_ocr_load_rec_weights": (i32, [vp, vp, sz]),
        "lumina_ocr_num_classes": (i32, [vp]),
        "lumina_ocr_normalize": (i32, [vp, vp, i32, i32, i32, i32, i32, c.POINTER(f32), c.POINTER(f32), i32, vp, vp]),
        "lumina_ocr_det_forward": (i32, [vp, vp, i32, i32, i32, i32, i32, vp, vp]),
        "lumina_ocr_det_postprocess": (i32, [vp, vp, i32, i32, i32, i32, i32, f32, f32, f32, i32, i32, vp, vp, vp, vp]),
        "lumina_ocr_rec_crop": (i32, [vp, vp, i32, i32, i32, vp, vp, i32, vp, vp, vp]),
        "lumina_ocr_rec_crop_oriented": (i32, [vp, vp, i32, i32, i32, vp, vp, i32, vp, vp, vp, vp]),
        "lumina_ocr_cls_crop": (i32, [vp, vp, i32, i32, i32, vp, vp, i32, vp, vp, vp]),
        "lumina_ocr_load_cls_weights": (i32, [vp, vp, sz]),
        "lumina_ocr_cls_forward": (i32, [vp, vp, vp, i32, f32, vp, vp, vp, vp]),
        "lumina_ocr_rec_forward": (i32, [vp, vp, vp, i32, vp, vp, vp]),
        "lumina_ocr_ctc_decode": (i32, [vp, vp, vp, i32, vp, vp, vp, vp]),
        "lumina_ocr_ctc_decode_words": (i32, [vp, vp, vp, i32, vp, vp, vp, i32, vp, vp, vp, vp, vp, vp, vp, vp]),
        "lumina_ocr_conv2d": (i32, [vp, vp, i32, i32, i32, i32, vp, vp, i32, i32, i32, i32, vp, vp, vp]),
        "lumina_ocr_read_tap": (i32, [vp, c.c_char_p, vp, sz, c.POINTER(i32)]),
        "lumina_ocr_conv_timing": (i32, [vp, c.POINTER(c.c_double), c.POINTER(c.c_double), c.POINTER(i32)]),
        "lumina_ocr_conv_timing_detail": (i32, [vp, c.c_char_p, sz]),
        "lumina_ocr_resize_lanczos": (i32, [vp, vp, i32, i32, i32, i32, vp, i32, i32, vp]),
        "lumina_ocr_enhance": (i32, [vp, vp, i32, i32, i32, f32, f32, vp, vp, vp]),
        "lumina_ocr_jpeg_encode": (i32, [vp, vp, i32, i32, i32, i32, i32, vp, sz, vp, vp]),
        "lumina_ocr_jpeg_probe": (i32, [vp, sz, vp]),
        "lumina_ocr_jpeg_last_passes": (i32, [vp]),
        "lumina_ocr_jpeg_decode_async": (i32, [vp, vp, vp, i32, i32, i32, vp, vp, i32, vp]),
        "lumina_ocr_jpeg_decode": (i32, [vp, vp, vp, i32, i32, i32, vp, vp, vp]),
        "lumina_ocr_jpeg_coefficients": (i32, [vp, vp, i32, i32, i32, i32, vp, vp]),
        "lumina_ocr_png_probe": (i32, [vp, sz, vp]),
        "lumina_ocr_png_decode": (i32, [vp, vp, vp, i32, i32, i32, vp, vp, vp]),
        "lumina_ocr_flate_image_decode": (i32, [vp, vp, vp, i32, i32, i32, vp, vp, vp, vp, vp]),
        "lumina_ocr_ccitt_decode": (i32, [vp, vp, vp, i32, i32, i32, vp, vp, vp, vp]),
        "lumina_ocr_fax_decode": (i32, [vp, vp, vp, i32, i32, i32, vp, vp, vp, vp]),
        "lumina_ocr_strip_image_decode": (i32, [vp, vp, vp, i32, vp, i32, i32, i32, i32, vp, vp, vp, vp, vp]),
        "lumina_ocr_load_svtr_weights": (i32, [vp, vp, sz]),
        "lumina_ocr_svtr_forward": (i32, [vp, vp, vp, i32, vp, vp, vp]),
        "lumina_ocr_svtr_num_classes": (i32, [vp]),
        "lumina_ocr_svtr_dtype": (i32, [vp]),
        "lumina_ocr_binarize": (i32, [vp, vp, i32, i32, i32, i32, i32, vp, vp]),
        "lumina_ocr_grayscale": (i32, [vp, vp, i32, i32, i32, vp, vp]),
        "lumina_ocr_exif_transpose": (i32, [vp, vp, i32, i32, i32, i32, vp, vp]),
        "lumina_ocr_denoise": (i32, [vp, vp, i32, i32, i32, vp, vp]),
        "lumina_ocr_deskew": (i32, [vp, vp, i32, i32, i32, vp, vp, vp, vp, vp, vp, vp]),
        "lumina_ocr_deskew_warp": (i32, [vp, vp, i32, i32, i32, vp, vp, vp]),
        "lumina_ocr_table_rules": (i32, [vp, vp, i32, i32, i32, i32, i32, i32, i32, i32, vp, vp, vp, vp, vp]),
        "lumina_ocr_selection_marks": (i32, [vp, vp, i32, i32, i32, i32, i32, i32, i32, vp, vp, vp, vp]),
        "lumina_ocr_barcodes": (i32, [vp, vp, i32, i32, i32, i32, i32, i32, i32, i32, i32, vp, vp, vp, vp, vp, vp]),
        "lumina_ocr_barcodes_kinds": (i32, [vp, vp, i32, i32, i32, i32, i32, i32, i32, i32, i32, vp, vp, vp, vp, vp, vp, i32]),
        "lumina_ocr_qrcodes": (i32, [vp, vp, i32, i32, i32] + [i32] * 9 + [vp] * 7),
        "lumina_ocr_qrcodes_versions": (i32, [vp, vp, i32, i32, i32] + [i32] * 10 + [vp] * 7),
        "lumina_ocr_datamatrix": (i32, [vp, vp, i32, i32, i32] + [i32] * 8 + [vp] * 7),
        "lumina_ocr_aztec": (i32, [vp, vp, i32, i32, i32] + [i32] * 9 + [vp] * 7),
        "lumina_ocr_aztec_layers": (i32, [vp, vp, i32, i32, i32] + [i32] * 10 + [vp] * 7),
        "lumina_ocr_rules_and_marks": (i32, [vp, vp, i32, i32, i32, i32, i32, i32, i32, i32, vp, vp, vp, i32, i32, i32, vp, vp, vp]),
        "lumina_ocr_selection_marks_round": (i32, [vp, vp, i32, i32, i32, i32, i32, i32, i32, vp, vp, vp, i32, i32, i32, i32, vp, vp, vp]),
        "lumina_ocr_rules_and_marks_round": (i32, [vp, vp, i32, i32, i32, i32, i32, i32, i32, i32, vp, vp, vp, i32, i32, i32, vp, vp,
                                                   i32, i32, i32, i32, vp, vp, vp]),
        "lumina_ocr_page_quarter_workspace_bytes": (sz, [i32, i32, i32]),
        "lumina_ocr_aztec_workspace_bytes": (sz, [i32, i32, i32, i32, i32]),
        "lumina_ocr_aztec_layers_workspace_bytes": (sz, [i32, i32, i32, i32, i32]),
        "lumina_ocr_page_quarter": (i32, [vp, vp, i32, i32, i32, i32, i32, vp, vp, vp]),
        "lumina_ocr_page_turn": (i32, [vp, vp, i32, i32, i32, vp, i32, i32, vp, vp]),
        "lumina_ocr_page_vote": (i32, [vp, vp, vp, i32, i32, vp, vp]),
    }
    missing = []
    for name, (res, args) in sig.items():
        try:
            fn = getattr(lib, name)
        except AttributeError:
            missing.append(name)
            continue
        fn.restype = res
        fn.argtypes = args
    lib._missing = missing
    _lib = lib
    return lib


EXPORTED_SYMBOLS = [
    "lumina_ocr_create", "lumina_ocr_destroy", "lumina_ocr_last_error", "lumina_ocr_version", "lumina_ocr_set_option",
    "lumina_ocr_load_det_weights", "lumina_ocr_load_rec_weights", "lumina_ocr_num_classes", "lumina_ocr_normalize",
    "lumina_ocr_det_forward", "lumina_ocr_det_postprocess", "lumina_ocr_rec_crop", "lumina_ocr_rec_crop_oriented", "lumina_ocr_cls_crop",
    "lumina_ocr_load_cls_weights", "lumina_ocr_cls_forward", "lumina_ocr_rec_forward",
    "lumina_ocr_ctc_decode", "lumina_ocr_ctc_decode_words", "lumina_ocr_conv2d", "lumina_ocr_read_tap", "lumina_ocr_conv_timing", "lumina_ocr_conv_timing_detail",
    "lumina_ocr_resize_lanczos", "lumina_ocr_enhance", "lumina_ocr_jpeg_encode", "lumina_ocr_jpeg_coefficients", "lumina_ocr_jpeg_probe", "lumina_ocr_jpeg_decode", "lumina_ocr_jpeg_decode_async", "lumina_ocr_jpeg_last_passes",
    "lumina_ocr_png_probe", "lumina_ocr_png_decode", "lumina_ocr_flate_image_decode", "lumina_ocr_ccitt_decode", "lumina_ocr_fax_decode", "lumina_ocr_strip_image_decode",
    "lumina_ocr_load_svtr_weights", "lumina_ocr_svtr_forward", "lumina_ocr_svtr_num_classes", "lumina_ocr_svtr_dtype", "lumina_ocr_binarize", "lumina_ocr_exif_transpose", "lumina_ocr_grayscale", "lumina_ocr_denoise", "lumina_ocr_deskew", "lumina_ocr_deskew_warp",
    "lumina_ocr_table_rules", "lumina_ocr_selection_marks", "lumina_ocr_rules_and_marks", "lumina_ocr_selection_marks_round",
    "lumina_ocr_rules_and_marks_round", "lumina_ocr_barcodes", "lumina_ocr_barcodes_kinds", "lumina_ocr_qrcodes", "lumina_ocr_qrcodes_versions", "lumina_ocr_datamatrix", "lumina_ocr_aztec", "lumina_ocr_aztec_workspace_bytes", "lumina_ocr_aztec_layers", "lumina_ocr_aztec_layers_workspace_bytes",
    "lumina_ocr_page_quarter_workspace_bytes", "lumina_ocr_page_quarter", "lumina_ocr_page_turn", "lumina_ocr_page_vote",
]


def _torch():
    import torch
    return torch


def _ptr(t) -> int:
    return 0 if t is None else t.data_ptr()


class Engine:

    def __init__(self, device: int = 0):
        torch = _torch()
        if not torch.cuda.is_available():
            raise EngineUnavailable("no ROCm device visible to torch (torch.cuda.is_available() is False)")
        self.lib = load_library()
        self.device = device
        torch.cuda.set_device(device)
        h = ctypes.c_void_p()
        rc = self.lib.lumina_ocr_create(device, ctypes.byref(h))
        self._h = h
        if rc != 0:
            msg = self.lib.lumina_ocr_last_error(h).decode() if h else "create failed"
            raise EngineUnavailable(msg)
        self.num_classes = self.svtr_num_classes = 0
        self.det_loaded = self.rec_loaded = self.svtr_loaded = self.cls_loaded = False

    def close(self):
        if getattr(self, "_h", None):
            self.lib.lumina_ocr_destroy(self._h)
            self._h = None

    def __del__(self):
        try:
            self.close()
        except Exception:
            pass

    def _chk(self, rc: int):
        if rc != 0:
            raise EngineError(self.lib.lumina_ocr_last_error(self._h).decode())

    def _stream(self) -> int:
        return _torch().cuda.current_stream().cuda_stream

    def jpeg_encode(self, pages, quality: int = 95, max_bytes: int = 2 * 1024 * 1024, optimize: bool = True):
        torch = _torch()
        n, h, w, c = pages.shape
        assert c == 3 and pages.dtype == torch.uint8
        stride = (int(max_bytes) + 1023) // 1024 * 1024
        out = torch.empty((n, stride), dtype=torch.uint8, device=pages.device)
        sizes = torch.empty((n,), dtype=torch.int32, device=pages.device)
        self._chk(self.lib.lumina_ocr_jpeg_encode(self._h, _ptr(pages), n, h, w, int(quality), int(bool(optimize)), _ptr(out), stride, _ptr(sizes),
                                                  self._stream()))
        return out, sizes

    @staticmethod
    def jpeg_probe(data: bytes):
        lib = load_library()
        info = (ctypes.c_int * 6)()
        buf = ctypes.c_char_p(data)
        rc = lib.lumina_ocr_jpeg_probe(buf, len(data), info)
        return rc, dict(width=info[0], height=info[1], ncomp=info[2], h=info[3], v=info[4], restart=info[5])

    def jpeg_decode(self, files, height: int, width: int, out=None):
        torch = _torch()
        n = len(files)
        if out is None:
            out = torch.empty((n, height, width, 3), dtype=torch.uint8, device=torch.device("cuda", self.device))
        ptrs = (ctypes.c_char_p * n)(*files)
        sizes = (ctypes.c_size_t * n)(*[len(f) for f in files])
        status = (ctypes.c_int * n)()
        self._chk(self.lib.lumina_ocr_jpeg_decode(self._h, ptrs, sizes, n, int(height), int(width), _ptr(out), status, self._stream()))
        return out, list(status)

    def jpeg_decode_async(self, files, height: int, width: int, out=None, passes: int = 12):
        torch = _torch()
        n = len(files)
        if out is None:
            out = torch.empty((n, height, width, 3), dtype=torch.uint8, device=torch.device("cuda", self.device))
        status = torch.zeros((n,), dtype=torch.int32).pin_memory()
        ptrs = (ctypes.c_char_p * n)(*files)
        sizes = (ctypes.c_size_t * n)(*[len(f) for f in files])
        self._chk(self.lib.lumina_ocr_jpeg_decode_async(self._h, ptrs, sizes, n, int(height), int(width), _ptr(out), status.data_ptr(), int(passes), self._stream()))
        return out, status

    @staticmethod
    def png_probe(data: bytes):
        lib = load_library()
        info = (ctypes.c_int * 8)()
        rc = lib.lumina_ocr_png_probe(ctypes.c_char_p(data), len(data), info)
        return rc, dict(width=info[0], height=info[1], color_type=info[2], bit_depth=info[3], interlace=info[4], palette_size=info[5],
                        orientation=info[6])

    def png_decode(self, files, height: int, width: int, out=None):
        torch = _torch()
        n = len(files)
        if out is None:
            out = torch.empty((n, height, width, 3), dtype=torch.uint8, device=torch.device("cuda", self.device))
        ptrs = (ctypes.c_char_p * n)(*files)
        sizes = (ctypes.c_size_t * n)(*[len(f) for f in files])
        status = (ctypes.c_int * n)()
        self._chk(self.lib.lumina_ocr_png_decode(self._h, ptrs, sizes, n, int(height), int(width), _ptr(out), status, self._stream()))
        return out, list(status)

    def _stream_batch(self, streams, height: int, width: int, out):
        torch = _torch()
        n = len(streams)
        if out is None:
            out = torch.empty((n, height, width, 3), dtype=torch.uint8, device=torch.device("cuda", self.device))
        streams = [s if isinstance(s, bytes) else bytes(s) for s in streams]
        ptrs = (ctypes.c_char_p * n)(*streams)
        sizes = (ctypes.c_size_t * n)(*[len(s) for s in streams])
        return n, out, streams, ptrs, sizes, (ctypes.c_int * n)()

    def flate_image_decode(self, streams, height: int, width: int, params, palettes=None, out=None):
        n, out, streams, ptrs, sizes, status = self._stream_batch(streams, height, width, out)
        flat = (ctypes.c_int32 * (5 * n))(*[int(v) for p in params for v in p])
        pals = None
        if palettes is not None and any(p is not None for p in palettes):
            keep = [None if p is None else bytes(p) for p in palettes]
            assert all(p is None or len(p) == 768 for p in keep)
            pals = (ctypes.c_char_p * n)(*keep)
        self._chk(self.lib.lumina_ocr_flate_image_decode(self._h, ptrs, sizes, n, int(height), int(width), flat, pals, _ptr(out), status, self._stream()))
        return out, list(status)

    def ccitt_decode(self, streams, rows: int, columns: int, params, out=None):
        n, out, streams, ptrs, sizes, status = self._stream_batch(streams, rows, columns, out)
        flat = (ctypes.c_int32 * (4 * n))(*[int(v) for p in params for v in p])
        self._chk(self.lib.lumina_ocr_ccitt_decode(self._h, ptrs, sizes, n, int(rows), int(columns), flat, _ptr(out), status, self._stream()))
        return out, list(status)

    def fax_decode(self, streams, rows: int, columns: int, params, out=None):
        n, out, streams, ptrs, sizes, status = self._stream_batch(streams, rows, columns, out)
        flat = (ctypes.c_int32 * (5 * n))(*[int(v) for p in params for v in p])
        assert len(flat) == 5 * n
        self._chk(self.lib.lumina_ocr_fax_decode(self._h, ptrs, sizes, n, int(rows), int(columns), flat, _ptr(out), status, self._stream()))
        return out, list(status)

    def strip_image_decode(self, pages, height: int, width: int, rows_per_strip: int, params, palettes=None, out=None):
        torch = _torch()
        n = len(pages)
        if out is None:
            out = torch.empty((n, height, width, 3), dtype=torch.uint8, device=torch.device("cuda", self.device))
        strips = [s if isinstance(s, bytes) else bytes(s) for p in pages for s in p]
        m = len(strips)
        ptrs = (ctypes.c_char_p * max(m, 1))(*strips)
        sizes = (ctypes.c_size_t * max(m, 1))(*[len(s) for s in strips])
        counts = (ctypes.c_int32 * n)(*[len(p) for p in pages])
        flat = (ctypes.c_int32 * (7 * n))(*[int(v) for p in params for v in p])
        assert len(flat) == 7 * n
        pals = None
        if palettes is not None and any(p is not None for p in palettes):
            keep = [None if p is None else bytes(p) for p in palettes]
            assert all(p is None or len(p) == 768 for p in keep)
            pals = (ctypes.c_char_p * n)(*keep)
        status = (ctypes.c_int * n)()
        self._chk(self.lib.lumina_ocr_strip_image_decode(self._h, ptrs, sizes, m, counts, n, int(height), int(width), int(rows_per_strip), flat, pals,
                                                         _ptr(out), status, self._stream()))
        return out, list(status)

    @property
    def jpeg_last_passes(self) -> int:
        return int(self.lib.lumina_ocr_jpeg_last_passes(self._h))

    def jpeg_coefficients(self, pages, quality: int = 95):
        torch = _torch()
        n, h, w, _ = pages.shape
        mcus = ((w + 15) // 16) * ((h + 15) // 16)
        coefs = torch.empty((n, mcus, 6, 64), dtype=torch.int16, device=pages.device)
        self._chk(self.lib.lumina_ocr_jpeg_coefficients(self._h, _ptr(pages), n, h, w, int(quality), _ptr(coefs), self._stream()))
        return coefs

    def set_option(self, key: str, value: int):
        self._chk(self.lib.lumina_ocr_set_option(self._h, key.encode(), int(value)))

    def version(self) -> str:
        return self.lib.lumina_ocr_version().decode()

    def load_det(self, weights):
        blob = weights if isinstance(weights, (bytes, bytearray)) else arch.write_blob(weights)
        buf = ctypes.create_string_buffer(bytes(blob), len(blob))
        self._chk(self.lib.lumina_ocr_load_det_weights(self._h, ctypes.cast(buf, ctypes.c_void_p), len(blob)))
        self.det_loaded = True

    def load_rec(self, weights):
        blob = weights if isinstance(weights, (bytes, bytearray)) else arch.write_blob(weights)
        buf = ctypes.create_string_buffer(bytes(blob), len(blob))
        self._chk(self.lib.lumina_ocr_load_rec_weights(self._h, ctypes.cast(buf, ctypes.c_void_p), len(blob)))
        self.num_classes = self.lib.lumina_ocr_num_classes(self._h)
        self.rec_loaded = True

    def load_cls(self, weights):
        blob = weights if isinstance(weights, (bytes, bytearray)) else arch.write_blob(weights)
        buf = ctypes.create_string_buffer(bytes(blob), len(blob))
        self._chk(self.lib.lumina_ocr_load_cls_weights(self._h, ctypes.cast(buf, ctypes.c_void_p), len(blob)))
        self.cls_loaded = True

    def load_svtr(self, weights, f16=None):
        self.set_option("svtr_f16", -1 if f16 is None else int(bool(f16)))
        blob = weights if isinstance(weights, (bytes, bytearray)) else arch.write_blob(weights)
        buf = ctypes.create_string_buffer(bytes(blob), len(blob))
        self._chk(self.lib.lumina_ocr_load_svtr_weights(self._h, ctypes.cast(buf, ctypes.c_void_p), len(blob)))
        self.svtr_loaded = True
        self.svtr_num_classes = self.lib.lumina_ocr_svtr_num_classes(self._h)
        self.svtr_dtype = "f16" if self.lib.lumina_ocr_svtr_dtype(self._h) else "bf16"

    def normalize(self, img, hp: int, wp: int, scale, shift, nchw: bool = False):
        torch = _torch()
        n, h, w, _ = img.shape
        out = torch.empty((n, 3, hp, wp) if nchw else (n, hp, wp, 3), dtype=torch.bfloat16, device=img.device)
        sc = (ctypes.c_float * 3)(*scale)
        sh = (ctypes.c_float * 3)(*shift)
        self._chk(self.lib.lumina_ocr_normalize(self._h, _ptr(img), n, h, w, hp, wp, sc, sh, int(nchw), _ptr(out), self._stream()))
        return out

    def det_forward(self, pages, hp: Optional[int] = None, wp: Optional[int] = None, out=None):
        torch = _torch()
        assert pages.dtype == torch.uint8 and pages.is_cuda and pages.is_contiguous() and pages.shape[-1] == 3
        b, h, w, _ = pages.shape
        hp = hp or (h + 31) // 32 * 32
        wp = wp or (w + 31) // 32 * 32
        if out is None:
            out = torch.empty((b, hp, wp), dtype=torch.bfloat16, device=pages.device)
        self._chk(self.lib.lumina_ocr_det_forward(self._h, _ptr(pages), b, h, w, hp, wp, _ptr(out), self._stream()))
        return out

    def det_postprocess(self, prob, valid_h: int, valid_w: int, thresh=arch.DET_THRESH, box_thresh=arch.DET_BOX_THRESH,
                        unclip_ratio=arch.DET_UNCLIP_RATIO, min_size=arch.DET_MIN_SIZE, max_boxes=MAX_BOXES):
        torch = _torch()
        b, hp, wp = prob.shape
        boxes = torch.zeros((b, max_boxes, 8), dtype=torch.int32, device=prob.device)
        scores = torch.zeros((b, max_boxes), dtype=torch.float32, device=prob.device)
        counts = torch.zeros((b,), dtype=torch.int32, device=prob.device)
        self._chk(self.lib.lumina_ocr_det_postprocess(self._h, _ptr(prob), b, hp, wp, valid_h, valid_w, thresh, box_thresh,
                                                      unclip_ratio, min_size, max_boxes, _ptr(boxes), _ptr(scores), _ptr(counts),
                                                      self._stream()))
        return boxes, scores, counts

    def rec_crop(self, pages, quads, page_idx, flip=None):
        torch = _torch()
        b, h, w, _ = pages.shape
        n = quads.shape[0]
        crops = torch.empty((n, REC_H, REC_W, 3), dtype=torch.uint8, device=pages.device)
        widths = torch.empty((n,), dtype=torch.int32, device=pages.device)
        if n and flip is None:
            self._chk(self.lib.lumina_ocr_rec_crop(self._h, _ptr(pages), b, h, w, _ptr(quads), _ptr(page_idx), n, _ptr(crops),
                                                   _ptr(widths), self._stream()))
        elif n:
            if flip.dtype != torch.int32 or flip.device != pages.device or tuple(flip.shape) != (n,):
                raise ValueError("flip must be int32 [%d] on %s" % (n, pages.device))
            flip = flip.contiguous()
            self._chk(self.lib.lumina_ocr_rec_crop_oriented(self._h, _ptr(pages), b, h, w, _ptr(quads), _ptr(page_idx), n, _ptr(flip),
                                                            _ptr(crops), _ptr(widths), self._stream()))
        return crops, widths

    def cls_crop(self, pages, quads, page_idx):
        torch = _torch()
        b, h, w, _ = pages.shape
        n = quads.shape[0]
        crops = torch.empty((n, arch.CLS_H, arch.CLS_W, 3), dtype=torch.uint8, device=pages.device)
        widths = torch.empty((n,), dtype=torch.int32, device=pages.device)
        if n:
            self._chk(self.lib.lumina_ocr_cls_crop(self._h, _ptr(pages), b, h, w, _ptr(quads), _ptr(page_idx), n, _ptr(crops),
                                                   _ptr(widths), self._stream()))
        return crops, widths

    def cls_forward(self, crops, widths=None, thresh: float = arch.CLS_THRESH):
        torch = _torch()
        n = crops.shape[0]
        label = torch.empty((n,), dtype=torch.int32, device=crops.device)
        score = torch.empty((n,), dtype=torch.float32, device=crops.device)
        flip = torch.empty((n,), dtype=torch.int32, device=crops.device)
        if n:
            if crops.dtype != torch.uint8 or tuple(crops.shape[1:]) != (arch.CLS_H, arch.CLS_W, 3) or not crops.is_contiguous():
                raise ValueError("crops must be contiguous uint8 [n, %d, %d, 3]" % (arch.CLS_H, arch.CLS_W))
            self._chk(self.lib.lumina_ocr_cls_forward(self._h, _ptr(crops), _ptr(widths), n, float(thresh), _ptr(label), _ptr(score), _ptr(flip),
                                                      self._stream()))
        return label, score, flip

    def rec_forward(self, crops, widths=None):
        torch = _torch()
        n = crops.shape[0]
        idx = torch.empty((n, REC_T), dtype=torch.int32, device=crops.device)
        prob = torch.empty((n, REC_T), dtype=torch.float32, device=crops.device)
        if n:
            self._chk(self.lib.lumina_ocr_rec_forward(self._h, _ptr(crops), _ptr(widths), n, _ptr(idx), _ptr(prob), self._stream()))
        return idx, prob

    def svtr_forward(self, crops, widths=None):
        torch = _torch()
        n = crops.shape[0]
        idx = torch.empty((n, REC_T), dtype=torch.int32, device=crops.device)
        prob = torch.empty((n, REC_T), dtype=torch.float32, device=crops.device)
        if n:
            self._chk(self.lib.lumina_ocr_svtr_forward(self._h, _ptr(crops), _ptr(widths), n, _ptr(idx), _ptr(prob), self._stream()))
        return idx, prob

    def ctc_decode(self, idx, prob):
        torch = _torch()
# ... 331 lines not shown
```

Measured before the change: 1625 pages/sec.

## Add transposed tile orientation for fused block-entry conv and rework stem kernel

Adds an optional transposed tile mapping to the fused 3x3 stride-2 shortcut conv kernel, picked automatically when it wastes less padding for the output shape. Separately reworks the fused stem kernel: a fast interior path for u8 halo fill, a byte-permute gather that replaces per-element LDS loads, a padded t1 tile pitch in place of the XOR swizzle, and earlier weight/bias loads interleaved with the MFMAs. Together these aim to cut wasted tile work on edge tiles and reduce LDS gather overhead in the stem. They add complexity, and the gather and permute selectors could break correctness if the halo layout assumptions are off.

```diff
diff --git a/include/lumina_ocr.h b/include/lumina_ocr.h
--- a/include/lumina_ocr.h
+++ b/include/lumina_ocr.h
@@ -20,6 +20,7 @@
 const char* lumina_ocr_last_error(const lumina_ocr_t* h);
 const char* lumina_ocr_version(void);
 int lumina_ocr_set_option(lumina_ocr_t* h, const char* key, int value);
+int lumina_ocr_entry_orientation(int ho, int wo, int orientation);
 
 int lumina_ocr_load_det_weights(lumina_ocr_t* h, const void* blob, size_t nbytes);
 int lumina_ocr_load_rec_weights(lumina_ocr_t* h, const void* blob, size_t nbytes);
diff --git a/ocr-system_amd/csrc/capi.hip b/ocr-system_amd/csrc/capi.hip
--- a/ocr-system_amd/csrc/capi.hip
+++ b/ocr-system_amd/csrc/capi.hip
@@ -120,6 +120,7 @@
     }
     if (hipSetDevice(device) != hipSuccess) { eng->err = "hipSetDevice failed"; *out = eng; return 2; }
     if (const char* e = getenv("LUMINA_RING_ORIENT")) eng->ring_orient = atoi(e) < 0 ? -1 : (atoi(e) != 0);
+    if (const char* e = getenv("LUMINA_ENTRY_ORIENT")) eng->entry_orient = atoi(e) < 0 ? -1 : (atoi(e) != 0);
     if (getenv("LUMINA_CONV_NO_RING")) eng->conv_ring = false;
     if (getenv("LUMINA_BLOCKED")) eng->blocked_layout = atoi(getenv("LUMINA_BLOCKED")) != 0;
     *out = eng;
@@ -152,6 +153,7 @@
     else if (!strcmp(key, "blocked_layout")) h->blocked_layout = value != 0;
     else if (!strcmp(key, "conv_big_min")) h->conv_big_min = value >= 0 ? value : 1024;
     else if (!strcmp(key, "ring_orient")) h->ring_orient = value < 0 ? -1 : (value != 0);
+    else if (!strcmp(key, "entry_orient")) h->entry_orient = value < 0 ? -1 : (value != 0);
     else if (!strcmp(key, "post_group")) h->post_group = value > 0 ? value : 1;
     else if (!strcmp(key, "tail_group")) h->tail_group = value > 0 ? value : 0;
     else if (!strcmp(key, "svtr_f16")) h->svtr_f16 = value < 0 ? -1 : (value != 0);
@@ -160,6 +162,8 @@
     else return locr_fail(h, "set_option: unknown key", key);
     return 0;
 }
+
+int lumina_ocr_entry_orientation(int ho, int wo, int orientation) { return conv_entry_transposed(ho, wo, orientation); }
 
 int lumina_ocr_load_det_weights(lumina_ocr_t* h, const void* blob, size_t nbytes) {
     if (!h || !blob) return 1;
diff --git a/ocr-system_amd/csrc/conv_mfma.h b/ocr-system_amd/csrc/conv_mfma.h
--- a/ocr-system_amd/csrc/conv_mfma.h
+++ b/ocr-system_amd/csrc/conv_mfma.h
@@ -39,6 +39,7 @@
     const float* bias2;
     bf16_t* y2;
     int y2_cstride;
+    int transposed;
 };
 
 struct ConvKernelCfg {
@@ -51,6 +52,7 @@
 bool conv_pick_cfg(int ks, int stride, int cin, int cout_gemm, ConvKernelCfg* cfg);
 hipError_t conv_launch(const ConvKernelCfg& cfg, ConvParams p, hipStream_t stream);
 const char* conv_kernel_name(const ConvKernelCfg& cfg);
+int conv_entry_transposed(int ho, int wo, int orientation);
 
 bool conv_ring_supported(const ConvKernelCfg& cfg, const ConvParams& p);
 bool conv_ring_transposed(const ConvParams& p, int orientation);
diff --git a/ocr-system_amd/csrc/conv_mfma.hip b/ocr-system_amd/csrc/conv_mfma.hip
--- a/ocr-system_amd/csrc/conv_mfma.hip
+++ b/ocr-system_amd/csrc/conv_mfma.hip
@@ -10,6 +10,7 @@
     static constexpr bool DMA = (DB == 3 || DB == 4);
     static constexpr bool POOL = (DB == 4);
     static constexpr bool SC = (DB == 5);
+    static constexpr bool ORI = SC;
     static_assert(!SC || (KS == 3 && S == 2 && CK == 16), "fused shortcut: the 3x3 / stride-2 block-entry kernel");
     static constexpr int TH = NW * MT;
     static constexpr int PAD = (KS == 3) ? 1 : 0;
@@ -62,6 +63,7 @@
     unsigned char* sA = smem;
     unsigned char* sW = sA + C::A_BYTES;
     const int r = lane & 31, h = lane >> 5;
+    const bool tr = C::ORI && p.transposed != 0;
 
     const int lid = xcd_remap(blockIdx.x, gridDim.x);
     const int ntile = lid % p.n_tiles;
@@ -87,8 +89,9 @@
     for (int it = 0; it < C::AIT; ++it) {
         const int i = tid + NTHR * it;
         const int pi = i / C::NPL, c = i - pi * C::NPL;
-        const int hy = pi / C::HW, hx = pi - hy * C::HW;
-        const int iy = iy0 + hy, ix = ix0 + hx;
+        int hy = pi / C::HW, hx = pi - hy * C::HW;
+        if (tr) { hx = pi / C::HH; hy = pi - hx * C::HH; }
+        const int iy = tr ? ix0 + hx : iy0 + hy, ix = tr ? iy0 + hy : ix0 + hx;
         const bool item = i < C::A_ITEMS;
         const bool inb = item && iy >= 0 && iy < p.H && ix >= 0 && ix < p.W && (p.pix_limit == 0 || iy * p.W + ix < p.pix_limit);
         a_goff[it] = inb ? (iy * p.W + ix) * pstride + c * 8 : -1;
@@ -194,6 +197,16 @@
         const int ty = wave * MT + mt, tx = r;
         aoff[mt] = h * C::A_SL + ((ty * S) * C::HWP + tx * S) * C::A_PIX;
     }
+    int aoff_t[C::ORI ? MT : 1][C::ORI ? 2 * KS - 1 : 1];
+    if constexpr (C::ORI) {
+#pragma unroll
+        for (int mt = 0; mt < MT; ++mt)
+#pragma unroll
+            for (int dd = 0; dd < 2 * KS - 1; ++dd) {
+                const int d = dd - (KS - 1), m = d < 0 ? -d : 0;
+                aoff_t[mt][dd] = aoff[mt] + ((tr ? d * C::HWP : d) + m * (C::HWP + 1)) * C::A_PIX;
+            }
+    }
     const int woff = h * C::W_SL + r * C::W_ROW;
     const int woff2 = h * (C::W2_ROWS * 16) + r * 16;
 
@@ -203,7 +216,8 @@
     {                                                                                                              \
         const int tap_ = (st_) / (CK / 16), kc_ = (st_) % (CK / 16), kh_ = tap_ / KS, kw_ = tap_ % KS;              \
         _Pragma("unroll") for (int mt = 0; mt < MT; ++mt)                                                           \
-            bfr[set_][mt] = lds_frag(sA + (boff_) + aoff[mt] + (2 * kc_) * C::A_SL + (kh_ * C::HWP + kw_) * C::A_PIX); \
+            bfr[set_][mt] = lds_frag(sA + (boff_) + (2 * kc_) * C::A_SL + (C::ORI ? aoff_t[C::ORI ? mt : 0][C::ORI ? kw_ - kh_ + KS - 1 : 0] + (kw_ < kh_ ? kw_ : kh_) * (C::HWP + 1) * C::A_PIX \
+                                                                                  : aoff[mt] + (kh_ * C::HWP + kw_) * C::A_PIX));                        \
         _Pragma("unroll") for (int nt = 0; nt < C::NT; ++nt)                                                       \
             afr[set_][nt] = lds_frag(sW + (boff_) + woff + (2 * kc_) * C::W_SL + (tap_ * BN + nt * 32) * C::W_ROW);   \
     }
@@ -267,7 +281,7 @@
 #pragma unroll
         for (int mt = 0; mt < MT; ++mt) {
             const int ty = wave * MT + mt, tx = r;
-            const int oy = oyb + ty, ox = oxb + tx;
+            const int oy = tr ? oxb + tx : oyb + ty, ox = tr ? oyb + ty : oxb + tx;
             const bool pvalid = oy >= 0 && ox >= 0 && oy < p.Ho && ox < p.Wo && (p.pix_limit == 0 || oy * p.Wo + ox < p.pix_limit);
             const bf16_t* rrow = p.res + (((size_t)n_img * p.res_h + (oy >> p.res_shift)) * p.res_w + (ox >> p.res_shift)) * p.res_cstride + ntile * BN;
 #pragma unroll
@@ -313,7 +327,7 @@
         if (direct) {
 #pragma unroll
             for (int mt = 0; mt < MT; ++mt) {
-                const int oy = oyb + wave * MT + mt, ox = oxb + r;
+                const int oy = tr ? oxb + r : oyb + wave * MT + mt, ox = tr ? oyb + wave * MT + mt : oxb + r;
                 const bool pvalid = oy < p.Ho && ox < p.Wo;
 #pragma unroll
                 for (int nt = 0; nt < C::NT; ++nt)
@@ -334,7 +348,7 @@
                 const float* b2 = p.bias2 + ntile * BN;
 #pragma unroll
                 for (int mt = 0; mt < MT; ++mt) {
-                    const int oy = oyb + wave * MT + mt, ox = oxb + r;
+                    const int oy = tr ? oxb + r : oyb + wave * MT + mt, ox = tr ? oyb + wave * MT + mt : oxb + r;
                     const bool pvalid = oy < p.Ho && ox < p.Wo;
 #pragma unroll
                     for (int nt = 0; nt < C::NT; ++nt)
@@ -530,6 +544,14 @@
     return true;
 }
 
+static long long entry_padded(int ho, int wo, int transposed) {
+    const int lh = transposed ? wo : ho, lw = transposed ? ho : wo;
+    return (long long)ceil_div(lh, 8) * 8 * ceil_div(lw, 32) * 32;
+}
+int conv_entry_transposed(int ho, int wo, int orientation) {
+    return orientation < 0 ? 8 * entry_padded(ho, wo, 1) <= 7 * entry_padded(ho, wo, 0) : orientation != 0;
+}
+
 const char* conv_kernel_name(const ConvKernelCfg& c) {
     static thread_local char buf[64];
     const int db = c.nw == 6 ? 3 : 0, mt = (c.nw == 5 || c.nw == 6) ? 4 : 2;
@@ -551,7 +573,9 @@
         if (cfg.ks == 3 && cfg.stride == 1 && cfg.bn == 64 && cfg.ck == 16) return launch_t<3, 1, 64, 16, 32, 4, 0, 4>(p, stream);
         return hipErrorInvalidValue;
     }
+    if (p.transposed && p.wpk2 == nullptr) return hipErrorInvalidValue;
     if (p.wpk2 != nullptr) {
+        if (p.transposed) { p.tiles_x = ceil_div(p.Ho, 32); p.tiles_y = ceil_div(p.Wo, 8); }
         if (!(cfg.ks == 3 && cfg.stride == 2 && cfg.bn == 64 && cfg.ck == 16 && cfg.nw == 4) || p.out_mode != OUT_NORMAL || (dbg & 32) || p.bias2 == nullptr ||
             p.y2 == nullptr || p.H % 2 != 0 || p.W % 2 != 0 || p.res != nullptr || p.y2_cstride % 8 != 0) return hipErrorInvalidValue;
         return launch_t<3, 2, 64, 16, 32, 4, 5, 2>(p, stream);
diff --git a/ocr-system_amd/csrc/engine.h b/ocr-system_amd/csrc/engine.h
--- a/ocr-system_amd/csrc/engine.h
+++ b/ocr-system_amd/csrc/engine.h
@@ -128,6 +128,7 @@
     int svtr_f16 = -1;
     int conv2d_variant = 0;
     int ring_orient = -1;
+    int entry_orient = -1;
     bool fuse_short = true;
     bool fpn_compose = true;
     bool fpn_multi = true;
diff --git a/ocr-system_amd/csrc/engine.hip b/ocr-system_amd/csrc/engine.hip
--- a/ocr-system_amd/csrc/engine.hip
+++ b/ocr-system_amd/csrc/engine.hip
@@ -393,6 +393,7 @@
     ConvChoice k;
     RUN(conv_choose(eng, L, p, c, &k));
     p.wpk = k.wpk;
+    if (p.wpk2 != nullptr && k.kernel == CONV_TILE_8X32) p.transposed = conv_entry_transposed(p.Ho, p.Wo, eng->entry_orient);
     hipError_t e = conv_dispatch(eng, k, p, st);
     if (e != hipSuccess) return locr_fail(eng, L.name.c_str(), hipGetErrorString(e));
     if (tm.on()) conv_account(eng, L, x, c, p, k, &tm);
@@ -431,6 +432,8 @@
     if (!fuse_stem) {
         tap(eng, "stem.conv1", t1);
         RUN(eng_run_conv(eng, c2, t1, &t2, st)); tap(eng, "stem.conv2", t2);
+    } else {
+        tap(eng, "stem.conv2", t2);
     }
     const bool fuse_pool = eng->fuse_pool && eng->keep_taps != 1;
     Tensor4 t3{};
diff --git a/ocr-system_amd/csrc/stem_conv.hip b/ocr-system_amd/csrc/stem_conv.hip
--- a/ocr-system_amd/csrc/stem_conv.hip
+++ b/ocr-system_amd/csrc/stem_conv.hip
@@ -4,13 +4,14 @@
 
 constexpr int TH = 8, TW = 32;
 constexpr int HH = 2 * (TH - 1) + 3, HW = 2 * (TW - 1) + 3;
-constexpr int ROW = HW * 3 + 1;
+constexpr int HALO_PADL = 4;
+constexpr int ROW = HW * 3 + 9;
 constexpr int STAGE_PITCH = 32 * 2 + 16;
 
 template <int NHH, int NHW, int NROW>
 __device__ __forceinline__ void fill_halo_u8(bf16_t* halo, const StemParams& p, int n_img, int iy0, int ix0, int vh, int vw, int tid) {
     constexpr int SEG = NHW * 3, WPR = (SEG + 3) / 4 + 1, NIT = (NHH * WPR + 255) / 256;
-    static_assert(NROW > SEG, "one dump element per row");
+    static_assert(NROW >= SEG + 9 && NROW % 2 == 0 && HALO_PADL >= 3 && 4 * (WPR - 1) + 3 < SEG + 9 - HALO_PADL, "a word's four elements stay inside its row");
     const long long img_off = (long long)n_img * p.H * p.W * 3, all_bytes = (long long)p.N * p.H * p.W * 3;
     const unsigned char* xal = p.x + (img_off & ~3ll);
     const int mis = (int)(img_off & 3);
@@ -19,6 +20,38 @@
     const float sc0 = p.scale[0], sc1 = p.scale[1], sc2 = p.scale[2], sh0 = p.shift[0], sh1 = p.shift[1], sh2 = p.shift[2];
     uint32_t word[NIT];
     int e0s[NIT];
+    const int qa = mis + (iy0 * p.W + ix0) * 3, qz = mis + ((iy0 + NHH - 1) * p.W + ix0) * 3;
+    const bool interior = iy0 >= 0 && iy0 + NHH <= vh && ix0 >= 0 && ix0 + NHW <= vw && (qa & ~3) >= lo_lim && (qz & ~3) + 4 * WPR <= hi_lim;
+    if (interior) {
+#pragma unroll
+        for (int u = 0; u < NIT; ++u) {
+            const int i = min(tid + 256 * u, NHH * WPR - 1);
+            const int hy = i / WPR, wi = i - hy * WPR;
+            const int q = mis + ((iy0 + hy) * p.W + ix0) * 3, w0 = (q & ~3) + 4 * wi;
+            e0s[u] = w0 - q;
+            word[u] = *reinterpret_cast<const uint32_t*>(xal + w0);
+        }
+#pragma unroll
+        for (int u = 0; u < NIT; ++u) {
+            const int i = min(tid + 256 * u, NHH * WPR - 1);
+            const int hy = i / WPR;
+            const int e0 = e0s[u];
+            const unsigned c0 = (unsigned)(e0 + 3) % 3u;
+            bf16_t* hw = halo + hy * NROW + e0;
+            float S[4], T[4];
+            S[0] = c0 == 0 ? sc0 : (c0 == 1 ? sc1 : sc2); S[1] = c0 == 0 ? sc1 : (c0 == 1 ? sc2 : sc0); S[2] = c0 == 0 ? sc2 : (c0 == 1 ? sc0 : sc1); S[3] = S[0];
+            T[0] = c0 == 0 ? sh0 : (c0 == 1 ? sh1 : sh2); T[1] = c0 == 0 ? sh1 : (c0 == 1 ? sh2 : sh0); T[2] = c0 == 0 ? sh2 : (c0 == 1 ? sh0 : sh1); T[3] = T[0];
+            float v[4];
+#pragma unroll
+            for (int b = 0; b < 4; ++b) {
+                v[b] = (float)((word[u] >> (8 * b)) & 0xffu) * S[b];
+                v[b] = v[b] + T[b];
+            }
+            const uint32_t lo = pack_bf16x2(v[0], v[1]), hi = pack_bf16x2(v[2], v[3]);
+            hw[0] = (bf16_t)lo; hw[1] = (bf16_t)(lo >> 16); hw[2] = (bf16_t)hi; hw[3] = (bf16_t)(hi >> 16);
+        }
+        return;
+    }
 #pragma unroll
     for (int u = 0; u < NIT; ++u) {
         const int i = tid + 256 * u;
@@ -79,9 +112,40 @@
         }
 }
 
+struct StemGather { int r0, r1, t1; uint32_t s00, s0, s10, s11, s12; };
+template <int NROW>
+__device__ __forceinline__ StemGather stem_gather_setup(int h) {
+    static_assert(NROW % 2 == 0, "halo rows start on a dword");
+    constexpr int RD = NROW / 2;
+    StemGather g;
+    g.r0 = h ? RD : 0;
+    g.r1 = h ? 2 * RD : RD;
+    g.t1 = h ? 0 : 2 * RD;
+    g.s00 = h ? 0x05040100u : 0x07060504u; g.s0 = h ? 0x05040302u : 0x07060504u;
+    g.s10 = h ? 0x03020100u : 0x05040302u; g.s11 = h ? 0x05040100u : 0x07060504u; g.s12 = h ? 0x01000100u : 0x07060504u;
+    return g;
+}
+__device__ __forceinline__ uint32_t stem_perm(uint32_t hi, uint32_t lo, uint32_t sel) { return __builtin_amdgcn_perm(hi, lo, sel); }
+__device__ __forceinline__ void stem_gather(const uint32_t* hb, const StemGather& g, bf16x8_t (&b)[2]) {
+    union { bf16x8_t v; uint32_t w[4]; } o;
+    {
+        const uint32_t* rr = hb + g.r0;
+        const uint32_t hd = hb[4], a0 = rr[0], a1 = rr[1], a2 = rr[2], a3 = rr[3];
+        o.w[0] = stem_perm(a0, hd, g.s00); o.w[1] = stem_perm(a1, a0, g.s0); o.w[2] = stem_perm(a2, a1, g.s0); o.w[3] = stem_perm(a3, a2, g.s0);
+        b[0] = o.v;
+    }
+    {
+        const uint32_t* pr = hb + g.r1;
+        const uint32_t* tr = hb + g.t1;
+        const uint32_t p3 = pr[3], p4 = pr[4], t0 = tr[0], t1 = tr[1], t2 = tr[2];
+        o.w[0] = stem_perm(p4, p3, g.s10); o.w[1] = stem_perm(t0, p4, g.s11); o.w[2] = stem_perm(t1, t0, g.s12); o.w[3] = stem_perm(t2, t0, g.s12);
+        b[1] = o.v;
+    }
+}
+
 __global__ __launch_bounds__(256) void stem_conv_kernel(const StemParams p) {
     __shared__ __attribute__((aligned(16))) unsigned char smem[256 * STAGE_PITCH > HH * ROW * 2 ? 256 * STAGE_PITCH : HH * ROW * 2];
-    bf16_t* halo = reinterpret_cast<bf16_t*>(smem);
+    bf16_t* halo = reinterpret_cast<bf16_t*>(smem) + HALO_PADL;
 
     const int tid = threadIdx.x, lane = tid & 63, wave = tid >> 6, r = lane & 31, h = lane >> 5;
     const int tiles_x = (p.Wo + TW - 1) / TW, tiles_y = (p.Ho + TH - 1) / TH;
@@ -155,12 +219,14 @@
 
 constexpr int F_T1H = TH + 2, F_T1W = TW + 2, F_T1PX = F_T1H * F_T1W;
 constexpr int F_HH = 2 * (F_T1H - 1) + 3, F_HW = 2 * (F_T1W - 1) + 3;
-constexpr int F_ROW = F_HW * 3 + 1;
-constexpr int F_HALO_BYTES = F_HH * F_ROW * 2, F_T1_BYTES = ((F_T1PX + 31) / 32) * 32 * 64;
+constexpr int F_ROW = F_HW * 3 + 9;
+static_assert((F_HH * F_ROW * 2) % 16 == 0, "the t1 tile starts on 16 bytes");
+constexpr int F_T1PITCH = 80;
+constexpr int F_HALO_BYTES = F_HH * F_ROW * 2, F_T1_BYTES = ((F_T1PX + 31) / 32) * 32 * F_T1PITCH;
 __global__ __launch_bounds__(256) void stem12_kernel(const StemParams p, const bf16_t* w2pk, const float* bias2) {
     static_assert(256 * STAGE_PITCH <= F_T1_BYTES, "the output stage re-uses the t1 tile");
     __shared__ __attribute__((aligned(16))) unsigned char smem[F_HALO_BYTES + F_T1_BYTES];
-    bf16_t* halo = reinterpret_cast<bf16_t*>(smem);
+    bf16_t* halo = reinterpret_cast<bf16_t*>(smem) + HALO_PADL;
     unsigned char* t1 = smem + F_HALO_BYTES;
     const int tid = threadIdx.x, lane = tid & 63, wave = tid >> 6, r = lane & 31, h = lane >> 5;
     const int tiles_x = (p.Wo + TW - 1) / TW, tiles_y = (p.Ho + TH - 1) / TH;
@@ -172,37 +238,34 @@
 
     const int y1_0 = tile_y * TH - 1, x1_0 = tile_x * TW - 1;
     const int iy0 = 2 * y1_0 - 1, ix0 = 2 * x1_0 - 1;
+    bf16x8_t a1[2];
+#pragma unroll
+    for (int ks = 0; ks < 2; ++ks) a1[ks] = *reinterpret_cast<const bf16x8_t*>(p.wpk + ((ks * 2 + h) * 32 + r) * 8);
+    float4 b1[4];
+#pragma unroll
+    for (int g = 0; g < 4; ++g) b1[g] = *reinterpret_cast<const float4*>(p.bias + 8 * g + 4 * h);
     fill_halo_u8<F_HH, F_HW, F_ROW>(halo, p, n_img, iy0, ix0, vh, vw, tid);
+    bf16x8_t w2[9];
+#pragma unroll
+    for (int tap = 0; tap < 9; ++tap) w2[tap] = *reinterpret_cast<const bf16x8_t*>(w2pk + ((size_t)h * (9 * 32) + tap * 32 + r) * 8);
     __syncthreads();
 
     {
-        bf16x8_t a1[2];
-#pragma unroll
-        for (int ks = 0; ks < 2; ++ks) a1[ks] = *reinterpret_cast<const bf16x8_t*>(p.wpk + ((ks * 2 + h) * 32 + r) * 8);
-        float4 b1[4];
-#pragma unroll
-        for (int g = 0; g < 4; ++g) b1[g] = *reinterpret_cast<const float4*>(p.bias + 8 * g + 4 * h);
-        int koff[2][8];
-        stem_koff<F_ROW>(h, koff);
+        const StemGather sg = stem_gather_setup<F_ROW>(h);
         for (int tile = wave; tile * 32 < F_T1PX; tile += 4) {
             const int pidx = tile * 32 + r;
             const int pc = min(pidx, F_T1PX - 1);
             const int py = pc / F_T1W, px = pc - py * F_T1W;
-            const bf16_t* hb = halo + (2 * py) * F_ROW + 6 * px;
+            bf16x8_t b[2];
+            stem_gather(reinterpret_cast<const uint32_t*>(halo) + py * F_ROW + 3 * px, sg, b);
             f32x16_t acc;
 #pragma unroll
             for (int j = 0; j < 16; ++j) acc[j] = 0.f;
 #pragma unroll
-            for (int ks = 0; ks < 2; ++ks) {
-                union { bf16x8_t v; bf16_t s[8]; } b;
-#pragma unroll
-                for (int j = 0; j < 8; ++j) b.s[j] = hb[koff[ks][j]];
-                acc = __builtin_amdgcn_mfma_f32_32x32x16_bf16(a1[ks], b.v, acc, 0, 0, 0);
-            }
+            for (int ks = 0; ks < 2; ++ks) acc = __builtin_amdgcn_mfma_f32_32x32x16_bf16(a1[ks], b[ks], acc, 0, 0, 0);
             const int y1 = y1_0 + py, x1 = x1_0 + px;
             const bool inimg = y1 >= 0 && y1 < p.Ho && x1 >= 0 && x1 < p.Wo;
             if (pidx < F_T1PX) {
-                const int swz = (pidx >> 2) & 3;
 #pragma unroll
                 for (int g = 0; g < 4; ++g) {
                     uint2 o = make_uint2(0, 0);
@@ -210,14 +273,11 @@
                         o.x = pack_bf16x2(fmaxf(acc[4 * g + 0] + b1[g].x, 0.f), fmaxf(acc[4 * g + 1] + b1[g].y, 0.f));
                         o.y = pack_bf16x2(fmaxf(acc[4 * g + 2] + b1[g].z, 0.f), fmaxf(acc[4 * g + 3] + b1[g].w, 0.f));
                     }
-                    *reinterpret_cast<uint2*>(t1 + pidx * 64 + ((g ^ swz) * 16) + 8 * h) = o;
+                    *reinterpret_cast<uint2*>(t1 + pidx * F_T1PITCH + g * 16 + 8 * h) = o;
                 }
             }
         }
     }
-    bf16x8_t w2[9];
-#pragma unroll
-    for (int tap = 0; tap < 9; ++tap) w2[tap] = *reinterpret_cast<const bf16x8_t*>(w2pk + ((size_t)h * (9 * 32) + tap * 32 + r) * 8);
     __syncthreads();
 
     f32x16_t acc2[2];
@@ -225,20 +285,25 @@
     for (int mt = 0; mt < 2; ++mt)
 #pragma unroll
         for (int j = 0; j < 16; ++j) acc2[mt][j] = 0.f;
+    const unsigned char* t1c = t1 + (wave * 2 * F_T1W + r) * F_T1PITCH + h * 16;
+    float4 b2[4];
 #pragma unroll
     for (int kc = 0; kc < 2; ++kc) {
+        if (kc == 1) {
+#pragma unroll
+            for (int g = 0; g < 4; ++g) b2[g] = *reinterpret_cast<const float4*>(bias2 + 8 * g + 4 * h);
+        }
 #pragma unroll
         for (int tap = 0; tap < 9; ++tap) {
 #pragma unroll
             for (int mt = 0; mt < 2; ++mt) {
-                const int pp = (wave * 2 + mt + tap / 3) * F_T1W + r + tap % 3;
-                const bf16x8_t bf = *reinterpret_cast<const bf16x8_t*>(t1 + pp * 64 + (((2 * kc + h) ^ ((pp >> 2) & 3)) * 16));
+                const bf16x8_t bf = *reinterpret_cast<const bf16x8_t*>(t1c + ((mt + tap / 3) * F_T1W + tap % 3) * F_T1PITCH + kc * 32);
                 acc2[mt] = __builtin_amdgcn_mfma_f32_32x32x16_bf16(w2[tap], bf, acc2[mt], 0, 0, 0);
             }
-        }
-        if (kc == 0) {
-#pragma unroll
-            for (int tap = 0; tap < 9; ++tap) w2[tap] = *reinterpret_cast<const bf16x8_t*>(w2pk + ((size_t)(2 + h) * (9 * 32) + tap * 32 + r) * 8);
+            if (kc == 0) {
+                w2[tap] = *reinterpret_cast<const bf16x8_t*>(w2pk + ((size_t)(2 + h) * (9 * 32) + tap * 32 + r) * 8);
+                __builtin_amdgcn_sched_barrier(0x38F);
+            }
         }
     }
     __syncthreads();
@@ -249,7 +314,7 @@
         const int tp = (wave * 2 + mt) * TW + r;
 #pragma unroll
         for (int g = 0; g < 4; ++g) {
-            const float4 b4 = *reinterpret_cast<const float4*>(bias2 + 8 * g + 4 * h);
+            const float4 b4 = b2[g];
             uint2 o;
             o.x = pack_bf16x2(apply_act(acc2[mt][4 * g + 0] + b4.x, ACT_RELU), apply_act(acc2[mt][4 * g + 1] + b4.y, ACT_RELU));
             o.y = pack_bf16x2(apply_act(acc2[mt][4 * g + 2] + b4.z, ACT_RELU), apply_act(acc2[mt][4 * g + 3] + b4.w, ACT_RELU));
diff --git a/ocr-system_amd/lumina_ocr/engine.py b/ocr-system_amd/lumina_ocr/engine.py
--- a/ocr-system_amd/lumina_ocr/engine.py
+++ b/ocr-system_amd/lumina_ocr/engine.py
@@ -104,6 +104,7 @@
         "lumina_ocr_page_quarter": (i32, [vp, vp, i32, i32, i32, i32, i32, vp, vp, vp]),
         "lumina_ocr_page_turn": (i32, [vp, vp, i32, i32, i32, vp, i32, i32, vp, vp]),
         "lumina_ocr_page_vote": (i32, [vp, vp, vp, i32, i32, vp, vp]),
+        "lumina_ocr_entry_orientation": (i32, [i32, i32, i32]),
     }
     missing = []
     for name, (res, args) in sig.items():
@@ -131,6 +132,7 @@
     "lumina_ocr_table_rules", "lumina_ocr_selection_marks", "lumina_ocr_rules_and_marks", "lumina_ocr_selection_marks_round",
     "lumina_ocr_rules_and_marks_round", "lumina_ocr_barcodes", "lumina_ocr_barcodes_kinds", "lumina_ocr_qrcodes", "lumina_ocr_qrcodes_versions", "lumina_ocr_datamatrix", "lumina_ocr_aztec", "lumina_ocr_aztec_workspace_bytes", "lumina_ocr_aztec_layers", "lumina_ocr_aztec_layers_workspace_bytes",
     "lumina_ocr_page_quarter_workspace_bytes", "lumina_ocr_page_quarter", "lumina_ocr_page_turn", "lumina_ocr_page_vote",
+    "lumina_ocr_entry_orientation",
 ]
 
 
```

New measurement: 1636 pages/sec, median of 6. About the same (+0.7%).
